# GuyTevet/motion-diffusion-model

Hardware: AMD Instinct MI355X
Metric: motions/sec (B=128, T=196, 50-step DDPM) (higher is better)
Workload: dtype f16x3 (fp32 operands split into fp16 hi+lo, 3 fp16 MFMA products, fp32 accumulate; everything else fp32); 1 GPU; HumanML3D text2motion, 50-step p_sample_loop with CFG 2.5 (2 denoiser forwards per step), batch=128 per GPU, T=196, 8-layer d=512 trans_enc MDM, random-init weights, cached text embedding; global_batch=128, diffusion_steps=50, parallelism=dp1: batch shards, no data-path collective, all_gather of final samples

## Files before the change

include/mdm_hip_probe.h:

```cpp
#ifndef MDM_HIP_PROBE_H
#define MDM_HIP_PROBE_H

#include "mdm_hip.h"

#ifdef __cplusplus
extern "C" {
#endif

int mdm_debug_set(int what, int value);
int mdm_debug_get(int idx, double* out);

size_t mdm_linear_f16f6_scratch_bytes(int32_t M, int32_t N, int32_t K);
int mdm_linear_f16f6(const float* in_dev, const float* w_dev, const float* bias_dev, const float* res_dev,
                     float* out_dev, int32_t M, int32_t N, int32_t K, int32_t act, void* scratch_dev,
                     size_t scratch_bytes, void* stream);

int mdm_probe_in_proj(const float* tokens, const float* w, const float* bias, void* planes_dev, int32_t nseq, int32_t S,
                      int32_t D, void* scratch_dev, void* stream);

int mdm_probe_attention_x3(const float* qkv_dev, float* out_dev, void* out_hi_dev, void* out_lo_dev, const int32_t* lengths_dev,
                           int32_t nseq, int32_t B, int32_t S, int32_t D, int32_t H, int32_t lead, int32_t wide, void* scratch_dev,
                           size_t scratch_bytes, void* stream);

#ifdef __cplusplus
}
#endif
#endif
```

motion-diffusion-model_amd/_native.py:

```python
import ctypes as C
import os

_HERE = os.path.dirname(os.path.abspath(__file__))
LIB_NAME = "libmdm_hip.so"
LIB_PATH = os.path.join(_HERE, "csrc", LIB_NAME)
PROBE_LIB_PATH = os.path.join(_HERE, "csrc", "libmdm_hip_probe.so")

MDM_OK = 0
BRANCH_COND, BRANCH_UNCOND, BRANCH_BOTH = 0, 1, 2
ACT_NONE, ACT_GELU, ACT_SILU = 0, 1, 2
PRECISIONS = {"f32": 0, "f16x3": 1}
PROF_CLASSES = ("linear", "attention", "layernorm", "embed", "outproj", "elementwise")

EXPORTED_SYMBOLS = [
    "mdm_abi_version", "mdm_build_info", "mdm_last_error", "mdm_create", "mdm_destroy", "mdm_set_weight", "mdm_const_bytes",
    "mdm_prepare", "mdm_workspace_bytes", "mdm_forward", "mdm_sampler_step", "mdm_randn", "mdm_sample_loop",
    "mdm_linear", "mdm_layernorm", "mdm_attention", "mdm_profile_enable", "mdm_profile_read", "mdm_profile_reset",
    "mdm_set_precision", "mdm_linear_x3", "mdm_linear_x3_scratch_bytes", "mdm_attention_x3", "mdm_attention_x3_scratch_bytes",
    "mdm_recover_from_ric", "mdm_workspace_bytes_dec", "mdm_forward_dec", "mdm_workspace_bytes_dec_loop",
    "mdm_sample_loop_dec", "mdm_weights_in_range", "mdm_set_option", "mdm_get_option", "mdm_set_time_add",
    "mdm_rot6d_to_smpl_joints", "mdm_smpl_workspace_bytes", "mdm_smpl_forward",
    "mdm_eval_workspace_bytes", "mdm_eval_motion_embeddings", "mdm_eval_text_embeddings",
    "mdm_text_workspace_bytes", "mdm_text_encode",
    "mdm_stgcn_workspace_bytes", "mdm_stgcn_forward",
    "mdm_gru_cls_workspace_bytes", "mdm_gru_cls_forward",
    "mdm_clip_text_workspace_bytes", "mdm_clip_text_encode",
]
PROBE_SYMBOLS = ["mdm_debug_set", "mdm_debug_get", "mdm_linear_f16f6", "mdm_linear_f16f6_scratch_bytes", "mdm_probe_in_proj",
                 "mdm_probe_attention_x3"]
ABI_VERSION = 10
OPTIONS = {"small_gemm_max_seqs": 1, "small_gemm_row_tiles": 2, "dec_fused_xattn": 3, "dec_fused_selfattn": 4, "attn_direct_out": 5,
           "dec_time_token": 6, "enc_shared_layer0": 7, "attn_wide": 8}
ARCH = {"trans_enc": 0, "trans_dec": 1}


class MdmConfig(C.Structure):
    _fields_ = [(n, C.c_int32) for n in ("njoints", "nfeats", "latent_dim", "ff_size", "num_layers", "num_heads",
                                         "clip_dim", "max_len", "mask_frames", "arch", "context_len")]


class MdmSmplModel(C.Structure):
    _fields_ = [(n, C.c_void_p) for n in ("j0", "jdirs", "blend", "weights_t", "sel_blend", "sel_weights_t", "extra_t")] + \
               [("parents", C.POINTER(C.c_int32))] + [(n, C.c_int32) for n in ("J", "V", "n_sel", "n_extra")]


class MdmSmplCall(C.Structure):
    _fields_ = [(n, C.c_int32) for n in ("pose_rep", "glob", "translation", "vertstrans", "n_points", "root_point")] + \
               [("point_map", C.POINTER(C.c_int32)), ("glob_rot_mat", C.POINTER(C.c_float)), ("beta1", C.c_float)]


class MdmEvalGru(C.Structure):
    _fields_ = [(n, C.c_void_p) for n in ("in_w", "in_b", "w_ih", "b_ih", "w_hh", "b_hh", "h0", "o1_w", "o1_b", "ln_g", "ln_b",
                                          "o2_w", "o2_b")] + [(n, C.c_int32) for n in ("in_dim", "hidden", "out")]


class MdmEvalModel(C.Structure):
    _fields_ = [(n, C.c_void_p) for n in ("conv1_w", "conv1_b", "conv2_w", "conv2_b", "out_w", "out_b", "pos_w", "pos_b")] + \
               [("motion", MdmEvalGru), ("text", MdmEvalGru)] + \
               [(n, C.c_int32) for n in ("dim_pose", "conv_hidden", "latent", "word", "pos", "unit_length")]


class MdmTextLayer(C.Structure):
    _fields_ = [(n, C.c_void_p) for n in ("qkv_w", "qkv_b", "out_w", "out_b", "sa_ln_g", "sa_ln_b", "lin1_w", "lin1_b", "lin2_w",
                                          "lin2_b", "out_ln_g", "out_ln_b")]


class MdmTextModel(C.Structure):
    _fields_ = [(n, C.c_void_p) for n in ("word_emb", "pos_emb", "emb_ln_g", "emb_ln_b")] + [("layers", C.POINTER(MdmTextLayer))] + \
               [(n, C.c_int32) for n in ("n_layers", "dim", "n_heads", "hidden", "vocab", "max_pos")] + [("ln_eps", C.c_float)]


class MdmStgcnBlock(C.Structure):
    _fields_ = [(n, C.c_void_p) for n in ("gcn_w", "gcn_scale", "gcn_shift", "nbr_idx", "nbr_w", "nbr_cnt", "tcn_w", "tcn_scale",
                                          "tcn_shift", "res_w", "res_scale", "res_shift")] + \
               [(n, C.c_int32) for n in ("c_in", "c_out", "stride", "residual")]


class MdmStgcnModel(C.Structure):
    _fields_ = [("blocks", C.POINTER(MdmStgcnBlock))] + [(n, C.c_void_p) for n in ("in_scale", "in_shift", "fcn_w", "fcn_b")] + \
               [(n, C.c_int32) for n in ("n_blocks", "V", "K", "num_class")]


class MdmGruClsLayer(C.Structure):
    _fields_ = [(n, C.c_void_p) for n in ("w_ih", "w_hh", "b_ih", "b_hh")]


GRU_CLS_MAX_LAYERS = 4


class MdmGruClsModel(C.Structure):
    _fields_ = [("layers", MdmGruClsLayer * GRU_CLS_MAX_LAYERS)] + [(n, C.c_void_p) for n in ("lin1_w", "lin1_b", "lin2_w", "lin2_b")] + \
               [(n, C.c_int32) for n in ("input_size", "hidden_size", "num_layers", "mid", "num_class")]


class MdmClipTextLayer(C.Structure):
    _fields_ = [(n, C.c_void_p) for n in ("ln1_g", "ln1_b", "qkv_w", "qkv_b", "out_w", "out_b", "ln2_g", "ln2_b", "fc_w", "fc_b", "proj_w",
                                          "proj_b")]


class MdmClipTextModel(C.Structure):
    _fields_ = [(n, C.c_void_p) for n in ("tok_emb", "pos_emb", "lnf_g", "lnf_b", "text_proj")] + [("layers", C.POINTER(MdmClipTextLayer))] + \
               [(n, C.c_int32) for n in ("n_layers", "dim", "n_heads", "mlp", "vocab", "max_pos", "embed")]


STGCN_RES = {"none": 0, "identity": 1, "conv": 2}
STGCN_MAX_BLOCKS, STGCN_MAX_NEIGHBOURS = 16, 8

SMPL_POSE_REPS = {"rot6d": 0, "rotvec": 1, "rotmat": 2, "rotquat": 3}
SMPL_REP_FEATS = {"rot6d": 6, "rotvec": 3, "rotmat": 9, "rotquat": 4}


class MdmStep(C.Structure):
    _fields_ = [("a_x0", C.c_float), ("a_xt", C.c_float), ("sigma", C.c_float), ("clip_denoised", C.c_int32),
                ("seed", C.c_uint64), ("sample_base", C.c_uint32), ("draw", C.c_uint32), ("const_noise", C.c_int32)]


class MdmSampleParams(C.Structure):
    _fields_ = [
        ("B", C.c_int32), ("T", C.c_int32), ("num_timesteps", C.c_int32), ("start_index", C.c_int32),
        ("a_x0", C.c_void_p), ("a_xt", C.c_void_p), ("sigma", C.c_void_p), ("timestep_map", C.c_void_p),
        ("text_embed_dev", C.c_void_p), ("scale_dev", C.c_void_p), ("lengths_dev", C.c_void_p),
        ("inpaint_mask_dev", C.c_void_p), ("inpaint_motion_dev", C.c_void_p), ("noise_dev", C.c_void_p),
        ("seed", C.c_uint64), ("sample_base", C.c_uint32), ("clip_denoised", C.c_int32),
        ("force_uncond", C.c_int32), ("x0_dev", C.c_void_p), ("dump_steps", C.c_void_p), ("num_dump", C.c_int32),
        ("dump_dev", C.c_void_p), ("const_noise", C.c_int32),
    ]


class MdmSampleDecParams(C.Structure):
    _fields_ = [("loop", MdmSampleParams), ("ntok", C.c_int32), ("prefix_dev", C.c_void_p),
                ("text_lengths_dev", C.c_void_p)]


class MdmError(RuntimeError):
    pass


class MdmLib:

    def __init__(self, path):
        if not os.path.isfile(path):
            raise MdmError(
                f"{path} not found: the MI355X HIP extension is not built. Run `python __graft_entry__.py build` "
                f"(hipcc --offload-arch=gfx950). There is no CPU fallback for this path.")
        self.path = path
        lib = self.lib = C.CDLL(path)
        vp, i32, i64, u32, u64, f32, sz = C.c_void_p, C.c_int32, C.c_int64, C.c_uint32, C.c_uint64, C.c_float, C.c_size_t
        P = C.POINTER
        sig = {
            "mdm_abi_version": (C.c_int, []),
            "mdm_last_error": (C.c_char_p, []),
            "mdm_build_info": (C.c_char_p, []),
            "mdm_create": (C.c_int, [P(MdmConfig), P(vp)]),
            "mdm_destroy": (None, [vp]),
            "mdm_set_weight": (C.c_int, [vp, C.c_char_p, vp, i64]),
            "mdm_const_bytes": (sz, [vp]),
            "mdm_prepare": (C.c_int, [vp, vp, sz, vp]),
            "mdm_workspace_bytes": (sz, [vp, i32, i32]),
            "mdm_forward": (C.c_int, [vp, vp, vp, vp, vp, i32, i32, i32, vp, vp, sz, vp]),
            "mdm_sampler_step": (C.c_int, [vp, vp, vp, vp, vp, vp, vp, vp, vp, i32, i32, P(MdmStep), vp]),
            "mdm_randn": (C.c_int, [vp, vp, vp, f32, f32, i32, i32, u64, u32, u32, vp]),
            "mdm_sample_loop": (C.c_int, [vp, P(MdmSampleParams), vp, vp, sz, vp]),
            "mdm_linear": (C.c_int, [vp, vp, vp, vp, vp, i32, i32, i32, i32, vp]),
            "mdm_layernorm": (C.c_int, [vp, vp, vp, i32, i32, vp]),
            "mdm_attention": (C.c_int, [vp, vp, vp, i32, i32, i32, i32, i32, vp]),
            "mdm_set_precision": (C.c_int, [vp, i32]),
            "mdm_weights_in_range": (C.c_int, [vp, P(i32), vp]),
            "mdm_linear_x3_scratch_bytes": (sz, [i32, i32, i32]),
            "mdm_linear_x3": (C.c_int, [vp, vp, vp, vp, vp, i32, i32, i32, i32, vp, sz, vp]),
            "mdm_attention_x3_scratch_bytes": (sz, [i32, i32, i32]),
            "mdm_attention_x3": (C.c_int, [vp, vp, vp, i32, i32, i32, i32, i32, vp, sz, vp]),
            "mdm_recover_from_ric": (C.c_int, [vp, vp, vp, vp, i32, i32, i32, i32, vp]),
            "mdm_workspace_bytes_dec": (sz, [vp, i32, i32, i32]),
            "mdm_forward_dec": (C.c_int, [vp, vp, vp, vp, vp, vp, vp, i32, i32, i32, i32, vp, vp, sz, vp]),
            "mdm_workspace_bytes_dec_loop": (sz, [vp, i32, i32, i32, i32]),
            "mdm_sample_loop_dec": (C.c_int, [vp, P(MdmSampleDecParams), vp, vp, sz, vp]),
            "mdm_profile_enable": (C.c_int, [vp, C.c_int]),
            "mdm_profile_read": (C.c_int, [vp, i32, P(C.c_double), P(i64), P(C.c_double)]),
            "mdm_profile_reset": (C.c_int, [vp]),
            "mdm_set_option": (C.c_int, [vp, i32, i32]),
            "mdm_get_option": (C.c_int, [vp, i32, P(i32)]),
            "mdm_set_time_add": (C.c_int, [vp, vp, i32]),
            "mdm_rot6d_to_smpl_joints": (C.c_int, [vp, vp, P(f32), P(i32), vp, i32, i32, i32, i32, vp]),
            "mdm_smpl_workspace_bytes": (sz, [P(MdmSmplModel), P(MdmSmplCall), i32, i32]),
            "mdm_smpl_forward": (C.c_int, [P(MdmSmplModel), P(MdmSmplCall), vp, vp, vp, vp, vp, i32, i32, i32, i32, vp, sz, vp]),
            "mdm_eval_workspace_bytes": (sz, [P(MdmEvalModel), i32, i32, i32]),
            "mdm_eval_motion_embeddings": (C.c_int, [P(MdmEvalModel), vp, vp, vp, i32, i32, i32, vp, sz, vp]),
            "mdm_eval_text_embeddings": (C.c_int, [P(MdmEvalModel), vp, vp, vp, vp, i32, i32, i32, vp, sz, vp]),
            "mdm_text_workspace_bytes": (sz, [P(MdmTextModel), i32, i32]),
            "mdm_text_encode": (C.c_int, [P(MdmTextModel), vp, vp, vp, i32, i32, i32, vp, sz, vp]),
            "mdm_clip_text_workspace_bytes": (sz, [P(MdmClipTextModel), i32, i32]),
            "mdm_clip_text_encode": (C.c_int, [P(MdmClipTextModel), vp, vp, vp, i32, i32, vp, sz, vp]),
            "mdm_stgcn_workspace_bytes": (sz, [P(MdmStgcnModel), i32, i32]),
            "mdm_stgcn_forward": (C.c_int, [P(MdmStgcnModel), vp, vp, vp, i32, i32, vp, sz, vp]),
            "mdm_gru_cls_workspace_bytes": (sz, [P(MdmGruClsModel), i32, i32]),
            "mdm_gru_cls_forward": (C.c_int, [P(MdmGruClsModel), vp, vp, vp, vp, vp, i32, i32, vp, sz, vp]),
        }
        probe_sig = {
            "mdm_debug_set": (C.c_int, [C.c_int, C.c_int]),
            "mdm_debug_get": (C.c_int, [C.c_int, P(C.c_double)]),
            "mdm_linear_f16f6_scratch_bytes": (sz, [i32, i32, i32]),
            "mdm_linear_f16f6": (C.c_int, [vp, vp, vp, vp, vp, i32, i32, i32, i32, vp, sz, vp]),
            "mdm_probe_in_proj": (C.c_int, [vp, vp, vp, vp, i32, i32, i32, vp, vp]),
            "mdm_probe_attention_x3": (C.c_int, [vp, vp, vp, vp, vp, i32, i32, i32, i32, i32, i32, i32, vp, sz, vp]),
        }
        self.has_probes = hasattr(lib, "mdm_debug_set")
        if self.has_probes:
            sig.update(probe_sig)
        for name, (res, args) in sig.items():
            fn = getattr(lib, name)
            fn.restype = res
            fn.argtypes = args
        if lib.mdm_abi_version() != ABI_VERSION:
            raise MdmError(f"{path}: ABI version {lib.mdm_abi_version()} != {ABI_VERSION}")
        self.build_info = dict(kv.split("=", 1) for kv in lib.mdm_build_info().decode().split(";"))
        if self.build_info.get("emu") != "1" and self.build_info.get("slp") != "off" \
                and os.environ.get("MDM_ALLOW_SLP_BUILD") != "1":
            raise MdmError(f"{path} was built without -fno-slp-vectorize -DMDM_NO_SLP=1 (mdm_build_info: "
                           f"{lib.mdm_build_info().decode()}): rebuild with `python __graft_entry__.py`, or set "
                           f"MDM_ALLOW_SLP_BUILD=1 for an A/B experiment on an otherwise idle device")

    def check(self, rc, what):
        if rc != MDM_OK:
            msg = self.lib.mdm_last_error()
            raise MdmError(f"{what} failed (rc={rc}): {msg.decode() if msg else ''}")

    def __getattr__(self, name):
        return getattr(self.lib, name)


_LIB = None


def load_native():
    global _LIB
    if _LIB is None:
        _LIB = MdmLib(os.environ.get("MDM_HIP_LIB", LIB_PATH))
    return _LIB


_PROBE_LIB = None


def load_probe():
    global _PROBE_LIB
    if _PROBE_LIB is None:
        _PROBE_LIB = MdmLib(os.environ.get("MDM_HIP_PROBE_LIB", PROBE_LIB_PATH))
        if not _PROBE_LIB.has_probes:
            raise MdmError(f"{_PROBE_LIB.path} was not built with -DMDM_PROBES")
    return _PROBE_LIB
```

motion-diffusion-model_amd/csrc/api_launch.h:

```cpp
#pragma once

namespace {

struct Workspace {
  float *tok, *qkv, *att, *ffn, *cond;
  QkvPlanes qp;
  p16_t *xah, *xal;
  float *stat1, *stat2;
  p16_t *tokh, *tokl;
  p16_t *atth, *attl;
  p16_t *ffnh, *ffnl;
  size_t bytes;
};

QkvPlanes carve_qkv_planes(float* qkv, size_t nseq, size_t S, size_t D, int H) {
  const size_t NKT = (S + 31) / 32, SP = 32 * NKT, plane = nseq * SP * D;
  p16_t* q = reinterpret_cast<p16_t*>(qkv);
  QkvPlanes qp{};
  qp.qh = q; qp.SP = (int)SP; qp.NKT = (int)NKT; qp.H = H;
  if (q != nullptr) { qp.ql = q + plane; qp.kh = q + 2 * plane; qp.kl = q + 3 * plane; qp.vh = q + 4 * plane; qp.vl = q + 5 * plane; }
  return qp;
}

Workspace carve(const mdm_model* m, int nseq, int T, void* base) {
  const size_t D = m->cfg.latent_dim, FF = m->cfg.ff_size, S = (size_t)T + 1, M = (size_t)nseq * S;
  size_t off = 0;
  auto take = [&](size_t floats) {
    size_t o = off;
    off += align_up(floats * sizeof(float), 256);
    return base ? reinterpret_cast<float*>(static_cast<char*>(base) + o) : nullptr;
  };
  Workspace w;
  w.tok = take(M * D);
  const size_t NKT = (S + 31) / 32, SP = 32 * NKT;
  w.qkv = take((size_t)nseq * SP * 3 * D);
  w.att = take(M * D);
  w.ffn = take(M * std::max(FF, (size_t)m->jf_k));
  w.cond = take((size_t)nseq * D);
  float* tp = take(M * D);
  w.tokh = reinterpret_cast<p16_t*>(tp);
  w.tokl = tp ? w.tokh + M * D : nullptr;
  w.atth = reinterpret_cast<p16_t*>(w.att);
  w.attl = w.att ? w.atth + M * D : nullptr;
  w.ffnh = reinterpret_cast<p16_t*>(w.ffn);
  w.ffnl = w.ffn ? w.ffnh + M * FF : nullptr;
  w.xah = reinterpret_cast<p16_t*>(w.tok);
  w.xal = w.tok ? w.xah + M * D : nullptr;
  const size_t parts = (D + 127) / 128;
  w.stat1 = take(M * parts * 2 + 4);
  w.stat2 = take(M * parts * 2 + 4);
  w.qp = carve_qkv_planes(w.qkv, nseq, S, D, m->cfg.num_heads);
  w.bytes = off;
  return w;
}

int launch_layernorm(Profiler* pf, float* x, const float* g, const float* b, int rows, int D, p16_t* xh, p16_t* xl,
                     hipStream_t s, bool write_f32 = true) {
  ProfScope ps(pf, MDM_PROF_LAYERNORM, 0.0, s);
  const dim3 grid((rows + 3) / 4), block(256);
  switch (D / 256) {
    case 1: { auto k = &layernorm_kernel<1>; MDM_LAUNCH(k, grid, block, 0, s, x, g, b, rows, 1e-5f, xh, xl, (int)write_f32); break; }
    case 2: { auto k = &layernorm_kernel<2>; MDM_LAUNCH(k, grid, block, 0, s, x, g, b, rows, 1e-5f, xh, xl, (int)write_f32); break; }
    case 3: { auto k = &layernorm_kernel<3>; MDM_LAUNCH(k, grid, block, 0, s, x, g, b, rows, 1e-5f, xh, xl, (int)write_f32); break; }
    case 4: { auto k = &layernorm_kernel<4>; MDM_LAUNCH(k, grid, block, 0, s, x, g, b, rows, 1e-5f, xh, xl, (int)write_f32); break; }
    default: return fail(MDM_EUNSUPPORTED, "layernorm: D must be 256, 512, 768 or 1024");
  }
  return rt_launch_status();
}

template <int NKT>
int launch_attention_t(const AttnF32Args& a, float* out, int nseq, int D, int H, p16_t* oh, p16_t* ol, hipStream_t s) {
  auto k = &attention_f32_kernel<NKT>;
  const int nqt = (a.Sq + 31) / 32;
  const size_t lds = attention_lds_bytes(NKT, nqt);
  if (int rc = rt_allow_lds(k, lds)) return rc;
  MDM_LAUNCH(k, dim3(nseq * H), dim3(64 * nqt), lds, s, a, out, D, H, oh, ol);
  return rt_launch_status();
}

int launch_attention_args(Profiler* pf, const AttnF32Args& a, float* out, int nseq, int D, int H, p16_t* oh, p16_t* ol,
                          hipStream_t s) {
  ProfScope ps(pf, MDM_PROF_ATTENTION, 4.0 * nseq * H * (double)a.Sq * a.Sk * ATT_HD, s);
  if (D != H * ATT_HD) return fail(MDM_EUNSUPPORTED, "attention: head_dim must be 128");
  if (a.Sq < 1 || a.Sk < 1) return fail(MDM_EUNSUPPORTED, "attention: no tokens");
  if (a.Sq > 224 || a.Sk > 224) {
    const int nqb = al_query_blocks(a.Sq);
    MDM_LAUNCH(attention_f32_long_kernel, dim3(nseq * H * nqb), dim3(256), al_f32_lds_bytes(), s, a, out, D, H, oh, ol, nqb);
    return rt_launch_status();
  }
  switch ((a.Sk + 31) / 32) {
    case 1: return launch_attention_t<1>(a, out, nseq, D, H, oh, ol, s);
    case 2: return launch_attention_t<2>(a, out, nseq, D, H, oh, ol, s);
    case 3: return launch_attention_t<3>(a, out, nseq, D, H, oh, ol, s);
    case 4: return launch_attention_t<4>(a, out, nseq, D, H, oh, ol, s);
    case 5: return launch_attention_t<5>(a, out, nseq, D, H, oh, ol, s);
    case 6: return launch_attention_t<6>(a, out, nseq, D, H, oh, ol, s);
    default: return launch_attention_t<7>(a, out, nseq, D, H, oh, ol, s);
  }
}

int launch_attention(Profiler* pf, const float* qkv, float* out, const int* lengths, int nseq, int B, int S, int D,
                     int H, p16_t* oh, p16_t* ol, hipStream_t s, int lead = 1, int len_B = 0, int len_b0 = 0) {
  AttnF32Args a{qkv, 3 * D, qkv + D, qkv + 2 * D, 3 * D, S, S, lengths, lead, B};
  a.len_B = len_B;
  a.len_b0 = len_b0;
  return launch_attention_args(pf, a, out, nseq, D, H, oh, ol, s);
}

template <int NKT, bool DIRECT>
int launch_attention_x3_t(const QkvPlanes& qp, const int* lengths, int nseq, int B, int S, int D, float* out, p16_t* oh,
                          p16_t* ol, hipStream_t s, int lead) {
  auto k = &attention_x3_kernel<NKT, DIRECT>;
  const size_t lds = attention_x3_lds_bytes(NKT);
  if (int rc = rt_allow_lds(k, lds)) return rc;
  const int items = nseq * qp.H, groups = (items + 7) / 8;
  const int grid = std::min(groups * 16, std::max(16, 2 * x3_grid_limit() / 16 * 16));
  MDM_LAUNCH(k, dim3(grid), dim3(256), lds, s, qp, lengths, S, D, B, lead, out, oh, ol, items);
  return rt_launch_status();
}
template <bool DIRECT>
int launch_attention_x3_nkt(const QkvPlanes& qp, const int* lengths, int nseq, int B, int S, int D, float* out, p16_t* oh,
                            p16_t* ol, hipStream_t s, int lead) {
  switch (qp.NKT) {
    case 1: return launch_attention_x3_t<1, DIRECT>(qp, lengths, nseq, B, S, D, out, oh, ol, s, lead);
    case 2: return launch_attention_x3_t<2, DIRECT>(qp, lengths, nseq, B, S, D, out, oh, ol, s, lead);
    case 3: return launch_attention_x3_t<3, DIRECT>(qp, lengths, nseq, B, S, D, out, oh, ol, s, lead);
    case 4: return launch_attention_x3_t<4, DIRECT>(qp, lengths, nseq, B, S, D, out, oh, ol, s, lead);
    case 5: return launch_attention_x3_t<5, DIRECT>(qp, lengths, nseq, B, S, D, out, oh, ol, s, lead);
    case 6: return launch_attention_x3_t<6, DIRECT>(qp, lengths, nseq, B, S, D, out, oh, ol, s, lead);
    default: return launch_attention_x3_t<7, DIRECT>(qp, lengths, nseq, B, S, D, out, oh, ol, s, lead);
  }
}

template <int NKT>
int launch_attention_x3_wide_t(const QkvPlanes& qp, const int* lengths, int nseq, int B, int S, int D, float* out, p16_t* oh,
                               p16_t* ol, hipStream_t s, int lead) {
  auto k = &attention_x3_kernel_wide<NKT>;
  const size_t lds = (size_t)axw_lds_bytes(NKT);
  if (int rc = rt_allow_lds(k, lds)) return rc;
  const int items = nseq * qp.H;
  const int grid = std::min(items, x3_grid_limit());
  MDM_LAUNCH(k, dim3(grid), dim3(AXW_THREADS), lds, s, qp, lengths, S, D, B, lead, out, oh, ol, items);
  return rt_launch_status();
}

int launch_attention_x3(Profiler* pf, const QkvPlanes& qp, const int* lengths, int nseq, int B, int S, int D, float* out,
                        p16_t* oh, p16_t* ol, hipStream_t s, int lead = 1, bool direct = false, bool wide = true) {
  ProfScope ps(pf, MDM_PROF_ATTENTION, 4.0 * nseq * qp.H * (double)S * S * AX_HD, s);
  if (D != qp.H * AX_HD) return fail(MDM_EUNSUPPORTED, "attention: head_dim must be 128");
  if (S < 1) return fail(MDM_EUNSUPPORTED, "attention: no tokens");
  if (S > 224) {
    if (qp.NKT != (S + 31) / 32 || qp.SP != 32 * qp.NKT) return fail(MDM_EINVAL, "attention: the operand planes do not match the sequence length");
    const int nqb = al_query_blocks(S);
    MDM_LAUNCH(attention_x3_long_kernel, dim3(nseq * qp.H * nqb), dim3(256), al_x3_lds_bytes(), s, qp, lengths, S, D, B, lead, out, oh, ol, nqb);
    return rt_launch_status();
  }
  if (direct && out == nullptr && oh != nullptr)
    return launch_attention_x3_nkt<true>(qp, lengths, nseq, B, S, D, out, oh, ol, s, lead);
  if (wide && qp.NKT >= 5) {
    if (qp.NKT != (S + 31) / 32 || qp.SP != 32 * qp.NKT) return fail(MDM_EINVAL, "attention: the operand planes do not match the sequence length");
    switch (qp.NKT) {
      case 5: return launch_attention_x3_wide_t<5>(qp, lengths, nseq, B, S, D, out, oh, ol, s, lead);
      case 6: return launch_attention_x3_wide_t<6>(qp, lengths, nseq, B, S, D, out, oh, ol, s, lead);
      default: return launch_attention_x3_wide_t<7>(qp, lengths, nseq, B, S, D, out, oh, ol, s, lead);
    }
  }
  return launch_attention_x3_nkt<false>(qp, lengths, nseq, B, S, D, out, oh, ol, s, lead);
}

struct X3Call {
  X3Kind kind = X3K_OUT_LN_RES;
  Profiler* pf = nullptr; int prof_cat = MDM_PROF_LINEAR;
  X3Operand a{nullptr, nullptr}; X3Weights w{nullptr, nullptr}; const float* bias = nullptr;
  float* out = nullptr; p16_t* oh = nullptr; p16_t* ol = nullptr; const QkvPlanes* qp = nullptr;
  int M = 0, N = 0, K = 0, S = 0, D = 0;
  int scale_cols = 0; float col_scale = 1.f;
  const float* astat = nullptr; const float* colsum = nullptr;
  X3Operand res{nullptr, nullptr}; const float* rstat = nullptr; const float* rgamma = nullptr; const float* rbeta = nullptr;
  float* ostat = nullptr;
  int parts = 1; float inv_dim = 1.f;
  const float* res_f32 = nullptr; int emb_T = 1, emb_B = 1, emb_nbranch = 1;
  bool small = false;
  X3sShape shape{1};
  int stat_cols = 256;
};
X3Epilogue x3_epilogue(const X3Call& c) {
  X3Epilogue ep{};
  ep.out = c.out; ep.bias = c.bias; ep.res = c.res_f32; ep.resh = c.res.hi; ep.resl = c.res.lo; ep.oh = c.oh; ep.ol = c.ol;
  ep.ld = c.N; ep.scale_cols = c.scale_cols; ep.col_scale = c.col_scale;
  if (c.qp != nullptr) ep.qkv = *c.qp;
  ep.S = c.S; ep.D = c.D;
  ep.astat = c.astat; ep.colsum = c.colsum; ep.rstat = c.rstat; ep.rgamma = c.rgamma; ep.rbeta = c.rbeta; ep.ostat = c.ostat;
  ep.stat_parts = c.parts; ep.inv_dim = c.inv_dim; ep.emb_T = c.emb_T; ep.emb_B = c.emb_B; ep.emb_nbranch = c.emb_nbranch;
  ep.stat_cols = c.stat_cols;
  return ep;
}

#ifdef MDM_PROBES
int g_f6_linear = 0;
void* g_f6_dbg_scratch = nullptr;
size_t g_f6_dbg_bytes = 0;
int launch_linear_f6_debug(Profiler* pf, const float* in, int ld_in, const float* w, const float* bias, const float* res,
                           float* out, int M, int N, int K, int act, int scale_cols, float col_scale, hipStream_t s) {
  const size_t wfrag = align_up(x3_packed_weight_elems(N, K) * 2, 256);
  const size_t need = f6_plane_bytes(M, K) + 2 * wfrag;
  if (need > g_f6_dbg_bytes) {
#ifdef MDM_EMU
    free(g_f6_dbg_scratch);
    g_f6_dbg_scratch = malloc(need);
#else
    if (hipDeviceSynchronize() != hipSuccess) return fail(MDM_EHIP, "f16f6 debug mode: synchronize failed");
    if (g_f6_dbg_scratch != nullptr) (void)hipFree(g_f6_dbg_scratch);
    if (hipMalloc(&g_f6_dbg_scratch, need) != hipSuccess) { g_f6_dbg_scratch = nullptr; g_f6_dbg_bytes = 0; return fail(MDM_EHIP, "f16f6 debug mode: hipMalloc failed"); }
#endif
    g_f6_dbg_bytes = need;
  }
  ProfScope ps(pf, MDM_PROF_LINEAR, 2.0 * M * (double)N * K, s);
  char* base = static_cast<char*>(g_f6_dbg_scratch);
  const F6Planes pa = f6_carve(base, M, K);
  p16_t* wfh = reinterpret_cast<p16_t*>(base + f6_plane_bytes(M, K));
  p16_t* wfl = reinterpret_cast<p16_t*>(base + f6_plane_bytes(M, K) + wfrag);
  MDM_LAUNCH(pack_f16f6_kernel, dim3((M * (K / 32) + 255) / 256), dim3(256), 0, s, in, pa, M, K, ld_in);
  if (int rc = rt_launch_status()) return rc;
  const int npad = (N + 31) / 32 * 32;
  MDM_LAUNCH(pack_weight_f16f6_kernel, dim3((npad * (K / 32) + 255) / 256), dim3(256), 0, s, w, wfh, wfl, N, K);
  if (int rc = rt_launch_status()) return rc;
  X3Call c; c.out = out; c.bias = bias; c.res_f32 = res; c.N = N; c.scale_cols = scale_cols; c.col_scale = col_scale;
  X3Epilogue ep = x3_epilogue(c);
  ep.acc_scale = 1.f;
  const X3Operand a{reinterpret_cast<const p16_t*>(pa.h16), reinterpret_cast<const p16_t*>(pa.rec)};
  const int rc = launch_gemm_f16f6(a, X3Weights{wfh, wfl}, ep, M, N, K, act, s);
  if (rc != 0) return fail(MDM_EUNSUPPORTED, "f16f6 debug mode: launch failed");
  return rt_launch_status();
}
#endif

int launch_linear(Profiler* pf, const float* in, int ld_in, const float* w, const float* bias, const float* res,
                  float* out, int M, int N, int K, int act, int scale_cols, float col_scale, hipStream_t s, bool x3 = false) {
#ifdef MDM_PROBES
  if (g_f6_linear && K % 32 == 0 && N % 4 == 0 && ld_in % 4 == 0 && (scale_cols % 256 == 0) &&
      (act == ACT_NONE || (act == ACT_GELU && res == nullptr)))
    return launch_linear_f6_debug(pf, in, ld_in, w, bias, res, out, M, N, K, act, scale_cols, col_scale, s);
#endif
  ProfScope ps(pf, MDM_PROF_LINEAR, 2.0 * M * (double)N * K, s);
  if (K % 4 != 0 || ld_in % 4 != 0) return fail(MDM_EINVAL, "linear: K and the row stride must be multiples of 4");
  RowMajorLoader al{in, ld_in, M, K};
  RowMajorLoader bl{w, K, N, K};
  LinearEpilogue ep{out, bias, res, N, act, scale_cols, col_scale, nullptr, nullptr};
  launch_gemm_f32(al, bl, ep, M, N, K, s, x3);
  return rt_launch_status();
}

int launch_linear_lnfold(Profiler* pf, const float* in, int ld_in, const LnFold& a_ln, const float* w, X3Weights wp,
                         const float* bias, const float* colsum, const float* res, const LnFold& res_ln, float* out,
                         float* ostat, int M, int N, int K, int act, int scale_cols, float col_scale, hipStream_t s, bool x3) {
  ProfScope ps(pf, MDM_PROF_LINEAR, 2.0 * M * (double)N * K, s);
  if (K % 16 != 0 || ld_in % 4 != 0 || N % LN_PART_COLS != 0) return fail(MDM_EINVAL, "linear (LayerNorm fold): bad K / N");
  RowMajorLoader al{in, ld_in, M, K};
  LnLinearEpilogue ep{out, bias, N, act, scale_cols, col_scale, a_ln, colsum, res, res_ln, ostat};
  if (x3 && wp.hi != nullptr) {
    X3FragB bl{wp.hi, wp.lo, (N + 31) / 32, K};
    launch_gemm_f32(al, bl, ep, M, N, K, s, true);
  } else {
    RowMajorLoader bl{w, K, N, K};
    launch_gemm_f32(al, bl, ep, M, N, K, s, x3);
  }
  return rt_launch_status();
}

int launch_linear_x3(Profiler* pf, X3Operand a, X3Weights w, const float* bias, const float* res, float* out,
                     p16_t* oh, p16_t* ol, int M, int N, int K, int act, int scale_cols, float col_scale, int seq_len,
                     hipStream_t s, X3Operand res_planes = X3Operand{nullptr, nullptr}) {
  if (K % X3_BK != 0) return fail(MDM_EINVAL, "f16x3 linear: K must be a multiple of 32");
  if (N % 4 != 0) return fail(MDM_EINVAL, "f16x3 linear: N must be a multiple of 4");
  ProfScope ps(pf, MDM_PROF_LINEAR, 2.0 * M * (double)N * K, s);
  X3Call c; c.out = out; c.oh = oh; c.ol = ol; c.bias = bias; c.res_f32 = res; c.res = res_planes; c.N = N;
  c.scale_cols = scale_cols; c.col_scale = col_scale;
  const int rc = launch_gemm_x3(a, w, x3_epilogue(c), M, N, K, act, seq_len, s);
  if (rc == -2) return fail(MDM_EUNSUPPORTED, "f16x3 linear: unsupported (activation, residual, output) combination");
  return rt_launch_status();
}

int launch_in_proj_x3(Profiler* pf, X3Operand a, X3Weights w, const float* bias, const QkvPlanes& qp, int nseq, int S,
                      int D, float qscale, hipStream_t s, int pair_B = 0) {
  if (D % X3_BK != 0) return fail(MDM_EINVAL, "f16x3 in_proj: latent_dim must be a multiple of 32");
  const double rows = pair_B > 0 ? (double)pair_B * (S + 1) : (double)nseq * S;
  ProfScope ps(pf, MDM_PROF_LINEAR, 2.0 * rows * 3.0 * D * (double)D, s);
  X3Call c; c.bias = bias; c.qp = &qp; c.N = 3 * D; c.S = S; c.D = D; c.scale_cols = D; c.col_scale = qscale;
  const int rc = launch_gemm_x3_qkv(a, w, x3_epilogue(c), nseq, S, D, s, pair_B);
  if (rc == -2) return fail(MDM_EUNSUPPORTED, pair_B > 0 ? "f16x3 in_proj: the paired layer-0 launch does not cover this shape"
                                                         : "f16x3 in_proj: sequences longer than 224 tokens");
  return rt_launch_status();
}

inline bool use_small_gemm(const mdm_model* m, int nseq, int S) {
  return m->precision == MDM_PREC_F16X3 && m->lnfold && (nseq <= m->x3s.max_seqs || S > X3_TM) &&
         m->cfg.latent_dim % 128 == 0 && m->cfg.latent_dim % 256 == 0 && m->cfg.ff_size % 256 == 0;
}
int launch_x3_ln(const X3Call& c, hipStream_t s) {
  const X3Kind kind = c.kind;
  const int M = c.M, N = c.N, K = c.K, S = c.S;
  if (K % X3_BK != 0 || N % 4 != 0) return fail(MDM_EINVAL, "f16x3 linear: K % 32 and N % 4 must be 0");
  if (c.parts < 1 || c.parts > (c.small ? 8 : 4)) return fail(MDM_EUNSUPPORTED, "folded LayerNorm: too many partial sums per row (D <= 1024)");
  ProfScope ps(c.pf, c.prof_cat, 2.0 * M * (double)N * K, s);
  const X3Epilogue ep = x3_epilogue(c);
  const bool in_proj = kind == X3K_IN_PROJ_FOLD || kind == X3K_IN_PROJ_PLAIN;
  if (c.small) {
    const int group_rows = in_proj ? S : (kind == X3K_EMBED ? c.emb_T : M);
    const int rc = launch_gemm_x3s(kind, c.shape, c.a, c.w, ep, M, N, K, group_rows, s);
    if (rc == -1 || rc == -3) return lds_fail(rc, "f16x3 linear (small tiles)");
    if (rc == -2) return fail(MDM_EUNSUPPORTED, "f16x3 linear (small tiles): unsupported shape (K must be 288 or a multiple of 256)");
    return rt_launch_status();
  }
  if (kind == X3K_IN_PROJ_PLAIN) {
    const int rc6 = launch_gemm_x3_qkv(c.a, c.w, ep, M / S, S, c.D, s);
    if (rc6 != 0) return fail(MDM_EUNSUPPORTED, "f16x3 in_proj: launch failed");
    return rt_launch_status();
  }
  const int rpt = (kind == X3K_IN_PROJ_FOLD) ? S : x3_rows_per_tile(M, kind == X3K_EMBED ? c.emb_T : S);
  const int rc = launch_gemm_x3_ln(kind, c.a, c.w, ep, M, N, K, rpt, s);
  if (rc == -1 || rc == -3) return lds_fail(rc, "f16x3 linear");
  if (rc == -2) return fail(MDM_EUNSUPPORTED, "f16x3 linear: unsupported folded-LayerNorm GEMM kind");
  return rt_launch_status();
}

int launch_pack_weights(const float* src, p16_t* hi, p16_t* lo, int N, int K, hipStream_t s, int* overflow = nullptr) {
  if (K % 16 != 0) return fail(MDM_EINVAL, "pack_weights: K must be a multiple of 16");
  const size_t n = x3_packed_weight_elems(N, K) / 8;
  const int grid = (int)std::min<size_t>((n + 255) / 256, 4096);
  MDM_LAUNCH(pack_weight_planes_kernel, dim3(grid), dim3(256), 0, s, src, hi, lo, N, K, overflow);
  return rt_launch_status();
}

int launch_split(const float* src, p16_t* hi, p16_t* lo, size_t n, hipStream_t s) {
  if (n % 4 != 0) return fail(MDM_EINVAL, "split: element count must be a multiple of 4");
  const size_t n4 = n / 4;
  const int grid = (int)std::min<size_t>((n4 + 255) / 256, 4096);
  MDM_LAUNCH(split_planes_kernel, dim3(grid), dim3(256), 0, s, src, hi, lo, n4);
  return rt_launch_status();
}

}
```

motion-diffusion-model_amd/csrc/api_runtime.h:

```cpp
#pragma once

namespace {

thread_local std::string g_err;
#ifdef MDM_PROBES
int g_x3_reuse_planes = 0;
int g_f6_reference = 0;
#else
constexpr int g_x3_reuse_planes = 0;
#endif

int fail(int code, const std::string& msg) {
  g_err = msg;
  return code;
}

#ifdef MDM_EMU
inline int rt_launch_status() { return 0; }
inline int rt_copy(void* dst, const void* src, size_t bytes, hipStream_t) { memcpy(dst, src, bytes); return 0; }
template <class K> inline int rt_allow_lds(K, size_t) { return 0; }
#else
inline int rt_launch_status() {
  hipError_t e = hipGetLastError();
  if (e != hipSuccess) return fail(MDM_EHIP, std::string("kernel launch failed: ") + hipGetErrorString(e));
  return 0;
}
inline int rt_copy(void* dst, const void* src, size_t bytes, hipStream_t s) {
  hipError_t e = hipMemcpyAsync(dst, src, bytes, hipMemcpyDeviceToDevice, s);
  if (e != hipSuccess) return fail(MDM_EHIP, std::string("hipMemcpyAsync failed: ") + hipGetErrorString(e));
  return 0;
}
template <class K> inline int rt_allow_lds(K kernel, size_t bytes) {
  hipError_t e = hipFuncSetAttribute(reinterpret_cast<const void*>(kernel),
                                     hipFuncAttributeMaxDynamicSharedMemorySize, (int)bytes);
  if (e != hipSuccess) return fail(MDM_EHIP, std::string("hipFuncSetAttribute failed: ") + hipGetErrorString(e));
  return 0;
}
#endif

inline size_t align_up(size_t v, size_t a) { return (v + a - 1) / a * a; }

inline size_t ws_bytes_of(size_t floats) { return floats * sizeof(float) + 64; }
inline float* ws_floats(void* ws) { return reinterpret_cast<float*>((reinterpret_cast<uintptr_t>(ws) + 15) & ~(uintptr_t)15); }

inline int check_weight_ptrs(const std::string& f, const void* const* ptrs, const char* const* names, int n,
                             const std::string& group = std::string()) {
  for (int i = 0; i < n; ++i) {
    if (ptrs[i] == nullptr) return fail(MDM_EINVAL, f + "null weight pointer " + group + names[i]);
    if ((reinterpret_cast<uintptr_t>(ptrs[i]) & 15) != 0)
      return fail(MDM_EINVAL, f + "weight pointer " + group + names[i] + " must be 16-byte aligned");
  }
  return 0;
}

inline int lds_fail(int rc, const char* what) {
  if (rc == -3)
    return fail(MDM_EUNSUPPORTED, std::string(what) + ": first use of this kernel instantiation while the stream is being captured into a "
                "hipGraph -- run one warm-up call of the SAME shapes (batch, frames, text tokens) outside the capture first");
  return fail(MDM_EHIP, std::string(what) + ": hipFuncSetAttribute(MaxDynamicSharedMemorySize) failed");
}

}

struct Profiler {
  bool on = false;
#ifdef MDM_EMU
  int64_t launches[MDM_PROF_NUM] = {};
#else
  struct Rec { int cat; hipEvent_t a, b; double flops; };
  std::vector<Rec> recs;
  std::vector<hipEvent_t> pool;
  hipEvent_t get() {
    if (!pool.empty()) { hipEvent_t e = pool.back(); pool.pop_back(); return e; }
    hipEvent_t e = nullptr;
    (void)hipEventCreate(&e);
    return e;
  }
  ~Profiler() {
    for (auto& r : recs) { (void)hipEventDestroy(r.a); (void)hipEventDestroy(r.b); }
    for (auto e : pool) (void)hipEventDestroy(e);
  }
#endif
};

struct ProfScope {
#ifndef MDM_EMU
  Profiler* p; size_t idx; hipStream_t s;
  ProfScope(Profiler* prof, int cat, double flops, hipStream_t st) : p(prof && prof->on ? prof : nullptr), idx(0), s(st) {
    if (!p) return;
    Profiler::Rec r{cat, p->get(), p->get(), flops};
    (void)hipEventRecord(r.a, s);
    idx = p->recs.size();
    p->recs.push_back(r);
  }
  ~ProfScope() { if (p) (void)hipEventRecord(p->recs[idx].b, s); }
#else
  ProfScope(Profiler* prof, int cat, double, hipStream_t) { if (prof && prof->on) ++prof->launches[cat]; }
#endif
};

struct AuxStreams {
  static constexpr int kMax = 3;
#ifndef MDM_EMU
  hipStream_t s[kMax] = {};
  hipEvent_t fork = nullptr, join[kMax] = {};
  int n = 0;
  int ensure(int want) {
    if (fork == nullptr && hipEventCreateWithFlags(&fork, hipEventDisableTiming) != hipSuccess) return fail(MDM_EHIP, "hipEventCreate failed");
    for (; n < want && n < kMax; ++n)
      if (hipStreamCreateWithFlags(&s[n], hipStreamNonBlocking) != hipSuccess ||
          hipEventCreateWithFlags(&join[n], hipEventDisableTiming) != hipSuccess) return fail(MDM_EHIP, "hipStreamCreate failed");
    return MDM_OK;
  }
  ~AuxStreams() {
    for (int i = 0; i < kMax; ++i) {
      if (join[i] != nullptr) (void)hipEventDestroy(join[i]);
      if (s[i] != nullptr) (void)hipStreamDestroy(s[i]);
    }
    if (fork != nullptr) (void)hipEventDestroy(fork);
  }
#endif
};

struct mdm_model {
  mdm_config_t cfg;
  Profiler prof;
  AuxStreams aux;
  std::map<std::string, const float*> w;
  std::map<std::string, int64_t> expect;
  bool prepared = false;
  int* range_flag = nullptr;
  float* w_in_pad = nullptr;
  float* time_table = nullptr;
  const float* time_add_next = nullptr;
  int time_add_B = 0;
  const float* time_add = nullptr;
  bool dec_time_token = false;
  int jf = 0, jf_pad = 0;
  int precision = MDM_PREC_F16X3;
  struct LayerPlanes { X3Weights in_proj, out_proj, linear1, linear2; };
  std::vector<LayerPlanes> planes;
  struct LayerFold { X3Weights in_proj, linear1; float *c_qkv, *b_qkv, *c_1, *b_1; };
  std::vector<LayerFold> fold;
  struct DecFold { float *w_in, *c_in, *b_in, *w_q, *c_q, *b_q, *w_1, *c_1, *b_1; };
  std::vector<DecFold> dec_fold;
  struct DecPlanes { X3Weights in_proj, out_proj, q, out_proj2, linear1, linear2; };
  std::vector<DecPlanes> dec_planes;
  X3Weights in_planes{nullptr, nullptr};
  int jf_k = 0;
  X3Weights out_planes_f{nullptr, nullptr};
  float *c_out = nullptr, *b_out = nullptr;
  float *wkv_all = nullptr, *bkv_all = nullptr;
  bool lnfold = false;
  X3sOptions x3s;
  int fused_xattn = 3;
  bool fused_selfattn = true;
  bool enc_shared_l0 = true;
  bool attn_direct = false;
  bool attn_wide = true;
  X3Weights out_planes{nullptr, nullptr};
  float* out_bias_pad = nullptr;
  int jf_out = 0;

  const float* W(const std::string& k) const { return w.at(k); }
  const float* L(int layer, const char* suffix) const {
    return w.at((cfg.arch == MDM_ARCH_TRANS_DEC ? "seqTransDecoder.layers." : "seqTransEncoder.layers.") +
                std::to_string(layer) + "." + suffix);
  }
};

namespace {

#ifdef MDM_EMU
struct ChainGuard { explicit ChainGuard(void*) {} };
#else
struct DeviceChain {
  std::mutex mu;
  hipEvent_t ev = nullptr;
  hipStream_t last = nullptr;
  bool has = false;
};
DeviceChain g_chain[kMaxDevices];
struct ChainGuard {
  DeviceChain& c;
  hipStream_t s;
  explicit ChainGuard(void* stream) : c(g_chain[rt_device_ordinal()]), s(static_cast<hipStream_t>(stream)) {
    c.mu.lock();
#ifdef MDM_PROBES
    static const bool chain_free = [] { const char* e = getenv("MDM_CHAIN_FREE"); return e != nullptr && e[0] == '1'; }();
#else
    constexpr bool chain_free = false;
#endif
    if (c.has && c.last != s && !chain_free) {
      hipStreamCaptureStatus cap = hipStreamCaptureStatusNone;
      const bool capturing = hipStreamIsCapturing(s, &cap) == hipSuccess && cap != hipStreamCaptureStatusNone;
      if (!capturing) {
        if (c.ev == nullptr && hipEventCreateWithFlags(&c.ev, hipEventDisableTiming) != hipSuccess) c.ev = nullptr;
        if (c.ev != nullptr && hipEventRecord(c.ev, c.last) == hipSuccess) (void)hipStreamWaitEvent(s, c.ev, 0);
        else (void)hipGetLastError();
      }
    }
  }
  ~ChainGuard() {
    c.last = s;
    c.has = true;
    c.mu.unlock();
  }
  ChainGuard(const ChainGuard&) = delete;
  ChainGuard& operator=(const ChainGuard&) = delete;
};
#endif

int check_ready(const mdm_model* m) {
  if (m == nullptr) return fail(MDM_EINVAL, "null model");
  if (!m->prepared) return fail(MDM_ESTATE, "mdm_prepare has not been called (or weights changed since)");
  return 0;
}

struct TimeAddScope {
  mdm_model* m;
  int rc = 0;
  TimeAddScope(mdm_model* m_, int B, const char* who) : m(m_) {
    if (m->time_add_next == nullptr) return;
    if (m->time_add_B != B)
      rc = fail(MDM_EINVAL, std::string(who) + ": mdm_set_time_add bound " + std::to_string(m->time_add_B) + " samples, this call has " +
                                std::to_string(B));
    else
      m->time_add = m->time_add_next;
    m->time_add_next = nullptr;
    m->time_add_B = 0;
  }
  ~TimeAddScope() { m->time_add = nullptr; }
  TimeAddScope(const TimeAddScope&) = delete;
  TimeAddScope& operator=(const TimeAddScope&) = delete;
};

}
```

motion-diffusion-model_amd/csrc/attention_x3.h:

```cpp
#pragma once
#include "common.h"

namespace mdm {

constexpr int AX_HD = 128;
constexpr int AX_OLD = AX_HD + 4;

struct QkvPlanes {
  p16_t *qh, *ql, *kh, *kl, *vh, *vl;
  int SP, NKT, H;
};

__host__ __device__ __forceinline__ int ax_key_of_pos(int p) { return (p & 3) + 8 * ((p >> 2) & 1) + 4 * (p >> 3); }

constexpr int AX_SLOT = 16384, AX_RING = 4;
constexpr int AX_OST = 64 + 4;
constexpr int AX_KMASK_BYTES = 1024;
constexpr int ax_lds_bytes(int) { return AX_RING * AX_SLOT + AX_KMASK_BYTES; }
static_assert(AX_SLOT + 4 * 32 * AX_OST * 4 <= AX_RING * AX_SLOT, "output staging must fit behind ring slot 0");

template <int N> __device__ __forceinline__ void ax_vm_wait() {
#ifdef MDM_EMU
  emu::vm_wait(N);
#else
// ... 11 lines not shown
  asm volatile("global_store_dwordx2 %0, %1, off" : : "v"(lo_p), "v"(u32x2{l01, l23}) : "memory");
#endif
}
template <int NKT, bool DIRECT>
__global__ __launch_bounds__(256, 2) void attention_x3_kernel(QkvPlanes P, const int* __restrict__ lengths,
                                                                    int S, int D, int B, int lead, float* __restrict__ out,
                                                                    p16_t* __restrict__ oh, p16_t* __restrict__ ol,
                                                                    int items) {
  MDM_DYN_SMEM(unsigned char, lds);
  constexpr int SP = 32 * NKT;
  constexpr int NTILES = 2 * NKT;

  const int tid = threadIdx.x;
  const int lane = tid & 63;
#ifdef MDM_EMU
  const int w = tid >> 6;
#else
  const int w = __builtin_amdgcn_readfirstlane(tid >> 6);
#endif
  const int r = lane & 31, h = lane >> 5;
  const int H = P.H;
  int vb = (int)blockIdx.x;
  const int vb_total = (items + 7) / 8 * 16, vb_step = (int)gridDim.x;
  const int half = (vb >> 3) & 1;
  auto item_of = [](int b) { return (b >> 4) * 8 + (b & 7); };
  if (item_of(vb) >= items) return;
  const int qt = 4 * half + w;
  const bool active = qt < NKT;
  const bool last_group = S > 32 * (NKT - 1) + 16;

  auto issue_tile = [&](size_t sh, int t, int lv) {
#pragma unroll
    for (int i = 0; i < 4; ++i) {
      const int j = 4 * w + i, plane = j >> 3, idx = j & 7;
      unsigned char* dst = lds + (t & (AX_RING - 1)) * AX_SLOT + plane * 8192 + idx * 1024;
      if (t < NKT) {
        const int key = 32 * t + 4 * idx + (lv >> 4);
        const p16_t* src = (plane ? P.kl : P.kh) + (sh * SP + (size_t)min(key, S - 1)) * AX_HD + (((lv & 15) ^ (key & 15)) * 8);
        glds16(src, dst);
      } else {
        const int d = 16 * idx + (lv >> 2);
        const p16_t* src = (plane ? P.vl : P.vh) + ((sh * NKT + (size_t)(t - NKT)) * AX_HD + d) * 32 + (((lv & 3) ^ ((d >> 2) & 3)) * 8);
        glds16(src, dst);
      }
    }
  };
  p16x8 qh[8], ql[8];
  auto load_q = [&](size_t sh) {
    const size_t qo = (sh * SP + min(32 * (active ? qt : 0) + r, S - 1)) * AX_HD + 8 * h;
#pragma unroll
    for (int st = 0; st < 8; ++st) {
      qh[st] = *reinterpret_cast<const p16x8*>(P.qh + qo + 16 * st);
      ql[st] = *reinterpret_cast<const p16x8*>(P.ql + qo + 16 * st);
    }
  };
  issue_tile((size_t)item_of(vb), 0, lane);
  load_q((size_t)item_of(vb));
  bool first_item = true;
  constexpr int AX_NST = 32;

  for (;;) {
  const int item = item_of(vb);
  const int seq = item / H, head = item - seq * H;
  const size_t sh = (size_t)item;
  const int vb_next = vb + vb_step;
  const bool has_next = vb_next < vb_total && item_of(vb_next) < items;
  int nvalid = S;
  const uint32_t* kbits = nullptr;
  if (lengths != nullptr) {
    const int cnt = lengths[seq % B];
    if (cnt >= 0) nvalid = min(S, lead + cnt);
    else kbits = reinterpret_cast<const uint32_t*>(lengths + B + 8 * (seq % B));
  }
  if (tid < 32 * NKT) {
    const int f = max(tid - lead, 0);
    const bool ok = kbits == nullptr ? tid < nvalid : (tid < S && (tid < lead || ((kbits[f >> 5] >> (f & 31)) & 1u)));
    reinterpret_cast<float*>(lds + AX_RING * AX_SLOT)[tid] = ok ? 0.f : -INFINITY;
  }
  int lv = lane;
#ifndef MDM_EMU
  asm volatile("" : "+v"(lv));
#endif

  const bool carried = DIRECT && !first_item;
  if (!carried) {
    wait_vmem_all();
    wg_barrier();
    if (NTILES > 1) issue_tile(sh, 1, lv);
    if (NTILES > 2) issue_tile(sh, 2, lv);
  }

  f32x16 p[NKT];
#pragma unroll
  for (int kt = 0; kt < NKT; ++kt)
#pragma unroll
    for (int e = 0; e < 16; ++e) p[kt][e] = 0.f;
  f32x16 o[4];
  float inv = 1.f;

  const uint32_t klane = (uint32_t)(r * 256 + ((h ^ (r & 15)) * 16));
  const uint32_t vlane = (uint32_t)(r * 64 + ((h ^ ((r >> 2) & 3)) * 16));
#ifndef MDM_EMU
  const uint32_t lbase = lds_addr_of(lds);
#endif

  static_for<NTILES>([&](auto t_tag) __attribute__((always_inline)) {
    constexpr int t = decltype(t_tag)::value;
    constexpr int slot = t & (AX_RING - 1);
    constexpr int ahead = (NTILES - 1 - t) < 2 ? (NTILES - 1 - t) : 2;
    if constexpr (DIRECT && t < 3 && NTILES > 3) {
#ifdef MDM_EMU
      constexpr int kTrk = 0;
#else
      constexpr int kTrk = 1;
#endif
      if (carried && active) ax_vm_wait<4 * ahead + kTrk * (AX_NST + (t == 0 ? 16 : 0))>();
      else if (carried) ax_vm_wait<4 * ahead + kTrk * (t == 0 ? 16 : 0)>();
      else wait_vmem_upto<4 * ahead>();
    } else wait_vmem_upto<4 * ahead>();
    wg_barrier();
    if constexpr (t + 3 < NTILES) issue_tile(sh, t + 3, lv);
    if constexpr (t == NTILES - 1) {
      if (has_next) issue_tile((size_t)item_of(vb_next), 0, lv);
      load_q(has_next ? (size_t)item_of(vb_next) : sh);
    }

    if constexpr (t < NKT) {
      if (active) {
        p16x8 kh[3], kl[3];
#ifdef MDM_EMU
#define AX_RD_K(dst, plane, st) lds_read16(dst, lds, slot * AX_SLOT + (plane) * 8192 + (klane ^ ((st) << 5)))
#else
        const uint32_t kb = lbase + klane;
#define AX_RD_K(dst, plane, st) lds_read16<slot * AX_SLOT + (plane) * 8192>(dst, kb ^ (uint32_t)((st) << 5))
#endif
        static_for<8 + 2>([&](auto u_tag) __attribute__((always_inline)) {
          constexpr int u = decltype(u_tag)::value;
          if constexpr (u < 8) {
            AX_RD_K(kh[u % 3], 0, u);
            AX_RD_K(kl[u % 3], 1, u);
          }
          if constexpr (u >= 2) {
            constexpr int st = u - 2;
            constexpr int younger = 2 * ((7 - st) < 2 ? (7 - st) : 2);
            lds_wait<younger>(kh[st % 3], kl[st % 3]);
            sched_fence();
            p[t] = mfma_p16(kl[st % 3], qh[st], p[t]);
            p[t] = mfma_p16(kh[st % 3], ql[st], p[t]);
            p[t] = mfma_p16(kh[st % 3], qh[st], p[t]);
            sched_fence();
          }
        });
#undef AX_RD_K
      }
      if constexpr (t == NKT - 1) {
        float mx = -INFINITY;
        {
          const float* km = reinterpret_cast<const float*>(lds + AX_RING * AX_SLOT) + 4 * h;
#pragma unroll
          for (int kt = 0; kt < NKT; ++kt)
#pragma unroll
            for (int g = 0; g < 4; ++g) {
              const float4 m4 = ld4(km + kt * 32 + 8 * g);
              const float s0 = p[kt][4 * g] + m4.x, s1 = p[kt][4 * g + 1] + m4.y, s2 = p[kt][4 * g + 2] + m4.z,
                          s3 = p[kt][4 * g + 3] + m4.w;
              p[kt][4 * g] = s0; p[kt][4 * g + 1] = s1; p[kt][4 * g + 2] = s2; p[kt][4 * g + 3] = s3;
              mx = fmaxf(mx, fmaxf(fmaxf(s0, s1), fmaxf(s2, s3)));
            }
        }
        mx = fmaxf(mx, shfl_xor_f32(mx, 32));
        mx -= 6.931471805599453f;
        float sum = 0.f;
#pragma unroll
        for (int kt = 0; kt < NKT; ++kt)
#pragma unroll
          for (int e = 0; e < 16; ++e) {
#ifdef MDM_EMU
            const float pe = expf(p[kt][e] - mx);
#else
            const float pe = __expf(p[kt][e] - mx);
#endif
            p[kt][e] = pe;
            sum += pe;
          }
        sum += shfl_xor_f32(sum, 32);
        inv = 1.0f / sum;
      }
    } else {
      constexpr int kt = t - NKT;
      if constexpr (kt == 0) {
#pragma unroll
        for (int dt = 0; dt < 4; ++dt)
#pragma unroll
          for (int e = 0; e < 16; ++e) o[dt][e] = 0.f;
      }
      if (active) {
        p16x8 vh[3], vl[3], ph, pl;
#ifdef MDM_EMU
#define AX_RD_V(dst, plane, s2, dt) lds_read16(dst, lds, slot * AX_SLOT + (plane) * 8192 + (dt) * 2048 + (vlane ^ ((s2) << 5)))
#else
        const uint32_t vb = lbase + vlane;
#define AX_RD_V(dst, plane, s2, dt) lds_read16<slot * AX_SLOT + (plane) * 8192 + (dt) * 2048>(dst, vb ^ (uint32_t)((s2) << 5))
#endif
        static_for<8 + 2>([&](auto u_tag) __attribute__((always_inline)) {
          constexpr int u = decltype(u_tag)::value;
          if constexpr (u < 8) {
            AX_RD_V(vh[u % 3], 0, u / 4, u % 4);
            AX_RD_V(vl[u % 3], 1, u / 4, u % 4);
          }
          if constexpr (u >= 2) {
            constexpr int uv = u - 2, s2 = uv / 4, dt = uv % 4;
            if constexpr (dt == 0) {
              float pv[8];
#pragma unroll
              for (int j = 0; j < 8; ++j) pv[j] = p[kt][8 * s2 + j];
              split8(pv, ph, pl);
            }
            constexpr int younger = 2 * ((7 - uv) < 2 ? (7 - uv) : 2);
            lds_wait<younger>(vh[uv % 3], vl[uv % 3]);
            sched_fence();
            if (kt < NKT - 1 || s2 == 0 || last_group) {
              o[dt] = mfma_p16(vl[uv % 3], ph, o[dt]);
              o[dt] = mfma_p16(vh[uv % 3], pl, o[dt]);
              o[dt] = mfma_p16(vh[uv % 3], ph, o[dt]);
            }
            sched_fence();
          }
        });
#undef AX_RD_V
      }
    }
  });
  wg_barrier();
  if constexpr (DIRECT) {
    if (has_next) {
      if (NTILES > 1) issue_tile((size_t)item_of(vb_next), 1, lv);
      if (NTILES > 2) issue_tile((size_t)item_of(vb_next), 2, lv);
    }
    if (active) {
      const int qq = 32 * qt + r;
      if (qq < S) {
        const size_t obase = ((size_t)seq * S + qq) * D + head * AX_HD + 4 * h;
#pragma unroll
        for (int dt = 0; dt < 4; ++dt)
#pragma unroll
          for (int g = 0; g < 4; ++g)
            ax_split4_store_counted(oh + obase + 32 * dt + 8 * g, ol + obase + 32 * dt + 8 * g,
                                    make_float4(o[dt][4 * g + 0] * inv, o[dt][4 * g + 1] * inv, o[dt][4 * g + 2] * inv, o[dt][4 * g + 3] * inv));
      }
    }
    first_item = false;
    if (!has_next) break;
    vb = vb_next;
    continue;
  }

  float* so = reinterpret_cast<float*>(lds + AX_SLOT) + w * (32 * AX_OST);
  if (active) {
    const size_t obase = (size_t)seq * S * D + head * AX_HD;
#pragma unroll
    for (int pass = 0; pass < 2; ++pass) {
#pragma unroll
      for (int dd = 0; dd < 2; ++dd)
#pragma unroll
        for (int g = 0; g < 4; ++g) {
          const int dt = 2 * pass + dd;
          st4(&so[r * AX_OST + dd * 32 + 8 * g + 4 * h],
              make_float4(o[dt][4 * g + 0] * inv, o[dt][4 * g + 1] * inv, o[dt][4 * g + 2] * inv, o[dt][4 * g + 3] * inv));
        }
      wave_lds_fence();
#pragma unroll
      for (int i = 0; i < 8; ++i) {
        const int row = 4 * i + (lv >> 4), qq = 32 * qt + row, c4 = lv & 15;
        if (qq < S) {
          const float4 v = ld4(&so[row * AX_OST + 4 * c4]);
          const size_t oo = obase + (size_t)qq * D + 64 * pass + 4 * c4;
          if (out != nullptr) st4(out + oo, v);
          if (oh != nullptr) {
            split4_store(oh + oo, ol + oo, v);
          }
        }
      }
      wave_lds_fence();
    }
  }
  if (!has_next) break;
  vb = vb_next;
  }
  wait_vmem_all();
}

inline size_t attention_x3_lds_bytes(int nkt) { return (size_t)ax_lds_bytes(nkt); }

constexpr int AXW_RING = 6, AXW_AHEAD = 3, AXW_THREADS = 512;
constexpr int AXW_STAGE = 32 * AX_OST * 4;
constexpr int AXW_KMASK_OFF = AXW_RING * AX_SLOT, AXW_STAGE_OFF = AXW_KMASK_OFF + AX_KMASK_BYTES;
constexpr int axw_lds_bytes(int nkt) { return AXW_STAGE_OFF + nkt * AXW_STAGE; }
static_assert(axw_lds_bytes(7) <= 160 * 1024, "ring + mask + staging of seven compute waves fit the CU's LDS");
__host__ __device__ __forceinline__ int axw_slot(int first, int t) {
  const int s = first + t % AXW_RING;
  return s >= AXW_RING ? s - AXW_RING : s;
}

template <int NKT>
__global__ __launch_bounds__(AXW_THREADS) void attention_x3_kernel_wide(QkvPlanes P, const int* __restrict__ lengths, int S, int D,
                                                                       int B, int lead, float* __restrict__ out,
                                                                       p16_t* __restrict__ oh, p16_t* __restrict__ ol, int items) {
  static_assert(NKT >= 5 && NKT <= 7, "one wave per query tile and at least one copy wave");
  MDM_DYN_SMEM(unsigned char, lds);
  constexpr int SP = 32 * NKT;
  constexpr int NTILES = 2 * NKT;
  static_assert(NTILES > AXW_AHEAD, "the prologue's tiles belong to the first item");
  constexpr int NCW = (8 - NKT) >= 2 ? 2 : 1;
  constexpr int PPW = 16 / NCW;

  const int tid = threadIdx.x;
  const int lane = tid & 63;
#ifdef MDM_EMU
  const int w = tid >> 6;
#else
  const int w = __builtin_amdgcn_readfirstlane(tid >> 6);
#endif
  const int H = P.H;
  const int step = (int)gridDim.x;
  int item = (int)blockIdx.x;
  int first = 0;

  if (w >= NKT) {
    const int c = w - NKT;
    const bool carrier = c < NCW;
    auto issue_tile = [&](size_t sh, int t, int slot, int lv) {
      if (!carrier) return;
#pragma unroll
      for (int i = 0; i < PPW; ++i) {
        const int j = PPW * c + i, plane = j >> 3, idx = j & 7;
        unsigned char* dst = lds + slot * AX_SLOT + plane * 8192 + idx * 1024;
        if (t < NKT) {
          const int key = 32 * t + 4 * idx + (lv >> 4);
          const p16_t* src = (plane ? P.kl : P.kh) + (sh * SP + (size_t)min(key, S - 1)) * AX_HD + (((lv & 15) ^ (key & 15)) * 8);
          glds16(src, dst);
        } else {
          const int d = 16 * idx + (lv >> 2);
          const p16_t* src = (plane ? P.vl : P.vh) + ((sh * NKT + (size_t)(t - NKT)) * AX_HD + d) * 32 + (((lv & 3) ^ ((d >> 2) & 3)) * 8);
          glds16(src, dst);
        }
      }
    };
#pragma unroll
    for (int t = 0; t < AXW_AHEAD; ++t) issue_tile((size_t)item, t, t, lane);
    for (;;) {
      const int next = item + step;
      const bool has_next = next < items;
      const int first_next = axw_slot(first, NTILES);
      int lv = lane;
#ifndef MDM_EMU
      asm volatile("" : "+v"(lv));
#endif
      static_for<NTILES>([&](auto t_tag) __attribute__((always_inline)) {
        constexpr int t = decltype(t_tag)::value;
        constexpr int tn = t + AXW_AHEAD;
        if constexpr (tn < NTILES) issue_tile((size_t)item, tn, axw_slot(first, tn), lv);
        else if (has_next) issue_tile((size_t)next, tn - NTILES, axw_slot(first_next, tn - NTILES), lv);
        constexpr int tail = (NTILES - 1 - t) < AXW_AHEAD ? (NTILES - 1 - t) : AXW_AHEAD;
        if (has_next) ax_vm_wait<PPW * AXW_AHEAD>();
        else ax_vm_wait<PPW * tail>();
        wg_barrier();
      });
      if (!has_next) break;
      item = next;
      first = first_next;
    }
    wait_vmem_all();
    return;
  }

  const int r = lane & 31, h = lane >> 5;
  const int qt = w;
  const bool last_group = S > 32 * (NKT - 1) + 16;
  p16x8 qh[8], ql[8];
  auto load_q = [&](size_t sh) {
    const size_t qo = (sh * SP + min(32 * qt + r, S - 1)) * AX_HD + 8 * h;
#pragma unroll
    for (int st = 0; st < 8; ++st) {
      qh[st] = *reinterpret_cast<const p16x8*>(P.qh + qo + 16 * st);
      ql[st] = *reinterpret_cast<const p16x8*>(P.ql + qo + 16 * st);
    }
  };
  load_q((size_t)item);
  const uint32_t klane = (uint32_t)(r * 256 + ((h ^ (r & 15)) * 16));
  const uint32_t vlane = (uint32_t)(r * 64 + ((h ^ ((r >> 2) & 3)) * 16));
#ifndef MDM_EMU
  const uint32_t lbase = lds_addr_of(lds);
#endif
  float* const kmask = reinterpret_cast<float*>(lds + AXW_KMASK_OFF);
  float* const so = reinterpret_cast<float*>(lds + AXW_STAGE_OFF) + w * (32 * AX_OST);

  for (;;) {
  const int seq = item / H, head = item - seq * H;
  const int next = item + step;
  const bool has_next = next < items;
  int nvalid = S;
  const uint32_t* kbits = nullptr;
  if (lengths != nullptr) {
    const int cnt = lengths[seq % B];
    if (cnt >= 0) nvalid = min(S, lead + cnt);
    else kbits = reinterpret_cast<const uint32_t*>(lengths + B + 8 * (seq % B));
  }
  if (tid < 32 * NKT) {
    const int f = max(tid - lead, 0);
    const bool ok = kbits == nullptr ? tid < nvalid : (tid < S && (tid < lead || ((kbits[f >> 5] >> (f & 31)) & 1u)));
    kmask[tid] = ok ? 0.f : -INFINITY;
  }

#ifndef MDM_EMU
  asm volatile("" : "+s"(first));
#endif

  f32x16 p[NKT];
#pragma unroll
  for (int kt = 0; kt < NKT; ++kt)
#pragma unroll
    for (int e = 0; e < 16; ++e) p[kt][e] = 0.f;
  f32x16 o[4];
  float inv = 1.f;

  static_for<NTILES>([&](auto t_tag) __attribute__((always_inline)) {
    constexpr int t = decltype(t_tag)::value;
    const uint32_t soff = (uint32_t)(axw_slot(first, t) * AX_SLOT);
    wg_barrier();
    if constexpr (t == NTILES - 1) load_q(has_next ? (size_t)next : (size_t)item);

    if constexpr (t < NKT) {
      {
        p16x8 kh[3], kl[3];
#ifdef MDM_EMU
#define AX_RD_K(dst, plane, st) lds_read16(dst, lds, soff + (plane) * 8192 + (klane ^ ((st) << 5)))
#else
        const uint32_t kb = lbase + soff + klane;
#define AX_RD_K(dst, plane, st) lds_read16<(plane) * 8192>(dst, kb ^ (uint32_t)((st) << 5))
#endif
        static_for<8 + 2>([&](auto u_tag) __attribute__((always_inline)) {
          constexpr int u = decltype(u_tag)::value;
          if constexpr (u < 8) {
            AX_RD_K(kh[u % 3], 0, u);
            AX_RD_K(kl[u % 3], 1, u);
          }
          if constexpr (u >= 2) {
            constexpr int st = u - 2;
            constexpr int younger = 2 * ((7 - st) < 2 ? (7 - st) : 2);
            lds_wait<younger>(kh[st % 3], kl[st % 3]);
            sched_fence();
            p[t] = mfma_p16(kl[st % 3], qh[st], p[t]);
            p[t] = mfma_p16(kh[st % 3], ql[st], p[t]);
            p[t] = mfma_p16(kh[st % 3], qh[st], p[t]);
            sched_fence();
          }
        });
#undef AX_RD_K
      }
      if constexpr (t == NKT - 1) {
        float mx = -INFINITY;
        {
          const float* km = kmask + 4 * h;
#pragma unroll
          for (int kt = 0; kt < NKT; ++kt)
#pragma unroll
            for (int g = 0; g < 4; ++g) {
              const float4 m4 = ld4(km + kt * 32 + 8 * g);
              const float s0 = p[kt][4 * g] + m4.x, s1 = p[kt][4 * g + 1] + m4.y, s2 = p[kt][4 * g + 2] + m4.z,
                          s3 = p[kt][4 * g + 3] + m4.w;
              p[kt][4 * g] = s0; p[kt][4 * g + 1] = s1; p[kt][4 * g + 2] = s2; p[kt][4 * g + 3] = s3;
              mx = fmaxf(mx, fmaxf(fmaxf(s0, s1), fmaxf(s2, s3)));
            }
        }
        mx = fmaxf(mx, shfl_xor_f32(mx, 32));
        mx -= 6.931471805599453f;
        float sum = 0.f;
#pragma unroll
        for (int kt = 0; kt < NKT; ++kt)
#pragma unroll
          for (int e = 0; e < 16; ++e) {
#ifdef MDM_EMU
            const float pe = expf(p[kt][e] - mx);
#else
            const float pe = __expf(p[kt][e] - mx);
#endif
            p[kt][e] = pe;
            sum += pe;
          }
        sum += shfl_xor_f32(sum, 32);
        inv = 1.0f / sum;
      }
    } else {
      constexpr int kt = t - NKT;
      if constexpr (kt == 0) {
#pragma unroll
        for (int dt = 0; dt < 4; ++dt)
#pragma unroll
          for (int e = 0; e < 16; ++e) o[dt][e] = 0.f;
      }
      {
        p16x8 vh[3], vl[3], ph, pl;
#ifdef MDM_EMU
#define AX_RD_V(dst, plane, s2, dt) lds_read16(dst, lds, soff + (plane) * 8192 + (dt) * 2048 + (vlane ^ ((s2) << 5)))
#else
        const uint32_t vb = lbase + soff + vlane;
#define AX_RD_V(dst, plane, s2, dt) lds_read16<(plane) * 8192 + (dt) * 2048>(dst, vb ^ (uint32_t)((s2) << 5))
#endif
        static_for<8 + 2>([&](auto u_tag) __attribute__((always_inline)) {
          constexpr int u = decltype(u_tag)::value;
          if constexpr (u < 8) {
            AX_RD_V(vh[u % 3], 0, u / 4, u % 4);
            AX_RD_V(vl[u % 3], 1, u / 4, u % 4);
          }
          if constexpr (u >= 2) {
            constexpr int uv = u - 2, s2 = uv / 4, dt = uv % 4;
            if constexpr (dt == 0) {
              float pv[8];
#pragma unroll
              for (int j = 0; j < 8; ++j) pv[j] = p[kt][8 * s2 + j];
              split8(pv, ph, pl);
            }
            constexpr int younger = 2 * ((7 - uv) < 2 ? (7 - uv) : 2);
            lds_wait<younger>(vh[uv % 3], vl[uv % 3]);
            sched_fence();
            if (kt < NKT - 1 || s2 == 0 || last_group) {
              o[dt] = mfma_p16(vl[uv % 3], ph, o[dt]);
              o[dt] = mfma_p16(vh[uv % 3], pl, o[dt]);
              o[dt] = mfma_p16(vh[uv % 3], ph, o[dt]);
            }
            sched_fence();
          }
        });
#undef AX_RD_V
      }
    }
  });

  {
    const size_t obase = (size_t)seq * S * D + head * AX_HD;
#pragma unroll
    for (int pass = 0; pass < 2; ++pass) {
#pragma unroll
      for (int dd = 0; dd < 2; ++dd)
#pragma unroll
        for (int g = 0; g < 4; ++g) {
          const int dt = 2 * pass + dd;
          st4(&so[r * AX_OST + dd * 32 + 8 * g + 4 * h],
              make_float4(o[dt][4 * g + 0] * inv, o[dt][4 * g + 1] * inv, o[dt][4 * g + 2] * inv, o[dt][4 * g + 3] * inv));
        }
      wave_lds_fence();
#pragma unroll
      for (int i = 0; i < 4; ++i) {
        const int row = 8 * i + (lane >> 3), qq = 32 * qt + row, c8 = lane & 7;
        if (qq < S) {
          const float4 v0 = ld4(&so[row * AX_OST + 8 * c8]), v1 = ld4(&so[row * AX_OST + 8 * c8 + 4]);
          const size_t oo = obase + (size_t)qq * D + 64 * pass + 8 * c8;
          if (out != nullptr) {
            st4(out + oo, v0);
            st4(out + oo + 4, v1);
          }
          if (oh != nullptr) {
            const float v[8] = {v0.x, v0.y, v0.z, v0.w, v1.x, v1.y, v1.z, v1.w};
            p16x8 hi, lo;
            split8(v, hi, lo);
            *reinterpret_cast<p16x8*>(oh + oo) = hi;
            *reinterpret_cast<p16x8*>(ol + oo) = lo;
          }
        }
      }
      wave_lds_fence();
    }
  }
  if (!has_next) break;
  item = next;
  first = axw_slot(first, NTILES);
  }
}

__global__ __launch_bounds__(256) void qkv_pack_kernel(const float* __restrict__ qkv, QkvPlanes P, int nseq, int S,
                                                       int D) {
  const int SP = P.SP, H = P.H;
  const size_t total = (size_t)nseq * H * SP * AX_HD;
  for (size_t i = (size_t)blockIdx.x * blockDim.x + threadIdx.x; i < total; i += (size_t)gridDim.x * blockDim.x) {
    const int d = (int)(i % AX_HD);
    const int tok = (int)((i / AX_HD) % SP);
    const size_t shd = i / ((size_t)AX_HD * SP);
    const int head = (int)(shd % H), seq = (int)(shd / H);
    float q = 0.f, k = 0.f, v = 0.f;
    if (tok < S) {
      const float* row = qkv + ((size_t)seq * S + tok) * 3 * D + head * AX_HD + d;
      q = row[0]; k = row[D]; v = row[2 * D];
    }
    p16_t a, b;
    const size_t rk = (shd * SP + tok) * AX_HD + d;
    split_p16(q, a, b); P.qh[rk] = a; P.ql[rk] = b;
    split_p16(k, a, b); P.kh[rk] = a; P.kl[rk] = b;
    const int kt = tok >> 5, k32 = tok & 31, g16 = k32 >> 4, k16 = k32 & 15;
    int pos = 0;
    for (int pp = 0; pp < 16; ++pp)
      if (ax_key_of_pos(pp) == k16) pos = pp;
    const size_t vk = ((shd * P.NKT + kt) * AX_HD + d) * 32 + 16 * g16 + pos;
    split_p16(v, a, b); P.vh[vk] = a; P.vl[vk] = b;
  }
}

}
```

motion-diffusion-model_amd/csrc/encoder.h:

```cpp
#pragma once

namespace {

int embed_frames_x3(mdm_model* m, const Workspace& ws, const float* x, int B, int T, int nbranch, hipStream_t s, const CondTokArgs& ct) {
  const int D = m->cfg.latent_dim, KP = m->jf_k;
  ProfScope ps(&m->prof, MDM_PROF_EMBED, 2.0 * B * T * (double)D * m->jf, s);
  p16_t* ph = reinterpret_cast<p16_t*>(ws.ffn);
  p16_t* pl = ph + (size_t)B * T * KP;
  MDM_LAUNCH(pose_planes_cond_kernel, dim3(((T + 31) / 32) * (KP / 32) * B + nbranch * B), dim3(256), 0, s, x, ph, pl, T, m->jf, KP, B, ct);
  if (int rc = rt_launch_status()) return rc;
  X3Call c;
  c.kind = X3K_EMBED; c.prof_cat = MDM_PROF_EMBED;
  c.a = X3Operand{ph, pl}; c.w = m->in_planes; c.bias = m->W("input_process.poseEmbedding.bias");
  c.oh = ws.tokh; c.ol = ws.tokl; c.M = B * T; c.N = D; c.K = KP; c.S = T + 1; c.D = D;
  c.res_f32 = m->W("sequence_pos_encoder.pe");
  c.emb_T = T; c.emb_B = B; c.emb_nbranch = nbranch;
  c.small = use_small_gemm(m, nbranch * B, T + 1) && KP == 288;
  c.shape = x3s_shape(m->x3s, nbranch * B);
  return launch_x3_ln(c, s);
}
inline bool use_embed_x3(const mdm_model* m, int T) {
  return m->precision == MDM_PREC_F16X3 &&
         (T + 1 <= X3_TM || (use_small_gemm(m, 1, T + 1) && m->jf_k == 288));
}

int launch_embed_f32(mdm_model* m, float* tok, p16_t* th, p16_t* tl, const float* x, const float* prefix, int C, int B, int T, int lead,
                     int nbranch, bool x3, hipStream_t s) {
  const int D = m->cfg.latent_dim;
  PoseGatherLoader al{x, T, m->jf, B * T, prefix, C};
  RowMajorLoader bl{m->w_in_pad, m->jf_pad, D, m->jf_pad};
  EmbedEpilogue ep{tok, m->W("input_process.poseEmbedding.bias"), m->W("sequence_pos_encoder.pe"), B, T, T + lead, D, nbranch, th, tl, lead};
  ProfScope ps(&m->prof, MDM_PROF_EMBED, 2.0 * B * T * (double)D * m->jf, s);
  launch_gemm_f32(al, bl, ep, B * T, D, m->jf_pad, s, x3);
  return rt_launch_status();
}

int embed_tokens(mdm_model* m, const Workspace& ws, const float* x, const long long* timesteps, int t_uniform,
                 const float* cond_emb, int B, int T, int nbranch, int uncond_from_branch, hipStream_t s) {
  const int D = m->cfg.latent_dim, S = T + 1;
  const bool x3 = m->precision == MDM_PREC_F16X3;
  if (use_embed_x3(m, T)) {
    const CondTokArgs ct{ws.tok, cond_emb, m->W("embed_text.bias"), m->time_table, timesteps, t_uniform, m->W("sequence_pos_encoder.pe"), B, S, D,
                         uncond_from_branch, (int)m->cfg.max_len, ws.tokh, ws.tokl, m->time_add};
    return embed_frames_x3(m, ws, x, B, T, nbranch, s, ct);
  }
  if (int rc = launch_embed_f32(m, ws.tok, x3 ? ws.tokh : nullptr, x3 ? ws.tokl : nullptr, x, nullptr, 0, B, T, 1, nbranch,
                                false, s)) return rc;
  ProfScope ps(&m->prof, MDM_PROF_ELEMENTWISE, 0.0, s);
  MDM_LAUNCH(cond_token_kernel, dim3(nbranch * B), dim3(128), 0, s, ws.tok, cond_emb, m->W("embed_text.bias"),
             (const float*)m->time_table, timesteps, t_uniform, m->W("sequence_pos_encoder.pe"), B, S, D, uncond_from_branch,
             (int)m->cfg.max_len, x3 ? ws.tokh : (p16_t*)nullptr, x3 ? ws.tokl : (p16_t*)nullptr, m->time_add);
  return rt_launch_status();
}

X3Call enc_ln_call(mdm_model* m, int nseq, int S) {
  const int D = m->cfg.latent_dim;
  X3Call c; c.M = nseq * S; c.S = S; c.D = D; c.inv_dim = 1.0f / (float)D;
  c.small = use_small_gemm(m, nseq, S);
  c.shape = x3s_shape(m->x3s, nseq);
  c.stat_cols = c.small ? X3S_TN : 256;
  c.parts = (D + c.stat_cols - 1) / c.stat_cols;
  return c;
}

int encoder(mdm_model* m, const Workspace& ws, int nseq, int B, int S, const int* lengths, hipStream_t s) {
  Profiler* pf = &m->prof;
  const int D = m->cfg.latent_dim, FF = m->cfg.ff_size, H = m->cfg.num_heads, M = nseq * S;
  const float qscale = 1.0f / sqrtf((float)(D / H));
  if (m->precision == MDM_PREC_F16X3 && m->lnfold && (S <= X3_TM || use_small_gemm(m, nseq, S))) {
    const X3Operand xb{ws.tokh, ws.tokl}, xa{ws.xah, ws.xal}, attp{ws.atth, ws.attl}, ffnp{ws.ffnh, ws.ffnl};
    const X3Call stack = enc_ln_call(m, nseq, S);
    const bool small = stack.small;
    auto LN = [&](X3Kind kind, X3Operand a, X3Weights w, const float* bias, int N, int K) {
      X3Call c = stack; c.kind = kind; c.pf = pf; c.a = a; c.w = w; c.bias = bias; c.N = N; c.K = K;
      return c;
    };
    for (int l = 0; l < m->cfg.num_layers; ++l) {
      const mdm_model::LayerPlanes& P = m->planes[l];
      const mdm_model::LayerFold& F = m->fold[l];
      if (l == 0 && small) {
        X3Call c = LN(X3K_IN_PROJ_PLAIN, xb, P.in_proj, m->L(l, "self_attn.in_proj_bias"), 3 * D, D);
        c.qp = &ws.qp; c.scale_cols = D; c.col_scale = qscale;
        if (int rc = launch_x3_ln(c, s)) return rc;
      } else if (l == 0) {
        const int pair_B = (m->enc_shared_l0 && nseq == 2 * B && x3_qkv_pairs(S, D)) ? B : 0;
        if (int rc = launch_in_proj_x3(pf, xb, P.in_proj, m->L(l, "self_attn.in_proj_bias"), ws.qp, nseq, S, D, qscale, s, pair_B)) return rc;
      } else {
        X3Call c = LN(X3K_IN_PROJ_FOLD, xb, F.in_proj, F.b_qkv, 3 * D, D);
        c.astat = ws.stat2; c.colsum = F.c_qkv; c.qp = &ws.qp; c.scale_cols = D; c.col_scale = qscale;
        if (int rc = launch_x3_ln(c, s)) return rc;
      }
      if (int rc = launch_attention_x3(pf, ws.qp, lengths, nseq, B, S, D, nullptr, ws.atth, ws.attl, s, 1, m->attn_direct, m->attn_wide)) return rc;
      {
        X3Call c = LN(l == 0 ? X3K_OUT_PROJ_L0 : X3K_OUT_LN_RES, attp, P.out_proj, m->L(l, "self_attn.out_proj.bias"), D, D);
        c.oh = ws.xah; c.ol = ws.xal; c.res = xb; c.ostat = ws.stat1;
        if (l >= 1) { c.rstat = ws.stat2; c.rgamma = m->L(l - 1, "norm2.weight"); c.rbeta = m->L(l - 1, "norm2.bias"); }
        if (int rc = launch_x3_ln(c, s)) return rc;
      }
      {
        X3Call c = LN(X3K_LINEAR1_GELU, xa, F.linear1, F.b_1, FF, D);
        c.oh = ws.ffnh; c.ol = ws.ffnl; c.astat = ws.stat1; c.colsum = F.c_1;
        if (int rc = launch_x3_ln(c, s)) return rc;
      }
      {
        X3Call c = LN(X3K_OUT_LN_RES, ffnp, P.linear2, m->L(l, "linear2.bias"), D, FF);
        c.oh = ws.tokh; c.ol = ws.tokl; c.res = xa; c.rstat = ws.stat1; c.rgamma = m->L(l, "norm1.weight"); c.rbeta = m->L(l, "norm1.bias");
        c.ostat = ws.stat2;
        if (int rc = launch_x3_ln(c, s)) return rc;
      }
    }
    return 0;
  }
  if (m->precision == MDM_PREC_F16X3) {
    const X3Operand tokp{ws.tokh, ws.tokl}, attp{ws.atth, ws.attl}, ffnp{ws.ffnh, ws.ffnl};
    for (int l = 0; l < m->cfg.num_layers; ++l) {
      const mdm_model::LayerPlanes& P = m->planes[l];
      if (int rc = launch_in_proj_x3(pf, tokp, P.in_proj, m->L(l, "self_attn.in_proj_bias"), ws.qp, nseq, S, D, qscale, s)) return rc;
      if (int rc = launch_attention_x3(pf, ws.qp, lengths, nseq, B, S, D, nullptr, ws.atth, ws.attl, s, 1, m->attn_direct, m->attn_wide)) return rc;
      if (int rc = launch_linear_x3(pf, attp, P.out_proj, m->L(l, "self_attn.out_proj.bias"), nullptr, ws.tok, nullptr,
                                    nullptr, M, D, D, ACT_NONE, 0, 1.f, S, s, tokp)) return rc;
      if (int rc = launch_layernorm(pf, ws.tok, m->L(l, "norm1.weight"), m->L(l, "norm1.bias"), M, D, ws.tokh, ws.tokl, s, false)) return rc;
      if (int rc = launch_linear_x3(pf, tokp, P.linear1, m->L(l, "linear1.bias"), nullptr, nullptr, ws.ffnh, ws.ffnl, M,
                                    FF, D, ACT_GELU, 0, 1.f, S, s)) return rc;
      if (int rc = launch_linear_x3(pf, ffnp, P.linear2, m->L(l, "linear2.bias"), nullptr, ws.tok, nullptr, nullptr, M, D,
                                    FF, ACT_NONE, 0, 1.f, S, s, tokp)) return rc;
      if (int rc = launch_layernorm(pf, ws.tok, m->L(l, "norm2.weight"), m->L(l, "norm2.bias"), M, D, ws.tokh, ws.tokl, s, false)) return rc;
    }
    return 0;
  }
  for (int l = 0; l < m->cfg.num_layers; ++l) {
    if (int rc = launch_linear(pf, ws.tok, D, m->L(l, "self_attn.in_proj_weight"), m->L(l, "self_attn.in_proj_bias"),
                               nullptr, ws.qkv, M, 3 * D, D, ACT_NONE, D, qscale, s)) return rc;
    if (int rc = launch_attention(pf, ws.qkv, ws.att, lengths, nseq, B, S, D, H, nullptr, nullptr, s)) return rc;
    if (int rc = launch_linear(pf, ws.att, D, m->L(l, "self_attn.out_proj.weight"), m->L(l, "self_attn.out_proj.bias"),
                               ws.tok, ws.tok, M, D, D, ACT_NONE, 0, 1.f, s)) return rc;
    if (int rc = launch_layernorm(pf, ws.tok, m->L(l, "norm1.weight"), m->L(l, "norm1.bias"), M, D, nullptr, nullptr, s)) return rc;
    if (int rc = launch_linear(pf, ws.tok, D, m->L(l, "linear1.weight"), m->L(l, "linear1.bias"), nullptr, ws.ffn, M,
                               FF, D, ACT_GELU, 0, 1.f, s)) return rc;
    if (int rc = launch_linear(pf, ws.ffn, FF, m->L(l, "linear2.weight"), m->L(l, "linear2.bias"), ws.tok, ws.tok, M,
                               D, FF, ACT_NONE, 0, 1.f, s)) return rc;
    if (int rc = launch_layernorm(pf, ws.tok, m->L(l, "norm2.weight"), m->L(l, "norm2.bias"), M, D, nullptr, nullptr, s)) return rc;
  }
  return 0;
}

int launch_outproj_finish(mdm_model* m, const float* out_tok, int nseq, int B, int S, int T, const float* scale, int mode, float* out,
                          float* x0_out, const float* x_t, NoiseSource noise, const unsigned char* inpaint_mask,
                          const float* inpaint_motion, StepCoefs co, hipStream_t s) {
  MDM_LAUNCH(outproj_finish_kernel, dim3((T + 31) / 32, (m->jf + 31) / 32, mode == 1 ? B : nseq), dim3(256), 0, s, out_tok,
             m->jf_out, S, T, m->jf, B, scale, mode, out, x0_out, x_t, noise, inpaint_mask, inpaint_motion, co);
  return rt_launch_status();
}

int outproj_x3(mdm_model* m, const Workspace& ws, int nseq, int B, int T, const float* scale, int mode, float* out,
               float* x0_out, const float* x_t, NoiseSource noise, const unsigned char* inpaint_mask,
               const float* inpaint_motion, StepCoefs co, hipStream_t s) {
  const int D = m->cfg.latent_dim, S = T + 1, ldo = m->jf_out;
  float* out_tok = ws.qkv;
  ProfScope ps(&m->prof, MDM_PROF_OUTPROJ, 2.0 * nseq * T * (double)D * m->jf, s);
  if (m->lnfold && (S <= X3_TM || use_small_gemm(m, nseq, S))) {
    X3Call c = enc_ln_call(m, nseq, S);
    c.kind = X3K_FOLD_F32; c.prof_cat = MDM_PROF_OUTPROJ;
    c.a = X3Operand{ws.tokh, ws.tokl}; c.w = m->out_planes_f; c.bias = m->b_out; c.out = out_tok; c.N = ldo; c.K = D;
    c.astat = ws.stat2; c.colsum = m->c_out;
    if (int rc = launch_x3_ln(c, s)) return rc;
  } else if (int rc = launch_linear_x3(nullptr, X3Operand{ws.tokh, ws.tokl}, m->out_planes, m->out_bias_pad, nullptr, out_tok,
                                       nullptr, nullptr, nseq * S, ldo, D, ACT_NONE, 0, 1.f, S, s)) return rc;
  return launch_outproj_finish(m, out_tok, nseq, B, S, T, scale, mode, out, x0_out, x_t, noise, inpaint_mask, inpaint_motion, co, s);
}

}
```

motion-diffusion-model_amd/csrc/gemm_x3.h:

```cpp
#pragma once
#include "attention_x3.h"
#include "common.h"
#include "gemm_f32.h"

namespace mdm {

constexpr int X3_TM = 224, X3_BK = 32;
__host__ __device__ constexpr int x3_swz(int q) { return (((q ^ (q >> 1)) & 1) << 1) | (q >> 1); }
static_assert(x3_swz(0) == 0 && x3_swz(1) == 2 && x3_swz(2) == 3 && x3_swz(3) == 1, "A-stage swizzle permutation");
constexpr int X3_NWAVE = 8;
constexpr int X3_TN = 32 * X3_NWAVE;
constexpr int X3_MSUB = X3_TM / 32;
constexpr int X3_A_BYTES = X3_TM * X3_BK * 2;
constexpr int X3_A_STAGE = 2 * X3_A_BYTES;
constexpr int X3_A_RING = 2;
constexpr int X3_PIPE_RING = 4;
constexpr int X3M_WAIT_WS = 7, X3M_WAIT_MID = 11;
constexpr int x3_patch_base(int ring) { return ring * X3_A_STAGE; }
constexpr int X3_PATCH_BYTES = 8 * 32 * 4;
constexpr int X3_TAB_BYTES = X3_TM * 8;
constexpr int x3_tab_base(int ring) { return x3_patch_base(ring) + X3_NWAVE * X3_PATCH_BYTES; }
constexpr int X3_RAW_BYTES = 7 * 1024;
constexpr int x3_raw_base(int ring) { return x3_tab_base(ring) + 2 * X3_TAB_BYTES; }
constexpr int x3_part_base(int ring) { return x3_raw_base(ring) + 2 * X3_RAW_BYTES; }
constexpr int X3_CVEC_BYTES = 4 * 1024;
constexpr int x3_cvec_base(bool ln, int ring) { return ln ? x3_part_base(ring) + X3_NWAVE * X3_TAB_BYTES : x3_tab_base(ring); }
constexpr int x3_lds_bytes(bool ln, int ring) { return x3_cvec_base(ln, ring) + 2 * X3_CVEC_BYTES; }
static_assert(x3_lds_bytes(false, X3_A_RING) == 73728 && x3_lds_bytes(true, X3_A_RING) == 105984, "LDS of the step-synchronous form");
static_assert(x3_lds_bytes(false, X3_PIPE_RING) == 131072 && x3_lds_bytes(true, X3_PIPE_RING) == 163328, "LDS of the pipelined form");
constexpr int X3_A_GROUPS = X3_A_STAGE / 1024;
constexpr int X3_A_PIECES = (X3_A_GROUPS + X3_NWAVE - 1) / X3_NWAVE;

struct X3Operand {
  const p16_t* hi;
  const p16_t* lo;
};
struct X3Weights {
  const p16_t* hi;
  const p16_t* lo;
};
inline size_t x3_packed_weight_elems(int N, int K) { return (size_t)((N + 31) / 32 * 32) * K; }

struct X3Epilogue {
  float* out;
  const float* bias;
  const float* res;
  const p16_t* resh;
  const p16_t* resl;
  p16_t* oh;
  p16_t* ol;
  int ld;
  int scale_cols;
  float col_scale;
  QkvPlanes qkv;
  int S, D;
  const float* astat;
  const float* colsum;
  const float* rstat;
  const float* rgamma;
  const float* rbeta;
  float* ostat;
  int stat_parts;
  float inv_dim;
  int emb_T, emb_B, emb_nbranch;
  float acc_scale = kX3AccScale;
  int stat_cols = 256;
  int pair_B = 0;
};

constexpr bool x3_has_col_scale(int act, int res) { return act == 0 && (res == 0 || res == 1); }

__device__ __forceinline__ float gelu_erf_fast(float x) {
  const float z = fabsf(x) * 0.70710678118654752440f;
#ifdef MDM_EMU
  const float t = 1.0f / (1.0f + 0.3275911f * z);
#else
  const float t = __builtin_amdgcn_rcpf(1.0f + 0.3275911f * z);
#endif
  float p = 1.061405429f;
  p = p * t - 1.453152027f;
  p = p * t + 1.421413741f;
  p = p * t - 0.284496736f;
  p = p * t + 0.254829592f;
#ifdef MDM_EMU
  const float erfc_z = p * t * expf(-z * z);
#else
  const float erfc_z = p * t * __expf(-z * z);
#endif
  const float erf_abs = 1.0f - erfc_z;
  return 0.5f * x * (1.0f + copysignf(erf_abs, x));
}

__global__ __launch_bounds__(256) void pack_weight_planes_kernel(const float* __restrict__ w, p16_t* __restrict__ hi,
                                                                 p16_t* __restrict__ lo, int N, int K, int* overflow) {
  const int npad = (N + 31) / 32 * 32, k8n = K / 8;
  const size_t total = (size_t)npad * k8n;
  for (size_t i = (size_t)blockIdx.x * blockDim.x + threadIdx.x; i < total; i += (size_t)gridDim.x * blockDim.x) {
    const int n = (int)(i / k8n), k8 = (int)(i - (size_t)n * k8n);
    float v[8];
#pragma unroll
    for (int j = 0; j < 8; ++j) v[j] = (n < N) ? w[(size_t)n * K + 8 * k8 + j] * kX3WeightScale : 0.f;
    p16x8 h8, l8;
    split8(v, h8, l8);
    if (overflow != nullptr) {
      bool bad = false;
#pragma unroll
      for (int j = 0; j < 8; ++j) {
        const float back = p16_to_f32((p16_t)h8[j]);
        bad = bad || !(fabsf(back) <= 3.0e38f);
      }
      if (bad) *overflow = 1;
    }
    const int kstep = k8 >> 1, half = k8 & 1, lane = (n & 31) + 32 * half;
    const size_t o = (((size_t)(n >> 5) * (K / 16) + kstep) * 64 + lane) * 8;
    *reinterpret_cast<p16x8*>(hi + o) = h8;
    *reinterpret_cast<p16x8*>(lo + o) = l8;
  }
}

constexpr int x3_res_rounds(int t, bool t16) { return (t16 && t == X3_MSUB - 1) ? 2 : 4; }
constexpr int x3_res_younger_rounds(int t, int rr, bool t16) {
  int n = 0;
  for (int q = t + 1; q <= t + rr - 1 && q < X3_MSUB; ++q) n += x3_res_rounds(q, t16);
  return n;
}

struct X3Cursor {
  int v;
  int k;
  uint32_t off[X3_A_PIECES];
};

enum : unsigned {
  X3_OUT_F32 = 1u << 0,
  X3_OUT_PLANES = 1u << 1,
  X3_OUT_QKV = 1u << 2,
  X3_FOLD = 1u << 3,
  X3_OSTAT = 1u << 4,
  X3_EMBED = 1u << 5,
  X3_T16 = 1u << 6,
  X3_F6 = 1u << 7,
  X3_PIPE = 1u << 8,
  X3_PAIR = 1u << 9,
};
template <int ACT, int RES, unsigned FLAGS>
__global__ __launch_bounds__(64 * X3_NWAVE, 2) void gemm_x3_kernel(X3Operand A, X3Weights W, X3Epilogue ep, int M, int N, int K,
                                                                   int rows_per_tile, int tiles_n, int total) {
  MDM_DYN_SMEM(unsigned char, lds);
  constexpr bool OUT_F32 = (FLAGS & X3_OUT_F32) != 0, OUT_PLANES = (FLAGS & X3_OUT_PLANES) != 0, OUT_QKV = (FLAGS & X3_OUT_QKV) != 0;
  constexpr bool FOLD = (FLAGS & X3_FOLD) != 0, OSTAT = (FLAGS & X3_OSTAT) != 0, EMBED = (FLAGS & X3_EMBED) != 0;
  constexpr bool T16 = (FLAGS & X3_T16) != 0, F6 = (FLAGS & X3_F6) != 0, PIPE = (FLAGS & X3_PIPE) != 0, PAIR = (FLAGS & X3_PAIR) != 0;
  static_assert(FLAGS < (X3_PAIR << 1), "unknown flag");
  static_assert((int)OUT_F32 + (int)OUT_PLANES + (int)OUT_QKV == 1, "exactly one output form");
  static_assert(RES >= 0 && RES <= 3 && !(OUT_QKV && RES != 0), "in_proj has no residual");
  static_assert(!(FOLD && RES == 3), "one (mean, rstd) table: of the A rows or of the residual rows");
  static_assert(!OSTAT || OUT_PLANES, "row statistics are written next to the planes they describe");
  static_assert(!EMBED || (OUT_PLANES && RES == 1 && !PIPE), "InputProcess: fp32 positional rows, planes out, step-synchronous loop");
  static_assert(!PIPE || (T16 && !F6), "the pipelined k-loop exists for 208-row (T16) tiles");
  static_assert(!F6 || (!T16 && OUT_F32 && !FOLD && !OSTAT), "the f16f6 k-loop: 224-row tiles, plain fp32-out epilogues");
  static_assert(!PAIR || (PIPE && OUT_QKV && !FOLD), "the paired tile: layer 0's in_proj (no folded LayerNorm) on the pipelined loop");
  constexpr int RINGN = PIPE ? X3_PIPE_RING : X3_A_RING;
  constexpr int NT32 = T16 ? X3_MSUB - 1 : X3_MSUB;
  constexpr int NROUNDS = 4 * NT32 + (T16 ? 2 : 0);
  using Cursor = X3Cursor;

  const int tid = threadIdx.x;
  const int lane = tid & 63;
#ifdef MDM_EMU
  const int wid = tid >> 6;
#else
  const int wid = __builtin_amdgcn_readfirstlane(tid >> 6);
#endif
  const int r = lane & 31, h = lane >> 5;
  const int nk = K / X3_BK;
  const int gstride = (int)gridDim.x;

  auto tile_origin = [&](int v, int& m0, int& n0) {
    const int lid = xcd_remap(v, total);
    const int tile_m = lid / tiles_n, tile_n = lid - tile_m * tiles_n;
    m0 = tile_m * rows_per_tile;
    n0 = tile_n * X3_TN;
  };

  const int schunk = (lane & 3) ^ x3_swz((lane >> 4) & 3);
  auto aim_a = [&](Cursor& c) {
    int m0, n0;
    tile_origin(c.v, m0, n0);
#pragma unroll
    for (int i = 0; i < X3_A_PIECES; ++i) {
      const int jj = min(wid + X3_NWAVE * i, 25);
      const int q = PIPE ? (jj < 13 ? jj : jj + 1) : min(wid + X3_NWAVE * i, X3_A_GROUPS - 1);
      const int ga = (q < 14) ? q : q - 14;
      int arow = min(m0 + ga * 16 + (lane >> 2), M - 1);
      if constexpr (PAIR) {
        if (ga * 16 + (lane >> 2) == rows_per_tile) arow = m0 + M;
      }
      c.off[i] = (uint32_t)arow * (uint32_t)K + schunk * 8;
    }
  };
  auto piece_a = [&](const Cursor& c, int i, int buf) {
    if constexpr (PIPE) {
      const int j = wid + X3_NWAVE * i;
      const int q = j < 13 ? j : j + 1;
      if (j < 26) glds16(((q < 14) ? A.hi : A.lo) + c.off[i] + c.k * X3_BK, lds + buf * X3_A_STAGE + q * 1024);
    } else {
      const int q = wid + X3_NWAVE * i;
      if (q < X3_A_GROUPS && !(T16 && (q == 13 || q == 27)))
        glds16(((q < 14) ? A.hi : A.lo) + c.off[i] + c.k * X3_BK, lds + buf * X3_A_STAGE + q * 1024);
    }
  };
  auto advance_a = [&](Cursor& c) {
    if (++c.k == nk) {
      c.k = 0;
      if (c.v + gstride < total) { c.v += gstride; aim_a(c); }
    }
  };

  const size_t wk16 = (size_t)(K / 16);
  auto load_w = [&](int v, int k, p16x8 (&fh)[2], p16x8 (&fl)[2]) {
    int m0, n0;
    tile_origin(v, m0, n0);
    const size_t nb = (size_t)((n0 >> 5) + wid);
    const size_t o = ((nb * wk16 + 2 * (size_t)k) * 64 + lane) * 8;
    fh[0] = *reinterpret_cast<const p16x8*>(W.hi + o);
    fl[0] = *reinterpret_cast<const p16x8*>(W.lo + o);
    fh[1] = *reinterpret_cast<const p16x8*>(W.hi + o + 512);
    fl[1] = *reinterpret_cast<const p16x8*>(W.lo + o + 512);
  };

  const int sw = x3_swz((r >> 2) & 3);
  const int fa = r * 64;
  const int r16 = lane & 15, g16 = lane >> 4;
  const int fa16 = (192 + r16) * 64 + ((g16 ^ x3_swz((r16 >> 2) & 3)) * 16);
#ifndef MDM_EMU
  const uint32_t lds_base = lds_addr_of(lds);
#endif

  int v = (int)blockIdx.x;
  if (v >= total) return;
  Cursor ca{v, 0, {}};
  aim_a(ca);
  int wv = v, wkk = 0;

  auto stats_dma = [&](int m0s, int par) {
    const float* st = FOLD ? ep.astat : ep.rstat;
    const int npieces = (X3_TM * ep.stat_parts * 8 + 1023) / 1024;
    for (int pc = wid; pc < npieces; pc += X3_NWAVE) {
      const long long total_f = (long long)M * ep.stat_parts * 2;
      long long fo = (long long)m0s * ep.stat_parts * 2 + 4LL * (64 * pc + lane);
      if (fo >= total_f) fo = 0;
      glds16(st + fo, lds + x3_raw_base(RINGN) + par * X3_RAW_BYTES + pc * 1024);
    }
  };
  constexpr bool LN_ANY = FOLD || OSTAT || RES == 3;
  auto cvec_dma = [&](int n0c, int par) {
    const float* src = nullptr;
    if (wid == 0) src = ep.bias;
    if constexpr (FOLD) { if (wid == 1) src = ep.colsum; }
    if constexpr (RES == 3) { if (wid == 2) src = ep.rgamma; if (wid == 3) src = ep.rbeta; }
    if (src != nullptr) glds16(src + min(n0c + 4 * lane, N - 4), lds + x3_cvec_base(LN_ANY, RINGN) + par * X3_CVEC_BYTES + wid * 1024);
  };
  {
    int m0f, n0f;
    tile_origin(v, m0f, n0f);
    if constexpr (FOLD || RES == 3) stats_dma(m0f, 0);
    cvec_dma(n0f, 0);
  }
  p16x8 wh[2], wl[2], wnh[2], wnl[2];
  p16x8 wsh[4] = {}, wsl[4] = {};
  uint32_t wso = 0;
  uint32_t wtile = 0;
  auto aim_w_tile = [&]() {
    int m0w, n0w;
    tile_origin(wv, m0w, n0w);
    wtile = (uint32_t)((n0w >> 5) + wid) * (uint32_t)wk16 * 512u;
  };
  const uint32_t lane_wo = (uint32_t)((lane >> 5) * 512 + ((lane & 15) + 32 * ((lane >> 4) & 1)) * 8);
  auto aim_w = [&]() { wso = wtile + (uint32_t)wkk * 1024u + lane_wo; };
  auto advance_w = [&]() {
    if (++wkk == nk) {
      wkk = 0;
      if (wv + gstride < total) { wv += gstride; aim_w_tile(); }
    }
  };
  auto load_w_half = [&](int c, auto q_tag) __attribute__((always_inline)) {
    constexpr int q = decltype(q_tag)::value;
    const uint32_t o = wso + 128u * (uint32_t)c;
    gload16_refill(wsh[q], W.hi + o);
    gload16_refill(wsl[q], W.lo + o);
  };
  auto wait_all_slots = [&]() __attribute__((always_inline)) {
    vmem_wait<0>(wsh[0], wsl[0], wsh[1], wsl[1], wsh[2], wsl[2], wsh[3], wsl[3]);
  };
  int gs = 0;
  if constexpr (PIPE) {
#pragma unroll
    for (int st = 0; st < 3; ++st) {
#pragma unroll
      for (int i = 0; i < X3_A_PIECES; ++i) piece_a(ca, i, st);
      advance_a(ca);
    }
    aim_w_tile();
#pragma unroll
    for (int st = 0; st < 2; ++st) {
      aim_w();
      if (st == 0) { load_w_half(0, std::integral_constant<int, 0>{}); load_w_half(1, std::integral_constant<int, 1>{}); }
      else { load_w_half(0, std::integral_constant<int, 2>{}); load_w_half(1, std::integral_constant<int, 3>{}); }
      advance_w();
    }
    wait_all_slots();
    wg_barrier();
  } else {
#pragma unroll
    for (int i = 0; i < X3_A_PIECES; ++i) piece_a(ca, i, 0);
    advance_a(ca);
    load_w(wv, wkk, wh, wl);
    wait_vmem_all();
    wg_barrier();
  }

  int abuf = 0;
  int tile_parity = 0;
  for (; v < total; v += gstride, tile_parity ^= 1) {
    int m0, n0;
    tile_origin(v, m0, n0);
    f32x16 acc[NT32];
    f32x4 acc16[2];
    constexpr int NS16 = 2 * X3_MSUB - 1;
    f32x4 accm_[PIPE ? NS16 : 1][2];
    if constexpr (PIPE) {
#pragma unroll
      for (int s = 0; s < NS16; ++s) accm_[s][0] = accm_[s][1] = f32x4{0.f, 0.f, 0.f, 0.f};
    } else {
#pragma unroll
      for (int t = 0; t < NT32; ++t)
#pragma unroll
        for (int e = 0; e < 16; ++e) acc[t][e] = 0.f;
      acc16[0] = f32x4{0.f, 0.f, 0.f, 0.f};
      acc16[1] = f32x4{0.f, 0.f, 0.f, 0.f};
    }
    const int ncol0 = n0 + wid * 32;
    const float* const cvec = reinterpret_cast<const float*>(lds + x3_cvec_base(LN_ANY, RINGN) + tile_parity * X3_CVEC_BYTES);
    const int kt_cvec = nk > 1 ? 1 : 0;
    if (nk == 1) wg_barrier();
    constexpr bool LN_TABS = FOLD || RES == 3;
    float2* const stab = reinterpret_cast<float2*>(lds + x3_tab_base(RINGN) + tile_parity * X3_TAB_BYTES);
    if constexpr (LN_TABS) {
      if (tid < X3_TM) {
        int m0t, n0t;
        tile_origin(v, m0t, n0t);
        const bool pad_row = m0t + tid >= M;
        const float* sraw = reinterpret_cast<const float*>(lds + x3_raw_base(RINGN) + tile_parity * X3_RAW_BYTES);
        float s1 = 0.f;
        for (int p = 0; p < ep.stat_parts; ++p) s1 += sraw[(tid * ep.stat_parts + p) * 2];
        const float mean = s1 * ep.inv_dim;
        const float pcols = (float)ep.stat_cols, inv_pcols = 1.0f / pcols;
        float m2 = 0.f;
        for (int p = 0; p < ep.stat_parts; ++p) {
          const float dm = sraw[(tid * ep.stat_parts + p) * 2] * inv_pcols - mean;
          m2 += sraw[(tid * ep.stat_parts + p) * 2 + 1] + pcols * dm * dm;
        }
        const float var = m2 * ep.inv_dim;
#ifdef MDM_EMU
        stab[tid] = pad_row ? make_float2(0.f, 0.f) : make_float2(mean, 1.0f / sqrtf(var + 1e-5f));
#else
        stab[tid] = pad_row ? make_float2(0.f, 0.f) : make_float2(mean, __builtin_amdgcn_rsqf(var + 1e-5f));
#endif
      }
      if (v + gstride < total) {
        int m0n, n0n;
        tile_origin(v + gstride, m0n, n0n);
        stats_dma(m0n, tile_parity ^ 1);
      }
    }
    float2* const atab = stab;
    float2* const rtab = stab;
    if constexpr (PIPE) {
      constexpr int NE = NS16, DEPTH = 2, RING = DEPTH + 1, XB = NE / 2;
      auto slot = [](int e) constexpr { return e == NE - 1 ? RING : e % RING; };
      p16x8 ah[RING + 1] = {}, al[RING + 1] = {};
#ifndef MDM_EMU
      const uint32_t lane_a = lds_base + fa16 - 192 * 64;
#endif
      auto issue_reads = [&](auto e_tag, uint32_t stg) __attribute__((always_inline)) {
        constexpr int e = decltype(e_tag)::value;
#ifdef MDM_EMU
        lds_refill16(ah[slot(e)], lds + stg * X3_A_STAGE, fa16 - 192 * 64 + e * 1024);
        lds_refill16(al[slot(e)], lds + stg * X3_A_STAGE, X3_A_BYTES + fa16 - 192 * 64 + e * 1024);
#else
        lds_refill16<e * 1024>(ah[slot(e)], lane_a + stg * X3_A_STAGE);
        lds_refill16<X3_A_BYTES + e * 1024>(al[slot(e)], lane_a + stg * X3_A_STAGE);
#endif
      };
      auto pipe_step = [&](auto par_tag) __attribute__((always_inline)) {
        constexpr int PAR = decltype(par_tag)::value, W0 = 2 * PAR, W1 = 2 * PAR + 1;
        const uint32_t cur = (uint32_t)gs & 3u, nxt = (uint32_t)(gs + 1) & 3u, fill = (uint32_t)(gs + 3) & 3u;
        vmem_wait<X3M_WAIT_WS>(wsh[W0], wsl[W0], wsh[W1], wsl[W1]);
        static_for<NE>([&](auto e_tag) __attribute__((always_inline)) {
          constexpr int e = decltype(e_tag)::value;
          if constexpr (e + DEPTH < NE) issue_reads(std::integral_constant<int, e + DEPTH>{}, cur);
          else issue_reads(std::integral_constant<int, e + DEPTH - NE>{}, nxt);
          if constexpr (e == XB) {
            vmem_wait<X3M_WAIT_MID>(wsh[W0], wsl[W0], wsh[W1], wsl[W1]);
            sched_fence();
            wg_barrier_nodrain();
            sched_fence();
          }
          lds_wait<2 * DEPTH>(ah[slot(e)], al[slot(e)]);
          sched_fence();
#pragma unroll
          for (int c = 0; c < 2; ++c) accm_[e][c] = mfma16_p16(al[slot(e)], wsh[W0 + c], accm_[e][c]);
#pragma unroll
          for (int c = 0; c < 2; ++c) accm_[e][c] = mfma16_p16(ah[slot(e)], wsl[W0 + c], accm_[e][c]);
#pragma unroll
          for (int c = 0; c < 2; ++c) accm_[e][c] = mfma16_p16(ah[slot(e)], wsh[W0 + c], accm_[e][c]);
          sched_fence();
          if constexpr (e >= XB && e < XB + X3_A_PIECES) piece_a(ca, e - XB, (int)fill);
          sched_fence();
        });
        aim_w();
        load_w_half(0, std::integral_constant<int, W0>{});
        load_w_half(1, std::integral_constant<int, W1>{});
        advance_w();
        advance_a(ca);
        ++gs;
      };
      static_for<DEPTH>([&](auto d_tag) __attribute__((always_inline)) { issue_reads(d_tag, (uint32_t)gs & 3u); });
      for (int kt = 0; kt < nk; kt += 2) {
        pipe_step(std::integral_constant<int, 0>{});
        if (kt == 0 && v + gstride < total) {
          int m0n, n0n;
          tile_origin(v + gstride, m0n, n0n);
          cvec_dma(n0n, tile_parity ^ 1);
        }
        pipe_step(std::integral_constant<int, 1>{});
      }
      lds_wait<0>(ah[0], al[0], ah[1], al[1]);
      wait_all_slots();
    } else {
    for (int kt = 0; kt < nk; ++kt) {
      if (kt == kt_cvec && v + gstride < total) {
        int m0n, n0n;
        tile_origin(v + gstride, m0n, n0n);
        cvec_dma(n0n, tile_parity ^ 1);
      }
      if (++wkk == nk) {
        wkk = 0;
        if (wv + gstride < total) wv += gstride;
      }
      load_w(wv, wkk, wnh, wnl);
      constexpr int DEPTH = 2, RING = DEPTH + 1;
      p16x8 ah[RING], al[RING];
#ifdef MDM_EMU
      const unsigned char* sa = lds + abuf * X3_A_STAGE;
#define X3_RD_A(dst, plane, t, ks) lds_read16(dst, sa, (plane) * X3_A_BYTES + fa + (t) * 2048 + ((((ks) * 2 + h) ^ sw) * 16))
#else
      const uint32_t sa0 = lds_base + abuf * X3_A_STAGE + fa;
      const uint32_t aaddr[2] = {sa0 + ((h ^ sw) * 16), sa0 + (((2 + h) ^ sw) * 16)};
#define X3_RD_A(dst, plane, t, ks) lds_read16<(plane) * X3_A_BYTES + (t) * 2048>(dst, aaddr[ks])
#endif
      p16x8 a16h, a16l, w16h[2], w16l[2];
      if constexpr (T16) {
#ifdef MDM_EMU
        lds_read16(a16h, sa, fa16);
        lds_read16(a16l, sa, X3_A_BYTES + fa16);
#else
        const uint32_t a16addr = lds_base + abuf * X3_A_STAGE + fa16;
        lds_read16<0>(a16h, a16addr);
        lds_read16<X3_A_BYTES>(a16l, a16addr);
#endif
        w16h[0] = wh[0]; w16h[1] = wh[1];
        w16l[0] = wl[0]; w16l[1] = wl[1];
        frag32_to_frag16(w16h[0], w16h[1]);
        frag32_to_frag16(w16l[0], w16l[1]);
      }
      constexpr int NU = 2 * NT32;
      p16x8 f6_hold = {0, 0, 0, 0, 0, 0, 0, 0};
      static_for<NU + DEPTH>([&](auto u_tag) __attribute__((always_inline)) {
        constexpr int u = decltype(u_tag)::value;
        if constexpr (u < NU) {
          constexpr int ks = F6 ? (u & 1) : u / NT32, t = F6 ? (u >> 1) : u - ks * NT32;
          X3_RD_A(ah[u % RING], 0, t, ks);
          X3_RD_A(al[u % RING], 1, t, ks);
        }
        if constexpr (u >= DEPTH) {
          constexpr int uv = u - DEPTH, ks = F6 ? (uv & 1) : uv / NT32, t = F6 ? (uv >> 1) : uv - ks * NT32;
          constexpr int younger = 2 * ((NU - 1 - uv) < DEPTH ? (NU - 1 - uv) : DEPTH);
          if constexpr (T16 && uv == 0) lds_wait<younger>(ah[uv % RING], al[uv % RING], a16h, a16l);
          else lds_wait<younger>(ah[uv % RING], al[uv % RING]);
          sched_fence();
          if constexpr (F6) {
            if constexpr (ks == 0) {
              f6_hold = al[uv % RING];
              acc[t] = mfma_f16(__builtin_bit_cast(f16x8, ah[uv % RING]), __builtin_bit_cast(f16x8, wh[0]), acc[t]);
            } else {
              acc[t] = mfma_f16(__builtin_bit_cast(f16x8, ah[uv % RING]), __builtin_bit_cast(f16x8, wh[1]), acc[t]);
              const u32x4 c0 = __builtin_bit_cast(u32x4, f6_hold), c1 = __builtin_bit_cast(u32x4, al[uv % RING]);
              const u32x4 w0 = __builtin_bit_cast(u32x4, wl[0]), w1 = __builtin_bit_cast(u32x4, wl[1]);
              const i32x8 a6 = {(int)c0[0], (int)c0[1], (int)c0[2], (int)c0[3], (int)c1[0], (int)c1[1], 0, 0};
              const i32x8 w6 = {(int)w0[0], (int)w0[1], (int)w0[2], (int)w0[3], (int)w1[0], (int)w1[1], 0, 0};
              acc[t] = mfma_mx_fp6(a6, w6, acc[t], (int)c1[2], (int)w1[2]);
            }
          } else {
            acc[t] = mfma_p16(al[uv % RING], wh[ks], acc[t]);
            acc[t] = mfma_p16(ah[uv % RING], wl[ks], acc[t]);
            acc[t] = mfma_p16(ah[uv % RING], wh[ks], acc[t]);
            if constexpr (T16 && uv == 0) {
#pragma unroll
              for (int cb = 0; cb < 2; ++cb) {
                acc16[cb] = mfma16_p16(a16l, w16h[cb], acc16[cb]);
                acc16[cb] = mfma16_p16(a16h, w16l[cb], acc16[cb]);
                acc16[cb] = mfma16_p16(a16h, w16h[cb], acc16[cb]);
              }
            }
          }
          sched_fence();
          if constexpr (uv < X3_A_PIECES) piece_a(ca, uv, abuf ^ 1);
          sched_fence();
        }
      });
#undef X3_RD_A
      advance_a(ca);
      wait_vmem_all();
      wg_barrier();
      abuf ^= 1;
      wh[0] = wnh[0]; wh[1] = wnh[1]; wl[0] = wnl[0]; wl[1] = wnl[1];
    }
    }

    [&]() __attribute__((always_inline)) {
    int lane_e = lane;
#ifndef MDM_EMU
    asm volatile("" : "+v"(lane_e));
#endif
    const int r = lane_e & 31, h = lane_e >> 5, r16 = lane_e & 15, g16 = lane_e >> 4;
    const int m_end = min(M, m0 + rows_per_tile);
    float* patch = reinterpret_cast<float*>(lds + x3_patch_base(RINGN)) + wid * (X3_PATCH_BYTES / 4);
    const int prow = lane_e >> 3, pc4 = (lane_e & 7) * 4;
    const int n4 = ncol0 + pc4;
    const int cl4 = wid * 32 + pc4;
    const float4 b4 = ld4(cvec + cl4);
    constexpr bool COL_SCALE = x3_has_col_scale(ACT, RES);
    const float mult4 = (COL_SCALE && n4 < ep.scale_cols) ? ep.col_scale : 1.f;
    float4 c4 = zero4(), g4 = zero4(), be4 = zero4();
    if constexpr (FOLD) c4 = ld4(cvec + 256 + cl4);
    if constexpr (RES == 3) {
      g4 = ld4(cvec + 512 + cl4);
      be4 = ld4(cvec + 768 + cl4);
    }
    const float bias = cvec[wid * 32 + r];
    float csum = 0.f;
    if constexpr (FOLD) csum = cvec[256 + wid * 32 + r];
    const float accs = ep.acc_scale;
    const float4 bb4 = RES == 3 ? make_float4(b4.x + be4.x, b4.y + be4.y, b4.z + be4.z, b4.w + be4.w) : b4;
    auto finish4 = [&](float4 v4, float2 st) __attribute__((always_inline)) {
      v4.x *= accs; v4.y *= accs; v4.z *= accs; v4.w *= accs;
      if constexpr (FOLD) {
        v4.x = st.y * (v4.x - st.x * c4.x) + bb4.x; v4.y = st.y * (v4.y - st.x * c4.y) + bb4.y;
        v4.z = st.y * (v4.z - st.x * c4.z) + bb4.z; v4.w = st.y * (v4.w - st.x * c4.w) + bb4.w;
      } else {
        v4.x += bb4.x; v4.y += bb4.y; v4.z += bb4.z; v4.w += bb4.w;
      }
      if (ACT == ACT_GELU) { v4.x = gelu_erf_fast(v4.x); v4.y = gelu_erf_fast(v4.y); v4.z = gelu_erf_fast(v4.z); v4.w = gelu_erf_fast(v4.w); }
      else if (ACT == ACT_SILU) { v4.x = silu(v4.x); v4.y = silu(v4.y); v4.z = silu(v4.z); v4.w = silu(v4.w); }
      if constexpr (COL_SCALE) { v4.x *= mult4; v4.y *= mult4; v4.z *= mult4; v4.w *= mult4; }
      return v4;
    };
    auto row_stats = [&](auto j_tag) __attribute__((always_inline)) {
      constexpr int j = decltype(j_tag)::value;
      if constexpr (LN_TABS && j < NROUNDS) return stab[(j / 4) * 32 + 8 * (j % 4) + prow];
      else return make_float2(0.f, 1.f);
    };
    auto patch_write = [&](auto j_tag) __attribute__((always_inline)) {
      constexpr int j = decltype(j_tag)::value, t = j / 4, g = j % 4;
      if constexpr (PIPE) {
        if constexpr (j < NROUNDS) {
          if (h == j % 2) {
#pragma unroll
            for (int cb = 0; cb < 2; ++cb)
#pragma unroll
              for (int e = 0; e < 4; ++e) patch[((e + 4 * (g16 & 1)) << 5) + 16 * cb + r16] = accm_[j / 2][cb][e];
          }
        }
      } else if constexpr (j < 4 * NT32) {
#pragma unroll
        for (int e = 0; e < 4; ++e) patch[((e + 4 * h) << 5) + r] = acc[t][4 * g + e];
      } else if constexpr (T16 && j < NROUNDS) {
        if (h == g) {
#pragma unroll
          for (int cb = 0; cb < 2; ++cb)
#pragma unroll
            for (int e = 0; e < 4; ++e) patch[((e + 4 * (g16 & 1)) << 5) + 16 * cb + r16] = acc16[cb][e];
        }
      }
    };

    if (OUT_QKV) {
      const int Dm = ep.D, SPq = ep.qkv.SP, Hq = ep.qkv.H;
      int ncol_e = ncol0, m0_e = m0;
#ifndef MDM_EMU
      asm volatile("" : "+s"(ncol_e), "+s"(m0_e));
#endif
      const int which = ncol_e / Dm, hcol = ncol_e - which * Dm, head = hcol >> 7, d0 = hcol & 127;
      const size_t shq = (size_t)(m0_e / rows_per_tile) * Hq + head;
      if (ncol0 < N) {
        if (which == 2) {
          p16_t* vhp = ep.qkv.vh + ((shq * ep.qkv.NKT) * AX_HD + d0 + r) * 32 + 8 * h;
          p16_t* vlp = ep.qkv.vl + ((shq * ep.qkv.NKT) * AX_HD + d0 + r) * 32 + 8 * h;
          const int nkt = ep.qkv.NKT;
          if constexpr (PIPE) {
#pragma unroll
            for (int cb = 0; cb < 2; ++cb) {
              const int cl = 16 * cb + r16;
              const float b16 = cvec[wid * 32 + cl];
              const float c16 = FOLD ? cvec[256 + wid * 32 + cl] : 0.f;
              const size_t o0 = (shq * ep.qkv.NKT * AX_HD + d0 + cl) * 32 + 4 * ((g16 >> 1) + 2 * (g16 & 1));
              auto vfin = [&](float a) __attribute__((always_inline)) { return a * accs + b16; };
              float u0 = 0.f;
              size_t po = 0;
              if constexpr (PAIR) {
                const int sS = ep.S >> 4, eS = ep.S & 3;
#pragma unroll
                for (int s = 0; s < NS16; ++s) {
                  if (s == sS) {
                    const f32x4 a = accm_[s][cb];
                    u0 = vfin(eS == 0 ? a[0] : eS == 1 ? a[1] : eS == 2 ? a[2] : a[3]);
                  }
                }
                u0 = lane_bcast(u0, r16 + 16 * ((ep.S >> 2) & 3));
                po = (size_t)ep.pair_B * Hq * ep.qkv.NKT * (AX_HD * 32);
              }
#pragma unroll
              for (int s = 0; s < NS16; ++s) {
                if ((s >> 1) < nkt) {
                  float vv[4];
#pragma unroll
                  for (int e = 0; e < 4; ++e) {
                    if constexpr (FOLD) {
                      const float2 st = atab[16 * s + 4 * g16 + e];
                      vv[e] = st.y * (accm_[s][cb][e] * accs - st.x * c16) + b16;
                    } else {
                      vv[e] = vfin(accm_[s][cb][e]);
                    }
                  }
                  const size_t o = o0 + (size_t)(s >> 1) * (AX_HD * 32) + 16 * (s & 1);
                  split4_store(ep.qkv.vh + o, ep.qkv.vl + o, make_float4(vv[0], vv[1], vv[2], vv[3]));
                  if constexpr (PAIR) {
                    const float k0 = (s == 0 && g16 == 0) ? u0 : vv[0];
                    split4_store(ep.qkv.vh + po + o, ep.qkv.vl + po + o, make_float4(k0, vv[1], vv[2], vv[3]));
                  }
                }
              }
            }
          } else {
#pragma unroll
          for (int t = 0; t < NT32; ++t) {
            if (t < nkt) {
#pragma unroll
              for (int s2 = 0; s2 < 2; ++s2) {
                float vv[8];
#pragma unroll
                for (int j = 0; j < 8; ++j) {
                  if constexpr (FOLD) {
                    const float2 st = atab[32 * t + mfma_row(8 * s2 + j, h)];
                    vv[j] = st.y * (acc[t][8 * s2 + j] * accs - st.x * csum) + bias;
                  } else {
                    vv[j] = acc[t][8 * s2 + j] * accs + bias;
                  }
                }
                p16x8 vh8, vl8;
                split8(vv, vh8, vl8);
                *reinterpret_cast<p16x8*>(vhp + t * (AX_HD * 32) + 16 * s2) = vh8;
                *reinterpret_cast<p16x8*>(vlp + t * (AX_HD * 32) + 16 * s2) = vl8;
              }
            }
          }
          if constexpr (T16) {
            if (NT32 < nkt) {
#pragma unroll
              for (int cb = 0; cb < 2; ++cb) {
                const int cl = 16 * cb + r16;
                const float b16 = lane_bcast(bias, cl);
                const float c16 = FOLD ? lane_bcast(csum, cl) : 0.f;
                float vv[4];
#pragma unroll
                for (int e = 0; e < 4; ++e) {
                  if constexpr (FOLD) {
                    const float2 st = atab[192 + 4 * g16 + e];
                    vv[e] = st.y * (acc16[cb][e] * accs - st.x * c16) + b16;
                  } else {
                    vv[e] = acc16[cb][e] * accs + b16;
                  }
                }
                const size_t o = ((shq * ep.qkv.NKT + NT32) * AX_HD + d0 + cl) * 32 + 4 * ((g16 >> 1) + 2 * (g16 & 1));
                split4_store(ep.qkv.vh + o, ep.qkv.vl + o, make_float4(vv[0], vv[1], vv[2], vv[3]));
              }
            }
          }
          }
        } else {
          p16_t* dh = (which == 0 ? ep.qkv.qh : ep.qkv.kh) + shq * SPq * AX_HD + d0 + pc4;
          p16_t* dl = (which == 0 ? ep.qkv.ql : ep.qkv.kl) + shq * SPq * AX_HD + d0 + pc4;
          const int nkt = PAIR ? (ep.S + 32) / 32 : ep.qkv.NKT;
          const size_t pq = PAIR ? (size_t)ep.pair_B * Hq * SPq * AX_HD : 0;
          patch_write(std::integral_constant<int, 0>{});
          float2 st_cur = row_stats(std::integral_constant<int, 0>{});
          static_for<NROUNDS>([&](auto j_tag) __attribute__((always_inline)) {
            constexpr int j = decltype(j_tag)::value, t = j / 4, g = j % 4;
            wave_lds_fence();
            float4 v4 = ld4(&patch[prow * 32 + pc4]);
            const float2 st_next = row_stats(std::integral_constant<int, j + 1>{});
            wave_lds_fence();
            patch_write(std::integral_constant<int, j + 1>{});
            const float2 st = st_cur;
            st_cur = st_next;
            if (t < nkt) {
              const int tok = 32 * t + 8 * g + prow;
              v4 = finish4(v4, st);
              if constexpr (PAIR) {
                if (tok < ep.S) split4_store(dh + tok * AX_HD, dl + tok * AX_HD, v4);
                if ((unsigned)(tok - 1) < (unsigned)ep.S) {
                  const int tok2 = tok == ep.S ? 0 : tok;
                  split4_store(dh + pq + tok2 * AX_HD, dl + pq + tok2 * AX_HD, v4);
                }
              } else {
                if (t < X3_MSUB - 1 || tok < ep.S) split4_store(dh + tok * AX_HD, dl + tok * AX_HD, v4);
              }
            }
          });
        }
      }
    } else {
      constexpr bool HAS_RES = RES != 0;
      constexpr bool RES_PLANES = RES == 2 || RES == 3;
      static_assert(!(EMBED && RES_PLANES), "the EMBED epilogue takes an fp32 residual");
      constexpr bool CLIP_OUT = OUT_PLANES && !EMBED;
      const uint32_t pitch2 = (uint32_t)ep.ld * 2u;
      const uint32_t voff0 = n4 < N ? ((uint32_t)prow * (uint32_t)ep.ld + (uint32_t)n4) * 2u : CLIP_OFF;
      ClipWin w_oh = {}, w_ol = {}, w_rh = {}, w_rl = {};
      {
        int m0_e = m0;
#ifndef MDM_EMU
        asm volatile("" : "+s"(m0_e));
#endif
        const size_t row0 = (size_t)m0_e * ep.ld;
        if constexpr (CLIP_OUT) {
          const uint32_t bytes = (uint32_t)(m_end - m0_e) * pitch2;
          w_oh = clip_win(ep.oh + row0, bytes);
          w_ol = clip_win(ep.ol + row0, bytes);
        }
        if constexpr (RES_PLANES) {
          const uint32_t bytes = (uint32_t)min(M - m0_e, X3_TM) * pitch2;
          w_rh = clip_win(ep.resh + row0, bytes);
          w_rl = clip_win(ep.resl + row0, bytes);
        }
      }
      constexpr int RR = (RES == 3) ? 2 : 3;
      f32x4 rr[RR][4];
      u32x2 rh[RR][4], rl[RR][4];
      auto res_issue = [&](auto t_tag) __attribute__((always_inline)) {
        constexpr int t = decltype(t_tag)::value;
        if constexpr (HAS_RES && t < X3_MSUB) {
#pragma unroll
          for (int g = 0; g < x3_res_rounds(t, T16); ++g) {
            if constexpr (RES == 1) {
              const int m = min(m0 + t * 32 + 8 * g + prow, M - 1);
              const size_t o = (size_t)(EMBED ? 1 + m % ep.emb_T : m) * ep.ld + (n4 < N ? n4 : 0);
              gload16_async(rr[t % RR][g], ep.res + o);
            } else {
              const uint32_t o = voff0 + (uint32_t)(t * 32 + 8 * g) * pitch2;
              clip_load8_async(rh[t % RR][g], w_rh, o);
              clip_load8_async(rl[t % RR][g], w_rl, o);
            }
          }
        }
      };
      auto res_wait = [&](auto t_tag) __attribute__((always_inline)) {
        constexpr int t = decltype(t_tag)::value;
        constexpr int ahead = x3_res_younger_rounds(t, RR, T16);
        if constexpr (RES == 1) {
          vmem_wait<ahead>(rr[t % RR][0], rr[t % RR][1], rr[t % RR][2], rr[t % RR][3]);
        } else if constexpr (RES_PLANES) {
          vmem_wait<2 * ahead>(rh[t % RR][0], rh[t % RR][1], rh[t % RR][2], rh[t % RR][3], rl[t % RR][0], rl[t % RR][1],
                               rl[t % RR][2], rl[t % RR][3]);
        }
      };
      res_issue(std::integral_constant<int, 0>{});
      if constexpr (RR == 3) res_issue(std::integral_constant<int, 1>{});
      float2* part = reinterpret_cast<float2*>(lds + x3_part_base(RINGN)) + wid * X3_TM;
      patch_write(std::integral_constant<int, 0>{});
      float2 st_cur = row_stats(std::integral_constant<int, 0>{});
      static_for<NROUNDS>([&](auto j_tag) __attribute__((always_inline)) {
        constexpr int j = decltype(j_tag)::value, t = j / 4, g = j % 4;
        if constexpr (HAS_RES && g == 0) {
          res_issue(std::integral_constant<int, t + RR - 1>{});
          res_wait(std::integral_constant<int, t>{});
        }
        wave_lds_fence();
        float4 v4 = ld4(&patch[prow * 32 + pc4]);
        const float2 st_next = row_stats(std::integral_constant<int, j + 1>{});
        wave_lds_fence();
        patch_write(std::integral_constant<int, j + 1>{});
        const float2 st = st_cur;
        st_cur = st_next;
        const int row_in_tile = t * 32 + 8 * g + prow;
        v4 = finish4(v4, st);
        if constexpr (RES == 1) {
          const f32x4 q4 = rr[t % RR][g];
          v4.x += q4[0]; v4.y += q4[1]; v4.z += q4[2]; v4.w += q4[3];
        } else if constexpr (RES_PLANES) {
          const u32x2 a = rh[t % RR][g], b = rl[t % RR][g];
          const float c0 = RES == 3 ? -st.x : 0.f;
          const float d0 = f16_half_plus<0>(b[0], f16_half_plus<0>(a[0], c0));
          const float d1 = f16_half_plus<1>(b[0], f16_half_plus<1>(a[0], c0));
          const float d2 = f16_half_plus<0>(b[1], f16_half_plus<0>(a[1], c0));
          const float d3 = f16_half_plus<1>(b[1], f16_half_plus<1>(a[1], c0));
          if constexpr (RES == 3) {
            v4.x = fmaf(d0, st.y * g4.x, v4.x); v4.y = fmaf(d1, st.y * g4.y, v4.y);
            v4.z = fmaf(d2, st.y * g4.z, v4.z); v4.w = fmaf(d3, st.y * g4.w, v4.w);
          } else {
            v4.x += d0; v4.y += d1; v4.z += d2; v4.w += d3;
          }
        }
        if constexpr (OSTAT) {
          const float s1 = sum_lanes8((v4.x + v4.y) + (v4.z + v4.w));
          const float mw = s1 * (1.0f / 32.0f);
          const float dx = v4.x - mw, dy = v4.y - mw, dz = v4.z - mw, dw = v4.w - mw;
          const float m2 = sum_lanes8((dx * dx + dy * dy) + (dz * dz + dw * dw));
          if ((lane_e & 7) == 0) part[row_in_tile] = make_float2(s1, m2);
        }
        if constexpr (CLIP_OUT) split4_store_clip(w_oh, w_ol, voff0 + (uint32_t)(t * 32 + 8 * g) * pitch2, v4);
        if constexpr (EMBED || OUT_F32) {
          const int m = m0 + row_in_tile;
          if (m < m_end && n4 < N) {
            if constexpr (EMBED) {
              const int bb = m / ep.emb_T, tt = m - bb * ep.emb_T;
              for (int br = 0; br < ep.emb_nbranch; ++br) {
                const size_t o = ((size_t)(br * ep.emb_B + bb) * (ep.emb_T + 1) + 1 + tt) * ep.ld + n4;
                split4_store(ep.oh + o, ep.ol + o, v4);
              }
            } else {
              st4(ep.out + (size_t)m * ep.ld + n4, v4);
            }
          }
        }
      });
    }
    }();
    if constexpr (OSTAT && !OUT_QKV) {
        const int m_end = min(M, m0 + rows_per_tile);
        wg_barrier();
        if (tid < X3_TM && m0 + tid < m_end) {
          const float2* pp = reinterpret_cast<const float2*>(lds + x3_part_base(RINGN));
          float s1 = 0.f;
#pragma unroll
          for (int w8 = 0; w8 < X3_NWAVE; ++w8) s1 += pp[w8 * X3_TM + tid].x;
          const float mt = s1 * (1.0f / X3_TN);
          float m2 = 0.f;
#pragma unroll
          for (int w8 = 0; w8 < X3_NWAVE; ++w8) {
            const float2 v = pp[w8 * X3_TM + tid];
            const float dm = v.x * (1.0f / 32.0f) - mt;
            m2 += v.y + 32.0f * dm * dm;
          }
          *reinterpret_cast<float2*>(ep.ostat + ((size_t)(m0 + tid) * tiles_n + n0 / X3_TN) * 2) = make_float2(s1, m2);
        }
      }
  }
  wait_vmem_all();
}

#ifndef MDM_X3_KERNEL_ONLY
inline int x3_rows_per_tile(int M, int seq_len) {
  if (seq_len > 0 && seq_len <= X3_TM && M % seq_len == 0) return (X3_TM / seq_len) * seq_len;
  return X3_TM;
}

inline int x3_grid_limit() {
#ifdef MDM_EMU
  return 3;
#else
  static int cus_of[kMaxDevices] = {};
  const int dev = rt_device_ordinal();
  int& cus = cus_of[dev];
  if (cus == 0) {
    hipDeviceProp_t prop;
    if (hipGetDeviceProperties(&prop, dev) == hipSuccess) cus = prop.multiProcessorCount;
    if (cus <= 0) cus = 256;
  }
  const int wgs = cus / 8 * 8;
  return wgs > 0 ? wgs : 8;
#endif
}

template <int ACT, int RES, unsigned FLAGS>
inline int launch_gemm_x3_w(const X3Operand& A, const X3Weights& W, const X3Epilogue& ep, int M, int N, int K,
                                int rpt, hipStream_t stream) {
  constexpr bool T16 = (FLAGS & X3_T16) != 0, PIPE = (FLAGS & X3_PIPE) != 0, PAIR = (FLAGS & X3_PAIR) != 0;
  constexpr bool LN = (FLAGS & (X3_FOLD | X3_OSTAT)) != 0 || RES == 3;
  constexpr int RINGN = PIPE ? X3_PIPE_RING : X3_A_RING;
  const int tiles_m = (M + rpt - 1) / rpt, tiles_n = (N + X3_TN - 1) / X3_TN;
  const int total = tiles_m * tiles_n;
  auto kfn = &gemm_x3_kernel<ACT, RES, FLAGS>;
  if (T16 && rpt > X3_TM - 16) return -2;
  if (PAIR && (rpt + 1 > X3_TM - 16 || ep.pair_B < 1 || M != ep.pair_B * rpt)) return -2;
  if (PIPE && (K / X3_BK) % 2 != 0) return -2;
  if (!x3_has_col_scale(ACT, RES) && ep.scale_cols > 0) return -2;
#ifndef MDM_EMU
  {
    static bool configured[kMaxDevices] = {};
    if (const int rc = rt_dyn_lds_once(kfn, x3_lds_bytes(LN, RINGN), configured, stream)) return rc;
  }
#endif
  const int grid = std::min(total, x3_grid_limit());
  MDM_LAUNCH(kfn, dim3(grid), dim3(64 * X3_NWAVE), x3_lds_bytes(LN, RINGN), stream, A, W, ep, M, N, K, rpt, tiles_n, total);
  return 0;
}

enum X3Kind : int {
  X3K_IN_PROJ_FOLD = 0,
  X3K_OUT_PROJ_L0 = 1,
  X3K_OUT_LN_RES = 2,
  X3K_LINEAR1_GELU = 3,
  X3K_FOLD_F32 = 4,
  X3K_EMBED = 5,
  X3K_IN_PROJ_PLAIN = 6,
};
template <unsigned TILE>
inline int launch_gemm_x3_ln_t(X3Kind kind, const X3Operand& A, const X3Weights& W, const X3Epilogue& ep, int M, int N,
                                   int K, int rpt, hipStream_t s) {
  switch (kind) {
    case X3K_IN_PROJ_FOLD: return launch_gemm_x3_w<ACT_NONE,  0, X3_OUT_QKV | X3_FOLD | TILE>(A, W, ep, M, N, K, rpt, s);
    case X3K_OUT_PROJ_L0: return launch_gemm_x3_w<ACT_NONE,  2, X3_OUT_PLANES | X3_OSTAT | TILE>(A, W, ep, M, N, K, rpt, s);
    case X3K_OUT_LN_RES: return launch_gemm_x3_w<ACT_NONE,  3, X3_OUT_PLANES | X3_OSTAT | TILE>(A, W, ep, M, N, K, rpt, s);
    case X3K_LINEAR1_GELU: return launch_gemm_x3_w<ACT_GELU,  0, X3_OUT_PLANES | X3_FOLD | TILE>(A, W, ep, M, N, K, rpt, s);
    case X3K_FOLD_F32: return launch_gemm_x3_w<ACT_NONE,  0, X3_OUT_F32 | X3_FOLD | TILE>(A, W, ep, M, N, K, rpt, s);
    case X3K_EMBED:
      return launch_gemm_x3_w<ACT_NONE,  1, X3_OUT_PLANES | X3_EMBED | (TILE & X3_T16)>(A, W, ep, M, N, K, rpt, s);
    default: return -2;
  }
}
inline int launch_gemm_x3_ln(X3Kind kind, const X3Operand& A, const X3Weights& W, const X3Epilogue& ep, int M, int N,
                                 int K, int rpt, hipStream_t s) {
  if (rpt <= X3_TM - 16) {
    if (kind != X3K_EMBED && (K / X3_BK) % 2 == 0) return launch_gemm_x3_ln_t<X3_T16 | X3_PIPE>(kind, A, W, ep, M, N, K, rpt, s);
    return launch_gemm_x3_ln_t<X3_T16>(kind, A, W, ep, M, N, K, rpt, s);
  }
  return launch_gemm_x3_ln_t<0u>(kind, A, W, ep, M, N, K, rpt, s);
}

inline int launch_gemm_x3(const X3Operand& A, const X3Weights& W, const X3Epilogue& ep, int M, int N, int K, int act,
                              int seq_len, hipStream_t s) {
  const bool res = ep.res != nullptr, f32 = ep.out != nullptr, pl = ep.oh != nullptr;
  const int rpt = x3_rows_per_tile(M, seq_len);
  if (ep.resh != nullptr) {
    if (act == ACT_NONE && !res && f32 && !pl) return launch_gemm_x3_w<ACT_NONE,  2, X3_OUT_F32>(A, W, ep, M, N, K, rpt, s);
    return -2;
  }
  if (act == ACT_NONE && !res && f32 && !pl) return launch_gemm_x3_w<ACT_NONE,  0, X3_OUT_F32>(A, W, ep, M, N, K, rpt, s);
  if (act == ACT_NONE && res && f32 && !pl) return launch_gemm_x3_w<ACT_NONE,  1, X3_OUT_F32>(A, W, ep, M, N, K, rpt, s);
  if (act == ACT_GELU && !res && !f32 && pl) return launch_gemm_x3_w<ACT_GELU,  0, X3_OUT_PLANES>(A, W, ep, M, N, K, rpt, s);
  if (act == ACT_GELU && !res && f32 && !pl) return launch_gemm_x3_w<ACT_GELU,  0, X3_OUT_F32>(A, W, ep, M, N, K, rpt, s);
  if (act == ACT_GELU && res && f32 && !pl) return launch_gemm_x3_w<ACT_GELU,  1, X3_OUT_F32>(A, W, ep, M, N, K, rpt, s);
  if (act == ACT_SILU && !res && f32 && !pl) return launch_gemm_x3_w<ACT_SILU,  0, X3_OUT_F32>(A, W, ep, M, N, K, rpt, s);
  return -2;
}

#ifdef MDM_PROBES
inline int launch_gemm_f16f6(const X3Operand& A, const X3Weights& W, const X3Epilogue& ep, int M, int N, int K, int act,
                             hipStream_t s) {
  const bool res = ep.res != nullptr;
  if (act == ACT_NONE && !res) return launch_gemm_x3_w<ACT_NONE,  0, X3_OUT_F32 | X3_F6>(A, W, ep, M, N, K, X3_TM, s);
  if (act == ACT_NONE && res) return launch_gemm_x3_w<ACT_NONE,  1, X3_OUT_F32 | X3_F6>(A, W, ep, M, N, K, X3_TM, s);
  if (act == ACT_GELU && !res) return launch_gemm_x3_w<ACT_GELU,  0, X3_OUT_F32 | X3_F6>(A, W, ep, M, N, K, X3_TM, s);
  return -2;
}
#endif

inline bool x3_qkv_pairs(int S, int D) { return S + 1 <= X3_TM - 16 && (D / X3_BK) % 2 == 0; }

inline int launch_gemm_x3_qkv(const X3Operand& A, const X3Weights& W, const X3Epilogue& ep, int nseq, int S, int D,
                                  hipStream_t s, int pair_B = 0) {
  if (S > X3_TM) return -2;
  if (pair_B > 0) {
    if (nseq != 2 * pair_B || !x3_qkv_pairs(S, D)) return -2;
    X3Epilogue ep2 = ep;
    ep2.pair_B = pair_B;
    return launch_gemm_x3_w<ACT_NONE,  0, X3_OUT_QKV | X3_T16 | X3_PIPE | X3_PAIR>(A, W, ep2, pair_B * S, 3 * D, D, S, s);
  }
  if (S <= X3_TM - 16) {
    if ((D / X3_BK) % 2 == 0) return launch_gemm_x3_w<ACT_NONE,  0, X3_OUT_QKV | X3_T16 | X3_PIPE>(A, W, ep, nseq * S, 3 * D, D, S, s);
    return launch_gemm_x3_w<ACT_NONE,  0, X3_OUT_QKV | X3_T16>(A, W, ep, nseq * S, 3 * D, D, S, s);
  }
  return launch_gemm_x3_w<ACT_NONE,  0, X3_OUT_QKV>(A, W, ep, nseq * S, 3 * D, D, S, s);
}

#endif

}
```

motion-diffusion-model_amd/csrc/mdm_api.hip:

```cpp
#include "../../include/mdm_hip.h"
#ifdef MDM_PROBES
#include "../../include/mdm_hip_probe.h"
#endif

#include <algorithm>
#include <cmath>
#include <cstdio>
#include <cstring>
#include <map>
#include <mutex>
#include <new>
#include <string>
#include <vector>

#include "attention_x3.h"
#include "attention_long.h"
#include "attention_f32.h"
#include "common.h"
#include "elementwise.h"
#include "gemm_f32.h"
#include "gemm_x3.h"
#include "gemm_x3s.h"
#include "xattn_block.h"
#include "selfattn_block.h"
#ifdef MDM_PROBES
#include "../../lab/csrc_probe/gemm_f16f6.h"
#endif
#include "motion_recover.h"
#include "smpl_joints.h"
#include "smpl_mesh.h"
#include "evaluator.h"
#include "text_encoder.h"
#include "clip_text.h"
#include "stgcn.h"
#include "gru_recogniser.h"

using namespace mdm;

#include "api_runtime.h"
#include "api_launch.h"
#include "encoder.h"

extern "C" {

int mdm_abi_version(void) { return MDM_ABI_VERSION; }

const char* mdm_build_info(void) {
  return "slp="
#ifdef MDM_NO_SLP
         "off"
#else
         "on"
#endif
         ";probes="
#ifdef MDM_PROBES
         "1"
#else
         "0"
#endif
         ";emu="
#ifdef MDM_EMU
         "1"
#else
         "0"
#endif
         ";planes=f16";
}
const char* mdm_last_error(void) { return g_err.c_str(); }

int mdm_create(const mdm_config_t* cfg, mdm_model_t** out) {
  if (cfg == nullptr || out == nullptr) return fail(MDM_EINVAL, "mdm_create: null argument");
  const int D = cfg->latent_dim, H = cfg->num_heads;
  if (D <= 0 || D % 256 != 0 || D > 1024) return fail(MDM_EUNSUPPORTED, "latent_dim must be 256, 512, 768 or 1024");
  if (H <= 0 || D != H * ATT_HD) return fail(MDM_EUNSUPPORTED, "latent_dim / num_heads must be 128");
  if (cfg->ff_size <= 0 || cfg->ff_size % 32) return fail(MDM_EUNSUPPORTED, "ff_size must be a positive multiple of 32");
  if (cfg->clip_dim <= 0 || cfg->clip_dim % 4) return fail(MDM_EUNSUPPORTED, "clip_dim must be a positive multiple of 4");
  if (cfg->njoints <= 0 || cfg->nfeats <= 0 || cfg->num_layers <= 0 || cfg->max_len < 2)
    return fail(MDM_EINVAL, "mdm_create: non-positive dimension");
  if (cfg->arch != MDM_ARCH_TRANS_ENC && cfg->arch != MDM_ARCH_TRANS_DEC) return fail(MDM_EUNSUPPORTED, "arch must be trans_enc or trans_dec");
  if (cfg->context_len < 0 || (cfg->arch == MDM_ARCH_TRANS_ENC && cfg->context_len != 0))
    return fail(MDM_EUNSUPPORTED, "context_len (prefix completion) belongs to the trans_dec (DiP) configuration");
  mdm_model* m = new (std::nothrow) mdm_model();
  if (m == nullptr) return fail(MDM_EINVAL, "out of host memory");
  m->cfg = *cfg;
  m->jf = cfg->njoints * cfg->nfeats;
  m->jf_pad = (m->jf + 3) / 4 * 4;
  m->jf_out = m->jf_pad;
  m->jf_k = (m->jf + 31) / 32 * 32;
  const int64_t d = D, ff = cfg->ff_size, jf = m->jf;
  auto& e = m->expect;
  e["input_process.poseEmbedding.weight"] = d * jf;
  e["input_process.poseEmbedding.bias"] = d;
  for (int l = 0; l < cfg->num_layers; ++l) {
    const std::string p = (cfg->arch == MDM_ARCH_TRANS_DEC ? "seqTransDecoder.layers." : "seqTransEncoder.layers.") +
                          std::to_string(l) + ".";
    if (cfg->arch == MDM_ARCH_TRANS_DEC) {
      e[p + "multihead_attn.in_proj_weight"] = 3 * d * d;
      e[p + "multihead_attn.in_proj_bias"] = 3 * d;
      e[p + "multihead_attn.out_proj.weight"] = d * d;
      e[p + "multihead_attn.out_proj.bias"] = d;
      e[p + "norm3.weight"] = d;
      e[p + "norm3.bias"] = d;
    }
    e[p + "self_attn.in_proj_weight"] = 3 * d * d;
    e[p + "self_attn.in_proj_bias"] = 3 * d;
    e[p + "self_attn.out_proj.weight"] = d * d;
    e[p + "self_attn.out_proj.bias"] = d;
    e[p + "linear1.weight"] = ff * d;
    e[p + "linear1.bias"] = ff;
    e[p + "linear2.weight"] = d * ff;
    e[p + "linear2.bias"] = d;
    e[p + "norm1.weight"] = d;
    e[p + "norm1.bias"] = d;
    e[p + "norm2.weight"] = d;
    e[p + "norm2.bias"] = d;
  }
  e["embed_timestep.time_embed.0.weight"] = d * d;
  e["embed_timestep.time_embed.0.bias"] = d;
  e["embed_timestep.time_embed.2.weight"] = d * d;
  e["embed_timestep.time_embed.2.bias"] = d;
  e["embed_text.weight"] = d * cfg->clip_dim;
  e["embed_text.bias"] = d;
  e["output_process.poseFinal.weight"] = jf * d;
  e["output_process.poseFinal.bias"] = jf;
  e["sequence_pos_encoder.pe"] = (int64_t)cfg->max_len * d;
  *out = m;
  return MDM_OK;
}

void mdm_destroy(mdm_model_t* m) { delete m; }

int mdm_set_option(mdm_model_t* m, int32_t key, int32_t value) {
  if (m == nullptr) return fail(MDM_EINVAL, "mdm_set_option: null model");
  switch (key) {
    case MDM_OPT_SMALL_GEMM_MAX_SEQS:
      if (value < 0) return fail(MDM_EINVAL, "mdm_set_option: MDM_OPT_SMALL_GEMM_MAX_SEQS must be >= 0");
      m->x3s.max_seqs = value;
      return MDM_OK;
    case MDM_OPT_SMALL_GEMM_ROW_TILES:
      if (value < 0 || value > 2) return fail(MDM_EINVAL, "mdm_set_option: MDM_OPT_SMALL_GEMM_ROW_TILES must be 0 (by size), 1 or 2");
      m->x3s.row_tiles = value;
      return MDM_OK;
    case MDM_OPT_DEC_FUSED_XATTN:
      if (value < 0 || value > 3) return fail(MDM_EINVAL, "mdm_set_option: MDM_OPT_DEC_FUSED_XATTN must be 0, 1, 2 or 3");
      m->fused_xattn = value;
      return MDM_OK;
    case MDM_OPT_DEC_FUSED_SELFATTN:
      if (value != 0 && value != 1) return fail(MDM_EINVAL, "mdm_set_option: MDM_OPT_DEC_FUSED_SELFATTN must be 0 or 1");
      m->fused_selfattn = value != 0;
      return MDM_OK;
    case MDM_OPT_ATTN_DIRECT_OUT:
      if (value != 0 && value != 1) return fail(MDM_EINVAL, "mdm_set_option: MDM_OPT_ATTN_DIRECT_OUT must be 0 or 1");
      m->attn_direct = value != 0;
      return MDM_OK;
    case MDM_OPT_ATTN_WIDE:
      if (value != 0 && value != 1) return fail(MDM_EINVAL, "mdm_set_option: MDM_OPT_ATTN_WIDE must be 0 or 1");
      m->attn_wide = value != 0;
      return MDM_OK;
    case MDM_OPT_DEC_TIME_TOKEN:
      if (value != 0 && value != 1) return fail(MDM_EINVAL, "mdm_set_option: MDM_OPT_DEC_TIME_TOKEN must be 0 or 1");
      if (value == 1 && (m->cfg.arch != MDM_ARCH_TRANS_DEC || m->cfg.context_len != 1))
        return fail(MDM_EINVAL, "mdm_set_option: MDM_OPT_DEC_TIME_TOKEN needs a trans_dec model created with context_len = 1 (the class-token row)");
      m->dec_time_token = value != 0;
      return MDM_OK;
    case MDM_OPT_ENC_SHARED_LAYER0:
      if (value != 0 && value != 1) return fail(MDM_EINVAL, "mdm_set_option: MDM_OPT_ENC_SHARED_LAYER0 must be 0 or 1");
      m->enc_shared_l0 = value != 0;
      return MDM_OK;
    default:
      return fail(MDM_EINVAL, "mdm_set_option: unknown key " + std::to_string(key));
  }
}

int mdm_set_time_add(mdm_model_t* m, const float* add_dev, int32_t B) {
  if (m == nullptr) return fail(MDM_EINVAL, "mdm_set_time_add: null model");
  if (add_dev != nullptr && B <= 0) return fail(MDM_EINVAL, "mdm_set_time_add: B must be >= 1");
  m->time_add_next = add_dev;
  m->time_add_B = add_dev != nullptr ? B : 0;
  return MDM_OK;
}

int mdm_get_option(const mdm_model_t* m, int32_t key, int32_t* value) {
  if (m == nullptr || value == nullptr) return fail(MDM_EINVAL, "mdm_get_option: null argument");
  switch (key) {
    case MDM_OPT_SMALL_GEMM_MAX_SEQS: *value = m->x3s.max_seqs; return MDM_OK;
    case MDM_OPT_SMALL_GEMM_ROW_TILES: *value = m->x3s.row_tiles; return MDM_OK;
    case MDM_OPT_DEC_FUSED_XATTN: *value = m->fused_xattn; return MDM_OK;
    case MDM_OPT_DEC_FUSED_SELFATTN: *value = m->fused_selfattn ? 1 : 0; return MDM_OK;
    case MDM_OPT_ATTN_DIRECT_OUT: *value = m->attn_direct ? 1 : 0; return MDM_OK;
    case MDM_OPT_ATTN_WIDE: *value = m->attn_wide ? 1 : 0; return MDM_OK;
    case MDM_OPT_DEC_TIME_TOKEN: *value = m->dec_time_token ? 1 : 0; return MDM_OK;
    case MDM_OPT_ENC_SHARED_LAYER0: *value = m->enc_shared_l0 ? 1 : 0; return MDM_OK;
    default: return fail(MDM_EINVAL, "mdm_get_option: unknown key " + std::to_string(key));
  }
}

int mdm_set_weight(mdm_model_t* m, const char* name, const float* dev_ptr, int64_t numel) {
  if (m == nullptr || name == nullptr || dev_ptr == nullptr) return fail(MDM_EINVAL, "mdm_set_weight: null argument");
  auto it = m->expect.find(name);
  if (it == m->expect.end()) return fail(MDM_EINVAL, std::string("unexpected state-dict key: ") + name);
  if (it->second != numel)
    return fail(MDM_EINVAL, std::string("size mismatch for ") + name + ": expected " + std::to_string(it->second) +
                                " elements, got " + std::to_string(numel));
  if ((reinterpret_cast<uintptr_t>(dev_ptr) & 15) != 0) return fail(MDM_EINVAL, std::string(name) + ": pointer must be 16-byte aligned");
  m->w[name] = dev_ptr;
  m->prepared = false;
  return MDM_OK;
}

size_t mdm_const_bytes(const mdm_model_t* m) {
  if (m == nullptr) return 0;
  const size_t D = m->cfg.latent_dim;
  const size_t FF = m->cfg.ff_size;
  if (m->cfg.arch == MDM_ARCH_TRANS_DEC) {
    const size_t fold = align_up(3 * D * D * 4, 256) + align_up(D * D * 4, 256) + align_up(FF * D * 4, 256) +
                        2 * (align_up(3 * D * 4, 256) + align_up(D * 4, 256) + align_up(FF * 4, 256));
    const size_t planes = align_up(3 * D * D * 4, 256) + 3 * align_up(D * D * 4, 256) + 2 * align_up(FF * D * 4, 256);
    const size_t outp = align_up((size_t)m->jf * D * 4, 256) + 2 * align_up((size_t)32 * ((m->jf_out + 31) / 32) * 4, 256) +
                        align_up(x3_packed_weight_elems(m->jf, (int)D) * 4, 256);
    const size_t kv_all = align_up((size_t)m->cfg.num_layers * 2 * D * D * 4, 256) + align_up((size_t)m->cfg.num_layers * 2 * D * 4, 256);
    return 256  + align_up(D * m->jf_pad * sizeof(float), 256) +
           2 * align_up((size_t)m->cfg.max_len * D * sizeof(float), 256) + (size_t)m->cfg.num_layers * (fold + planes) + outp + kv_all;
  }
  const size_t per_layer = align_up(3 * D * D * 4, 256) + align_up(D * D * 4, 256) + 2 * align_up(FF * D * 4, 256);
  return 256  + align_up(D * m->jf_pad * sizeof(float), 256) +
         2 * align_up((size_t)m->cfg.max_len * D * sizeof(float), 256) + (size_t)m->cfg.num_layers * per_layer + align_up(x3_packed_weight_elems(m->jf, (int)D) * 4, 256) +
         align_up((size_t)m->jf_out * sizeof(float), 256) +
         (size_t)m->cfg.num_layers * (align_up(3 * D * D * 4, 256) + align_up(FF * D * 4, 256) +
                                      2 * align_up(3 * D * 4, 256) + 2 * align_up(FF * 4, 256)) +
         align_up(x3_packed_weight_elems(m->jf, (int)D) * 4, 256) + 2 * align_up((size_t)32 * ((m->jf_out + 31) / 32) * 4, 256) +
         align_up(std::max<size_t>(3 * D, FF) * D * 4, 256) + align_up((size_t)D * m->jf_k * 4, 256);
}

int mdm_prepare(mdm_model_t* m, void* const_ws, size_t const_ws_bytes, void* stream) {
  ChainGuard chain_guard(stream);
  if (m == nullptr || const_ws == nullptr) return fail(MDM_EINVAL, "mdm_prepare: null argument");
  for (const auto& kv : m->expect)
    if (m->w.find(kv.first) == m->w.end()) return fail(MDM_ESTATE, "missing weight: " + kv.first);
  if (const_ws_bytes < mdm_const_bytes(m)) return fail(MDM_ENOSPC, "mdm_prepare: const workspace too small");
  hipStream_t s = static_cast<hipStream_t>(stream);
  const int D = m->cfg.latent_dim, R = m->cfg.max_len;
  char* base = static_cast<char*>(const_ws);
  m->range_flag = reinterpret_cast<int*>(base);
  base += 256;
#ifdef MDM_EMU
  *m->range_flag = 0;
#else
  if (hipMemsetAsync(m->range_flag, 0, 4, s) != hipSuccess) return fail(MDM_EHIP, "mdm_prepare: hipMemsetAsync failed");
#endif
  m->w_in_pad = reinterpret_cast<float*>(base);
  base += align_up((size_t)D * m->jf_pad * sizeof(float), 256);
  m->time_table = reinterpret_cast<float*>(base);
  base += align_up((size_t)R * D * sizeof(float), 256);
  float* hidden = reinterpret_cast<float*>(base);
  MDM_LAUNCH(pad_rows_kernel, dim3(256), dim3(256), 0, s, m->w_in_pad, m->W("input_process.poseEmbedding.weight"), D,
             m->jf, m->jf_pad);
  if (int rc = rt_launch_status()) return rc;
  if (int rc = launch_linear(nullptr, m->W("sequence_pos_encoder.pe"), D, m->W("embed_timestep.time_embed.0.weight"),
                             m->W("embed_timestep.time_embed.0.bias"), nullptr, hidden, R, D, D, ACT_SILU, 0, 1.f, s))
    return rc;
  if (int rc = launch_linear(nullptr, hidden, D, m->W("embed_timestep.time_embed.2.weight"),
                             m->W("embed_timestep.time_embed.2.bias"), nullptr, m->time_table, R, D, D, ACT_NONE, 0,
                             1.f, s))
    return rc;
  if (m->cfg.arch == MDM_ARCH_TRANS_DEC) {
    base += align_up((size_t)R * D * sizeof(float), 256);
    const int L = m->cfg.num_layers, FFd = m->cfg.ff_size;
    auto take = [&](size_t n) { float* p = reinterpret_cast<float*>(base); base += align_up(n * 4, 256); return p; };
    auto fold_one = [&](const float* w, const float* bias, const float* gamma, const float* beta, int N, float*& wf, float*& cvec,
                        float*& bvec) -> int {
      wf = take((size_t)N * D);
      cvec = take(N);
      bvec = take(N);
      MDM_LAUNCH(fold_layernorm_kernel, dim3((N + 3) / 4), dim3(256), 0, s, w, gamma, beta, bias, wf, cvec, bvec, N, D, N);
      return rt_launch_status();
    };
    m->dec_fold.assign(L, mdm_model::DecFold{});
    for (int l = 0; l < L; ++l) {
      mdm_model::DecFold& F = m->dec_fold[l];
      if (l >= 1)
        if (int rc = fold_one(m->L(l, "self_attn.in_proj_weight"), m->L(l, "self_attn.in_proj_bias"), m->L(l - 1, "norm3.weight"),
                              m->L(l - 1, "norm3.bias"), 3 * D, F.w_in, F.c_in, F.b_in)) return rc;
      if (int rc = fold_one(m->L(l, "multihead_attn.in_proj_weight"), m->L(l, "multihead_attn.in_proj_bias"), m->L(l, "norm1.weight"),
                            m->L(l, "norm1.bias"), D, F.w_q, F.c_q, F.b_q)) return rc;
      if (int rc = fold_one(m->L(l, "linear1.weight"), m->L(l, "linear1.bias"), m->L(l, "norm2.weight"), m->L(l, "norm2.bias"),
                            FFd, F.w_1, F.c_1, F.b_1)) return rc;
    }
    auto make_planes = [&](const float* src, int N, int K, X3Weights& op) -> int {
      const size_t n = x3_packed_weight_elems(N, K);
      p16_t* hi = reinterpret_cast<p16_t*>(base);
      base += align_up(n * 4, 256);
      op = X3Weights{hi, hi + n};
      return launch_pack_weights(src, hi, hi + n, N, K, s, m->range_flag);
    };
    m->dec_planes.assign(L, mdm_model::DecPlanes{});
    for (int l = 0; l < L; ++l) {
      const mdm_model::DecFold& F = m->dec_fold[l];
      mdm_model::DecPlanes& P = m->dec_planes[l];
      if (int rc = make_planes(l >= 1 ? F.w_in : m->L(l, "self_attn.in_proj_weight"), 3 * D, D, P.in_proj)) return rc;
      if (int rc = make_planes(m->L(l, "self_attn.out_proj.weight"), D, D, P.out_proj)) return rc;
      if (int rc = make_planes(F.w_q, D, D, P.q)) return rc;
      if (int rc = make_planes(m->L(l, "multihead_attn.out_proj.weight"), D, D, P.out_proj2)) return rc;
      if (int rc = make_planes(F.w_1, FFd, D, P.linear1)) return rc;
      if (int rc = make_planes(m->L(l, "linear2.weight"), D, FFd, P.linear2)) return rc;
    }
    {
      const int jf32 = (m->jf_out + 31) / 32 * 32;
      float* wf = take((size_t)m->jf * D);
      m->c_out = take(jf32);
      m->b_out = take(jf32);
      MDM_LAUNCH(fold_layernorm_kernel, dim3((jf32 + 3) / 4), dim3(256), 0, s, m->W("output_process.poseFinal.weight"),
                 m->L(L - 1, "norm3.weight"), m->L(L - 1, "norm3.bias"), m->W("output_process.poseFinal.bias"), wf, m->c_out,
                 m->b_out, m->jf, D, jf32);
      if (int rc = rt_launch_status()) return rc;
      if (int rc = make_planes(wf, m->jf, D, m->out_planes_f)) return rc;
    }
    m->wkv_all = take((size_t)L * 2 * D * D);
    m->bkv_all = take((size_t)L * 2 * D);
    for (int l = 0; l < L; ++l) {
      if (int rc = rt_copy(m->wkv_all + (size_t)l * 2 * D * D, m->L(l, "multihead_attn.in_proj_weight") + (size_t)D * D,
                           (size_t)2 * D * D * sizeof(float), s)) return rc;
      if (int rc = rt_copy(m->bkv_all + (size_t)l * 2 * D, m->L(l, "multihead_attn.in_proj_bias") + D, (size_t)2 * D * sizeof(float), s)) return rc;
    }
    if ((size_t)(base - static_cast<char*>(const_ws)) > const_ws_bytes) return fail(MDM_ENOSPC, "mdm_prepare: const workspace too small");
    m->prepared = true;
    return MDM_OK;
  }
  base += align_up((size_t)R * D * sizeof(float), 256);
  const size_t FF = m->cfg.ff_size;
  m->planes.assign(m->cfg.num_layers, mdm_model::LayerPlanes{});
  auto make_planes = [&](const float* src, int N, int K, X3Weights& op) -> int {
    const size_t n = x3_packed_weight_elems(N, K);
    p16_t* hi = reinterpret_cast<p16_t*>(base);
    p16_t* lo = hi + n;
    base += align_up(n * 4, 256);
    op = X3Weights{hi, lo};
    return launch_pack_weights(src, hi, lo, N, K, s, m->range_flag);
  };
  for (int l = 0; l < m->cfg.num_layers; ++l) {
    if (int rc = make_planes(m->L(l, "self_attn.in_proj_weight"), 3 * D, D, m->planes[l].in_proj)) return rc;
    if (int rc = make_planes(m->L(l, "self_attn.out_proj.weight"), D, D, m->planes[l].out_proj)) return rc;
    if (int rc = make_planes(m->L(l, "linear1.weight"), (int)FF, D, m->planes[l].linear1)) return rc;
    if (int rc = make_planes(m->L(l, "linear2.weight"), D, (int)FF, m->planes[l].linear2)) return rc;
  }
  if (int rc = make_planes(m->W("output_process.poseFinal.weight"), m->jf, D, m->out_planes)) return rc;
  m->out_bias_pad = reinterpret_cast<float*>(base);
  base += align_up((size_t)m->jf_out * sizeof(float), 256);
  MDM_LAUNCH(pad_rows_kernel, dim3(1), dim3(256), 0, s, m->out_bias_pad, m->W("output_process.poseFinal.bias"), 1, m->jf,
             m->jf_out);
  if (int rc = rt_launch_status()) return rc;
  {
    const int L = m->cfg.num_layers;
    float* scratch_w = reinterpret_cast<float*>(base);
    base += align_up(std::max<size_t>(3 * (size_t)D, FF) * D * 4, 256);
    auto take_vec = [&](size_t n) { float* p = reinterpret_cast<float*>(base); base += align_up(n * 4, 256); return p; };
    auto fold_one = [&](const float* w, const float* bias, const float* gamma, const float* beta, int N, int Npad,
                        X3Weights& op, float*& cvec, float*& bvec) -> int {
      cvec = take_vec(Npad);
      bvec = take_vec(Npad);
      MDM_LAUNCH(fold_layernorm_kernel, dim3((Npad + 3) / 4), dim3(256), 0, s, w, gamma, beta, bias, scratch_w, cvec, bvec,
                 N, D, Npad);
      if (int rc = rt_launch_status()) return rc;
      return make_planes(scratch_w, N, D, op);
    };
    m->fold.assign(L, mdm_model::LayerFold{});
    for (int l = 0; l < L; ++l) {
      mdm_model::LayerFold& F = m->fold[l];
      if (l >= 1) {
        if (int rc = fold_one(m->L(l, "self_attn.in_proj_weight"), m->L(l, "self_attn.in_proj_bias"),
                              m->L(l - 1, "norm2.weight"), m->L(l - 1, "norm2.bias"), 3 * D, 3 * D, F.in_proj, F.c_qkv, F.b_qkv)) return rc;
      }
      if (int rc = fold_one(m->L(l, "linear1.weight"), m->L(l, "linear1.bias"), m->L(l, "norm1.weight"),
                            m->L(l, "norm1.bias"), (int)FF, (int)FF, F.linear1, F.c_1, F.b_1)) return rc;
    }
    const int jf32 = (m->jf_out + 31) / 32 * 32;
    if (int rc = fold_one(m->W("output_process.poseFinal.weight"), m->W("output_process.poseFinal.bias"),
                          m->L(L - 1, "norm2.weight"), m->L(L - 1, "norm2.bias"), m->jf, jf32, m->out_planes_f, m->c_out,
                          m->b_out)) return rc;
    MDM_LAUNCH(pad_rows_kernel, dim3(256), dim3(256), 0, s, scratch_w, m->W("input_process.poseEmbedding.weight"), D, m->jf,
               m->jf_k);
    if (int rc = rt_launch_status()) return rc;
    {
      const size_t n = x3_packed_weight_elems(D, m->jf_k);
      p16_t* hi = reinterpret_cast<p16_t*>(base);
      base += align_up(n * 4, 256);
      m->in_planes = X3Weights{hi, hi + n};
      if (int rc = launch_pack_weights(scratch_w, hi, hi + n, D, m->jf_k, s, m->range_flag)) return rc;
    }
    m->lnfold = true;
  }
  m->prepared = true;
  return MDM_OK;
}

int mdm_weights_in_range(mdm_model_t* m, int32_t* in_range, void* stream) {
  if (int rc = check_ready(m)) return rc;
  if (in_range == nullptr) return fail(MDM_EINVAL, "mdm_weights_in_range: null argument");
  int flag = 0;
#ifdef MDM_EMU
  (void)stream;
  flag = *m->range_flag;
#else
  hipStream_t s = static_cast<hipStream_t>(stream);
  if (hipMemcpyAsync(&flag, m->range_flag, 4, hipMemcpyDeviceToHost, s) != hipSuccess || hipStreamSynchronize(s) != hipSuccess)
    return fail(MDM_EHIP, "mdm_weights_in_range: reading the flag back failed");
#endif
  *in_range = flag == 0 ? 1 : 0;
  return MDM_OK;
}

int mdm_set_precision(mdm_model_t* m, int32_t mode) {
  if (m == nullptr) return fail(MDM_EINVAL, "mdm_set_precision: null model");
  if (mode != MDM_PREC_F32 && mode != MDM_PREC_F16X3) return fail(MDM_EINVAL, "mdm_set_precision: unknown mode");
  if (mode == MDM_PREC_F16X3 && (m->cfg.latent_dim % X3_BK != 0 || m->cfg.ff_size % X3_BK != 0))
    return fail(MDM_EUNSUPPORTED, "f16x3 needs latent_dim and ff_size to be multiples of 32");
  m->precision = mode;
  return MDM_OK;
}

size_t mdm_workspace_bytes(const mdm_model_t* m, int32_t nseq, int32_t nframes) {
  if (m == nullptr || nseq <= 0 || nframes <= 0) return 0;
  return carve(m, nseq, nframes, nullptr).bytes;
}

int mdm_forward(mdm_model_t* m, const float* x, const int64_t* timesteps, const float* text_embed,
                const int32_t* lengths, int32_t B, int32_t T, int32_t branches, float* out, void* ws_dev,
                size_t ws_bytes, void* stream) {
  ChainGuard chain_guard(stream);
  if (int rc = check_ready(m)) return rc;
  TimeAddScope time_add(m, B, "mdm_forward");
  if (time_add.rc) return time_add.rc;
  if (m->cfg.arch != MDM_ARCH_TRANS_ENC) return fail(MDM_ESTATE, "mdm_forward: trans_dec models go through mdm_forward_dec");
  if (x == nullptr || timesteps == nullptr || out == nullptr || ws_dev == nullptr) return fail(MDM_EINVAL, "mdm_forward: null pointer");
  if (B <= 0 || T <= 0 || T + 1 > m->cfg.max_len) return fail(MDM_EINVAL, "mdm_forward: need B >= 1 and 1 <= T < the positional table's length");
  if (branches < 0 || branches > 2) return fail(MDM_EINVAL, "mdm_forward: bad branches");
  if (branches != MDM_BRANCH_UNCOND && text_embed == nullptr) return fail(MDM_EINVAL, "mdm_forward: text_embed required");
  hipStream_t s = static_cast<hipStream_t>(stream);
  const int nbranch = (branches == MDM_BRANCH_BOTH) ? 2 : 1;
  const int nseq = nbranch * B, S = T + 1, D = m->cfg.latent_dim;
  Workspace ws = carve(m, nseq, T, ws_dev);
  if (ws_bytes < ws.bytes) return fail(MDM_ENOSPC, "mdm_forward: workspace too small");
  const int* len = m->cfg.mask_frames ? lengths : nullptr;
  if (branches != MDM_BRANCH_UNCOND)
    if (int rc = launch_linear(nullptr, text_embed, m->cfg.clip_dim, m->W("embed_text.weight"), m->W("embed_text.bias"), nullptr,
                               ws.cond, B, D, m->cfg.clip_dim, ACT_NONE, 0, 1.f, s)) return rc;
  const int uncond_from = (branches == MDM_BRANCH_UNCOND) ? 0 : 1;
  if (int rc = embed_tokens(m, ws, x, reinterpret_cast<const long long*>(timesteps), 0, ws.cond, B, T, nbranch,
                            uncond_from, s)) return rc;
  if (int rc = encoder(m, ws, nseq, B, S, len, s)) return rc;
  if (m->precision == MDM_PREC_F16X3)
    return outproj_x3(m, ws, nseq, B, T, nullptr, 0, out, nullptr, nullptr, NoiseSource{}, nullptr, nullptr, StepCoefs{}, s);
  RowMajorLoader al{m->W("output_process.poseFinal.weight"), D, m->jf, D};
  CfgTokenLoader bl{ws.tok, nullptr, nseq, T, S, D, nseq * T};
  OutProjEpilogue ep{};
  ep.bias = m->W("output_process.poseFinal.bias");
  ep.out = out;
  ep.T = T; ep.JF = m->jf; ep.mode = 0;
  ProfScope ps(&m->prof, MDM_PROF_OUTPROJ, 2.0 * nseq * T * (double)D * m->jf, s);
  launch_gemm_f32(al, bl, ep, m->jf, nseq * T, D, s);
  return rt_launch_status();
}

#include "decoder.h"

size_t mdm_workspace_bytes_dec(const mdm_model_t* m, int32_t nseq, int32_t pred_len, int32_t ntok) {
  if (m == nullptr || nseq <= 0 || pred_len <= 0 || ntok <= 0) return 0;
  return carve_dec(m, nseq, m->cfg.context_len + pred_len, ntok, nseq, nullptr).bytes;
}

size_t mdm_workspace_bytes_dec_loop(const mdm_model_t* m, int32_t nseq, int32_t pred_len, int32_t ntok, int32_t nsteps) {
  if (m == nullptr || nseq <= 0 || pred_len <= 0 || ntok <= 0 || nsteps <= 0) return 0;
  return carve_dec(m, nseq, m->cfg.context_len + pred_len, ntok, nseq, nullptr, nsteps, pred_len).bytes;
}

int mdm_forward_dec(mdm_model_t* m, const float* x, const float* prefix, const int64_t* timesteps, const float* text_tokens,
                    const int32_t* text_lengths, const int32_t* lengths, int32_t B, int32_t pred_len, int32_t ntok,
                    int32_t branches, float* out, void* ws_dev, size_t ws_bytes, void* stream) {
  ChainGuard chain_guard(stream);
  if (int rc = check_ready(m)) return rc;
  TimeAddScope time_add(m, B, "mdm_forward_dec");
  if (time_add.rc) return time_add.rc;
  if (x == nullptr || timesteps == nullptr || out == nullptr || ws_dev == nullptr || text_lengths == nullptr)
    return fail(MDM_EINVAL, "mdm_forward_dec: null pointer");
  if (int rc = check_dec_shapes(m, "mdm_forward_dec", prefix, B, pred_len, ntok)) return rc;
  if (branches < 0 || branches > 2) return fail(MDM_EINVAL, "mdm_forward_dec: bad branches");
  if (branches != MDM_BRANCH_UNCOND && text_tokens == nullptr) return fail(MDM_EINVAL, "mdm_forward_dec: text tokens required");
  const int nseq = ((branches == MDM_BRANCH_BOTH) ? 2 : 1) * B;
  DecWorkspace ws = carve_dec(m, nseq, m->cfg.context_len + pred_len, ntok, B, ws_dev);
  if (ws_bytes < ws.bytes) return fail(MDM_ENOSPC, "mdm_forward_dec: workspace too small");
  return decoder_pass(m, ws, x, prefix, timesteps, text_tokens, text_lengths, lengths, B, pred_len, ntok, branches, out,
                      static_cast<hipStream_t>(stream), DecHoist{});
}

int mdm_sampler_step(const float* x_t, const float* out_cond, const float* out_uncond, const float* scale,
                     const uint8_t* inpaint_mask, const float* inpaint_motion, const float* noise, float* x_prev,
// ... 151 lines not shown
```

motion-diffusion-model_amd/csrc/probe_api.h:

```cpp
#pragma once

extern "C" {

int mdm_debug_set(int what, int value) {
  if (what == 0 || what == 2 || what == 3 || what == 6 || what == 8)
    return fail(MDM_EINVAL, "mdm_debug_set: code " + std::to_string(what) + " belonged to a " +
                                (what == 3 ? "attention_x3.h" : "gemm_x3.h") + " experiment that has been removed");
  if (what == 1) g_x3_reuse_planes = value;
  if (what == 4) g_f6_reference = value;
  if (what == 5) g_f6_linear = value;
#ifndef MDM_EMU
  if (what == 9) { x3s_tl_target() = value; x3s_tl_count() = 0; }
  if (what == 10) { xb_tl_target() = value; xb_tl_count() = 0; }
  if (what == 11) { sb_tl_target() = value; sb_tl_count() = 0; }
#endif
  return MDM_OK;
}

int mdm_debug_get(int idx, double* out) {
#ifndef MDM_EMU
  if (idx >= 300000) {
    static std::vector<unsigned long long> tl(8 * SB_TL_WGS);
    if (idx - 300000 >= 8 * SB_TL_WGS || out == nullptr) return fail(MDM_EINVAL, "mdm_debug_get: bad timeline index");
    if (idx == 300000 && (hipDeviceSynchronize() != hipSuccess ||
                          hipMemcpyFromSymbol(tl.data(), HIP_SYMBOL(g_sb_tl), tl.size() * sizeof(unsigned long long)) != hipSuccess))
      return fail(MDM_EHIP, "mdm_debug_get: reading the timeline failed");
    *out = (double)tl[idx - 300000];
    return MDM_OK;
  }
  if (idx >= 200000) {
    static std::vector<unsigned long long> tl(8 * XB_TL_WGS);
    if (idx - 200000 >= 8 * XB_TL_WGS || out == nullptr) return fail(MDM_EINVAL, "mdm_debug_get: bad timeline index");
    if (idx == 200000 && (hipDeviceSynchronize() != hipSuccess ||
                          hipMemcpyFromSymbol(tl.data(), HIP_SYMBOL(g_xb_tl), tl.size() * sizeof(unsigned long long)) != hipSuccess))
      return fail(MDM_EHIP, "mdm_debug_get: reading the timeline failed");
    *out = (double)tl[idx - 200000];
    return MDM_OK;
  }
  if (idx >= 100) {
    static std::vector<unsigned long long> tl(4 * X3S_TL_WGS);
    if (idx - 100 >= 4 * X3S_TL_WGS || out == nullptr) return fail(MDM_EINVAL, "mdm_debug_get: bad timeline index");
    if (idx == 100 && (hipDeviceSynchronize() != hipSuccess ||
                       hipMemcpyFromSymbol(tl.data(), HIP_SYMBOL(g_x3s_tl), tl.size() * sizeof(unsigned long long)) != hipSuccess))
      return fail(MDM_EHIP, "mdm_debug_get: reading the timeline failed");
    *out = (double)tl[idx - 100];
    return MDM_OK;
  }
  return fail(MDM_EINVAL, "mdm_debug_get: not a timeline index");
#else
  if (out != nullptr) *out = 0.0;
  (void)idx;
  return MDM_OK;
#endif
}

size_t mdm_linear_f16f6_scratch_bytes(int32_t M, int32_t N, int32_t K) {
  if (M <= 0 || N <= 0 || K <= 0 || K % 32 != 0) return 0;
  return f6_plane_bytes(M, K) + 2 * align_up(x3_packed_weight_elems(N, K) * 2, 256) + f6_plane_bytes(N, K);
}

int mdm_linear_f16f6(const float* in, const float* w, const float* bias, const float* res, float* out, int32_t M,
                     int32_t N, int32_t K, int32_t act, void* scratch, size_t scratch_bytes, void* stream) {
  ChainGuard chain_guard(stream);
  if (!in || !w || !bias || !out || !scratch || M <= 0 || N <= 0 || K <= 0) return fail(MDM_EINVAL, "mdm_linear_f16f6: bad argument");
  if (K % 32 != 0) return fail(MDM_EINVAL, "mdm_linear_f16f6: K must be a multiple of 32");
  if (act != ACT_NONE && act != ACT_GELU && act != ACT_SILU) return fail(MDM_EINVAL, "mdm_linear_f16f6: bad activation");
  if (scratch_bytes < mdm_linear_f16f6_scratch_bytes(M, N, K)) return fail(MDM_ENOSPC, "mdm_linear_f16f6: scratch too small");
  hipStream_t s = static_cast<hipStream_t>(stream);
  char* base = static_cast<char*>(scratch);
  const F6Planes pa = f6_carve(base, M, K);
  p16_t* wfh = reinterpret_cast<p16_t*>(base + f6_plane_bytes(M, K));
  p16_t* wfl = reinterpret_cast<p16_t*>(base + f6_plane_bytes(M, K) + align_up(x3_packed_weight_elems(N, K) * 2, 256));
  const F6Planes pw = f6_carve(base + f6_plane_bytes(M, K) + 2 * align_up(x3_packed_weight_elems(N, K) * 2, 256), N, K);
  const bool fast = !g_f6_reference && N % 4 == 0 && ((act == ACT_NONE) || (act == ACT_GELU && res == nullptr));
  if (!g_x3_reuse_planes) {
    MDM_LAUNCH(pack_f16f6_kernel, dim3((M * (K / 32) + 255) / 256), dim3(256), 0, s, in, pa, M, K, K);
    if (int rc = rt_launch_status()) return rc;
    if (fast) {
      const int npad = (N + 31) / 32 * 32;
      MDM_LAUNCH(pack_weight_f16f6_kernel, dim3((npad * (K / 32) + 255) / 256), dim3(256), 0, s, w, wfh, wfl, N, K);
    } else {
      MDM_LAUNCH(pack_f16f6_kernel, dim3((N * (K / 32) + 255) / 256), dim3(256), 0, s, w, pw, N, K, K);
    }
    if (int rc = rt_launch_status()) return rc;
  }
  if (fast) {
    X3Call c; c.out = out; c.bias = bias; c.res_f32 = res; c.N = N;
    X3Epilogue ep = x3_epilogue(c);
    ep.acc_scale = 1.f;
    const X3Operand a{reinterpret_cast<const p16_t*>(pa.h16), reinterpret_cast<const p16_t*>(pa.rec)};
    const int rc = launch_gemm_f16f6(a, X3Weights{wfh, wfl}, ep, M, N, K, act, s);
    if (rc == -1 || rc == -3) return lds_fail(rc, "mdm_linear_f16f6");
    if (rc == -2) return fail(MDM_EUNSUPPORTED, "mdm_linear_f16f6: unsupported (activation, residual) combination");
    return rt_launch_status();
  }
  const dim3 grid((N + 31) / 32, (M + 31) / 32);
  if (act == ACT_GELU) MDM_LAUNCH(gemm_f16f6_ref_kernel<ACT_GELU>, grid, dim3(64), 0, s, pa, pw, bias, res, out, M, N, K);
  else if (act == ACT_SILU) MDM_LAUNCH(gemm_f16f6_ref_kernel<ACT_SILU>, grid, dim3(64), 0, s, pa, pw, bias, res, out, M, N, K);
  else MDM_LAUNCH(gemm_f16f6_ref_kernel<ACT_NONE>, grid, dim3(64), 0, s, pa, pw, bias, res, out, M, N, K);
  return rt_launch_status();
}

int mdm_probe_attention_x3(const float* qkv, float* out, void* out_hi, void* out_lo, const int32_t* lengths, int32_t nseq, int32_t B,
                           int32_t S, int32_t D, int32_t H, int32_t lead, int32_t wide, void* scratch, size_t scratch_bytes,
                           void* stream) {
  ChainGuard chain_guard(stream);
  if (!qkv || (!out && !out_hi) || (out_hi == nullptr) != (out_lo == nullptr) || !scratch || nseq <= 0 || B <= 0 || S <= 0 || H <= 0 ||
      lead < 0)
    return fail(MDM_EINVAL, "mdm_probe_attention_x3: bad argument");
  if (D != H * AX_HD) return fail(MDM_EUNSUPPORTED, "attention: head_dim must be 128");
  if (scratch_bytes < mdm_attention_x3_scratch_bytes(nseq, S, D)) return fail(MDM_ENOSPC, "mdm_probe_attention_x3: scratch too small");
  hipStream_t s = static_cast<hipStream_t>(stream);
  const int NKT = (S + 31) / 32, SP = 32 * NKT;
  const size_t plane = (size_t)nseq * SP * D;
  p16_t* q = static_cast<p16_t*>(scratch);
  QkvPlanes qp{q, q + plane, q + 2 * plane, q + 3 * plane, q + 4 * plane, q + 5 * plane, SP, NKT, H};
  MDM_LAUNCH(qkv_pack_kernel, dim3((int)std::min<size_t>((plane + 255) / 256, 4096)), dim3(256), 0, s, qkv, qp, nseq, S, D);
  if (int rc = rt_launch_status()) return rc;
  return launch_attention_x3(nullptr, qp, lengths, nseq, B, S, D, out, static_cast<p16_t*>(out_hi), static_cast<p16_t*>(out_lo), s, lead,
                             false, wide != 0);
}

int mdm_probe_in_proj(const float* tokens, const float* w, const float* bias, void* planes_dev, int32_t nseq, int32_t S,
                      int32_t D, void* scratch_dev, void* stream) {
  ChainGuard chain_guard(stream);
  if (!tokens || !w || !bias || !planes_dev || !scratch_dev || nseq <= 0 || S <= 0 || D % 256 != 0) return fail(MDM_EINVAL, "mdm_probe_in_proj");
  hipStream_t s = static_cast<hipStream_t>(stream);
  const size_t n = (size_t)nseq * S * D;
  p16_t* ah = static_cast<p16_t*>(scratch_dev);
  p16_t* al = ah + n;
  p16_t* wh = al + n;
  p16_t* wl = wh + (size_t)3 * D * D;
  if (!g_x3_reuse_planes) {
    if (int rc = launch_split(tokens, ah, al, n, s)) return rc;
    if (int rc = launch_pack_weights(w, wh, wl, 3 * D, D, s)) return rc;
  }
  const int H = D / AX_HD, NKT = (S + 31) / 32, SP = 32 * NKT;
  const size_t plane = (size_t)nseq * SP * D;
  p16_t* q = static_cast<p16_t*>(planes_dev);
  QkvPlanes qp{q, q + plane, q + 2 * plane, q + 3 * plane, q + 4 * plane, q + 5 * plane, SP, NKT, H};
  return launch_in_proj_x3(nullptr, X3Operand{ah, al}, X3Weights{wh, wl}, bias, qp, nseq, S, D, 0.08838834764831845f, s);
}

}
```

Baseline: 401.8 motions/s.

## Share layer-0 attention between CFG branches with a paired single-plane kernel

New measurement: 405.9 motions/s, median of 5. 1.0% higher.

```diff
diff --git a/include/mdm_hip_probe.h b/include/mdm_hip_probe.h
--- a/include/mdm_hip_probe.h
+++ b/include/mdm_hip_probe.h
@@ -22,6 +22,12 @@
                            int32_t nseq, int32_t B, int32_t S, int32_t D, int32_t H, int32_t lead, int32_t wide, void* scratch_dev,
                            size_t scratch_bytes, void* stream);
 
+int mdm_probe_attention_x3_pair(const float* qkv_dev, float* out_dev, void* out_hi_dev, void* out_lo_dev, const int32_t* lengths_dev,
+                                int32_t B, int32_t S, int32_t D, int32_t H, void* scratch_dev, size_t scratch_bytes, void* stream);
+
+int mdm_probe_in_proj_pair(const float* tokens, const float* w, const float* bias, void* planes_dev, int32_t B, int32_t S, int32_t D,
+                           int32_t one, void* scratch_dev, void* stream);
+
 #ifdef __cplusplus
 }
 #endif
diff --git a/motion-diffusion-model_amd/_native.py b/motion-diffusion-model_amd/_native.py
--- a/motion-diffusion-model_amd/_native.py
+++ b/motion-diffusion-model_amd/_native.py
@@ -27,7 +27,7 @@
     "mdm_clip_text_workspace_bytes", "mdm_clip_text_encode",
 ]
 PROBE_SYMBOLS = ["mdm_debug_set", "mdm_debug_get", "mdm_linear_f16f6", "mdm_linear_f16f6_scratch_bytes", "mdm_probe_in_proj",
-                 "mdm_probe_attention_x3"]
+                 "mdm_probe_attention_x3", "mdm_probe_attention_x3_pair", "mdm_probe_in_proj_pair"]
 ABI_VERSION = 10
 OPTIONS = {"small_gemm_max_seqs": 1, "small_gemm_row_tiles": 2, "dec_fused_xattn": 3, "dec_fused_selfattn": 4, "attn_direct_out": 5,
            "dec_time_token": 6, "enc_shared_layer0": 7, "attn_wide": 8}
@@ -203,6 +203,8 @@
             "mdm_linear_f16f6": (C.c_int, [vp, vp, vp, vp, vp, i32, i32, i32, i32, vp, sz, vp]),
             "mdm_probe_in_proj": (C.c_int, [vp, vp, vp, vp, i32, i32, i32, vp, vp]),
             "mdm_probe_attention_x3": (C.c_int, [vp, vp, vp, vp, vp, i32, i32, i32, i32, i32, i32, i32, vp, sz, vp]),
+            "mdm_probe_attention_x3_pair": (C.c_int, [vp, vp, vp, vp, vp, i32, i32, i32, i32, vp, sz, vp]),
+            "mdm_probe_in_proj_pair": (C.c_int, [vp, vp, vp, vp, i32, i32, i32, i32, vp, vp]),
         }
         self.has_probes = hasattr(lib, "mdm_debug_set")
         if self.has_probes:
diff --git a/motion-diffusion-model_amd/csrc/api_launch.h b/motion-diffusion-model_amd/csrc/api_launch.h
--- a/motion-diffusion-model_amd/csrc/api_launch.h
+++ b/motion-diffusion-model_amd/csrc/api_launch.h
@@ -144,6 +144,31 @@
   return rt_launch_status();
 }
 
+template <int NKT>
+int launch_attention_x3_pair_t(const QkvPlanes& qp, const int* lengths, int B, int S, int D, float* out, p16_t* oh, p16_t* ol,
+                               hipStream_t s, int lead) {
+  auto k = &attention_x3_kernel_pair<NKT>;
+  const size_t lds = (size_t)axw_pair_lds_bytes(NKT);
+  if (int rc = rt_allow_lds(k, lds)) return rc;
+  const int items = B * qp.H;
+  const int grid = std::min(items, x3_grid_limit());
+  MDM_LAUNCH(k, dim3(grid), dim3(AXW_THREADS), lds, s, qp, lengths, S, D, B, lead, out, oh, ol, items);
+  return rt_launch_status();
+}
+inline bool attention_x3_pairs(int S) { return S % 32 != 0 && (S + 31) / 32 >= 5 && S <= 224; }
+int launch_attention_x3_pair(Profiler* pf, const QkvPlanes& qp, const int* lengths, int B, int S, int D, float* out, p16_t* oh,
+                             p16_t* ol, hipStream_t s, int lead = 1) {
+  ProfScope ps(pf, MDM_PROF_ATTENTION, 4.0 * B * qp.H * (double)(S + 1) * (S + 1) * AX_HD, s);
+  if (D != qp.H * AX_HD) return fail(MDM_EUNSUPPORTED, "attention: head_dim must be 128");
+  if (!attention_x3_pairs(S) || lead != 1) return fail(MDM_EUNSUPPORTED, "paired attention: this length has no row S in the planes");
+  if (qp.NKT != (S + 31) / 32 || qp.SP != 32 * qp.NKT) return fail(MDM_EINVAL, "attention: the operand planes do not match the sequence length");
+  switch (qp.NKT) {
+    case 5: return launch_attention_x3_pair_t<5>(qp, lengths, B, S, D, out, oh, ol, s, lead);
+    case 6: return launch_attention_x3_pair_t<6>(qp, lengths, B, S, D, out, oh, ol, s, lead);
+    default: return launch_attention_x3_pair_t<7>(qp, lengths, B, S, D, out, oh, ol, s, lead);
+  }
+}
+
 int launch_attention_x3(Profiler* pf, const QkvPlanes& qp, const int* lengths, int nseq, int B, int S, int D, float* out,
                         p16_t* oh, p16_t* ol, hipStream_t s, int lead = 1, bool direct = false, bool wide = true) {
   ProfScope ps(pf, MDM_PROF_ATTENTION, 4.0 * nseq * qp.H * (double)S * S * AX_HD, s);
@@ -282,12 +307,12 @@
 }
 
 int launch_in_proj_x3(Profiler* pf, X3Operand a, X3Weights w, const float* bias, const QkvPlanes& qp, int nseq, int S,
-                      int D, float qscale, hipStream_t s, int pair_B = 0) {
+                      int D, float qscale, hipStream_t s, int pair_B = 0, bool pair_one = false) {
   if (D % X3_BK != 0) return fail(MDM_EINVAL, "f16x3 in_proj: latent_dim must be a multiple of 32");
   const double rows = pair_B > 0 ? (double)pair_B * (S + 1) : (double)nseq * S;
   ProfScope ps(pf, MDM_PROF_LINEAR, 2.0 * rows * 3.0 * D * (double)D, s);
   X3Call c; c.bias = bias; c.qp = &qp; c.N = 3 * D; c.S = S; c.D = D; c.scale_cols = D; c.col_scale = qscale;
-  const int rc = launch_gemm_x3_qkv(a, w, x3_epilogue(c), nseq, S, D, s, pair_B);
+  const int rc = launch_gemm_x3_qkv(a, w, x3_epilogue(c), nseq, S, D, s, pair_B, pair_one);
   if (rc == -2) return fail(MDM_EUNSUPPORTED, pair_B > 0 ? "f16x3 in_proj: the paired layer-0 launch does not cover this shape"
                                                          : "f16x3 in_proj: sequences longer than 224 tokens");
   return rt_launch_status();
diff --git a/motion-diffusion-model_amd/csrc/api_runtime.h b/motion-diffusion-model_amd/csrc/api_runtime.h
--- a/motion-diffusion-model_amd/csrc/api_runtime.h
+++ b/motion-diffusion-model_amd/csrc/api_runtime.h
@@ -155,7 +155,7 @@
   X3sOptions x3s;
   int fused_xattn = 3;
   bool fused_selfattn = true;
-  bool enc_shared_l0 = true;
+  int enc_shared_l0 = 2;
   bool attn_direct = false;
   bool attn_wide = true;
   X3Weights out_planes{nullptr, nullptr};
diff --git a/motion-diffusion-model_amd/csrc/attention_x3.h b/motion-diffusion-model_amd/csrc/attention_x3.h
--- a/motion-diffusion-model_amd/csrc/attention_x3.h
+++ b/motion-diffusion-model_amd/csrc/attention_x3.h
@@ -337,10 +337,13 @@
   return s >= AXW_RING ? s - AXW_RING : s;
 }
 
-template <int NKT>
-__global__ __launch_bounds__(AXW_THREADS) void attention_x3_kernel_wide(QkvPlanes P, const int* __restrict__ lengths, int S, int D,
-                                                                       int B, int lead, float* __restrict__ out,
-                                                                       p16_t* __restrict__ oh, p16_t* __restrict__ ol, int items) {
+constexpr int axw_pair_lds_bytes(int nkt) { return axw_lds_bytes(nkt) + 2 * AX_HD * 4; }
+static_assert(axw_pair_lds_bytes(7) <= 160 * 1024, "... and the two lead-token V rows");
+static_assert(AX_OST - 64 >= 4, "the four branch coefficients of a query ride in the pad columns of its staging row");
+
+template <int NKT, bool PAIR>
+__device__ __forceinline__ void axw_body(const QkvPlanes& P, const int* __restrict__ lengths, int S, int D, int B, int lead,
+                                         float* __restrict__ out, p16_t* __restrict__ oh, p16_t* __restrict__ ol, int items) {
   static_assert(NKT >= 5 && NKT <= 7, "one wave per query tile and at least one copy wave");
   MDM_DYN_SMEM(unsigned char, lds);
   constexpr int SP = 32 * NKT;
@@ -372,7 +375,7 @@
         unsigned char* dst = lds + slot * AX_SLOT + plane * 8192 + idx * 1024;
         if (t < NKT) {
           const int key = 32 * t + 4 * idx + (lv >> 4);
-          const p16_t* src = (plane ? P.kl : P.kh) + (sh * SP + (size_t)min(key, S - 1)) * AX_HD + (((lv & 15) ^ (key & 15)) * 8);
+          const p16_t* src = (plane ? P.kl : P.kh) + (sh * SP + (size_t)min(key, PAIR ? S : S - 1)) * AX_HD + (((lv & 15) ^ (key & 15)) * 8);
           glds16(src, dst);
         } else {
           const int d = 16 * idx + (lv >> 2);
@@ -411,10 +414,10 @@
 
   const int r = lane & 31, h = lane >> 5;
   const int qt = w;
-  const bool last_group = S > 32 * (NKT - 1) + 16;
+  const bool last_group = S + (PAIR ? 1 : 0) > 32 * (NKT - 1) + 16;
   p16x8 qh[8], ql[8];
   auto load_q = [&](size_t sh) {
-    const size_t qo = (sh * SP + min(32 * qt + r, S - 1)) * AX_HD + 8 * h;
+    const size_t qo = (sh * SP + min(32 * qt + r, PAIR ? S : S - 1)) * AX_HD + 8 * h;
 #pragma unroll
     for (int st = 0; st < 8; ++st) {
       qh[st] = *reinterpret_cast<const p16x8*>(P.qh + qo + 16 * st);
@@ -429,6 +432,7 @@
 #endif
   float* const kmask = reinterpret_cast<float*>(lds + AXW_KMASK_OFF);
   float* const so = reinterpret_cast<float*>(lds + AXW_STAGE_OFF) + w * (32 * AX_OST);
+  float* const v0 = reinterpret_cast<float*>(lds + axw_lds_bytes(NKT));
 
   for (;;) {
   const int seq = item / H, head = item - seq * H;
@@ -444,7 +448,16 @@
   if (tid < 32 * NKT) {
     const int f = max(tid - lead, 0);
     const bool ok = kbits == nullptr ? tid < nvalid : (tid < S && (tid < lead || ((kbits[f >> 5] >> (f & 31)) & 1u)));
-    kmask[tid] = ok ? 0.f : -INFINITY;
+    kmask[tid] = (ok && !(PAIR && tid == 0)) ? 0.f : -INFINITY;
+  }
+  float v0_mine = 0.f;
+  if constexpr (PAIR) {
+    if (tid < 2 * AX_HD) {
+      const int key = tid >= AX_HD ? S : 0, k16 = key & 15;
+      const int pos = 16 * ((key >> 4) & 1) + ((k16 & 3) | (((k16 >> 3) & 1) << 2) | (((k16 >> 2) & 1) << 3));
+      const size_t vo = (((size_t)item * NKT + (key >> 5)) * AX_HD + (tid & (AX_HD - 1))) * 32 + pos;
+      v0_mine = p16_to_f32(P.vh[vo]) + p16_to_f32(P.vl[vo]);
+    }
   }
 
 #ifndef MDM_EMU
@@ -464,6 +477,9 @@
     const uint32_t soff = (uint32_t)(axw_slot(first, t) * AX_SLOT);
     wg_barrier();
     if constexpr (t == NTILES - 1) load_q(has_next ? (size_t)next : (size_t)item);
+    if constexpr (PAIR && t == 1) {
+      if (tid < 2 * AX_HD) v0[tid] = v0_mine;
+    }
 
     if constexpr (t < NKT) {
       {
@@ -495,6 +511,16 @@
       }
       if constexpr (t == NKT - 1) {
         float mx = -INFINITY;
+        float s_c = -INFINITY, s_u = -INFINITY;
+        if constexpr (PAIR) {
+          if (h == 0) s_c = p[0][0];
+          const int kS = S & 31;
+#pragma unroll
+          for (int e = 0; e < 16; ++e)
+            if (8 * (e >> 2) + 4 * h + (e & 3) == kS) s_u = p[NKT - 1][e];
+          s_c = fmaxf(s_c, shfl_xor_f32(s_c, 32));
+          s_u = fmaxf(s_u, shfl_xor_f32(s_u, 32));
+        }
         {
           const float* km = kmask + 4 * h;
 #pragma unroll
@@ -509,6 +535,8 @@
             }
         }
         mx = fmaxf(mx, shfl_xor_f32(mx, 32));
+        const float m_sh = mx;
+        if constexpr (PAIR) mx = mx == -INFINITY ? 0.f : mx;
         mx -= 6.931471805599453f;
         float sum = 0.f;
 #pragma unroll
@@ -524,7 +552,20 @@
             sum += pe;
           }
         sum += shfl_xor_f32(sum, 32);
-        inv = 1.0f / sum;
+        if constexpr (PAIR) {
+          const float m_c = fmaxf(m_sh, s_c), m_u = fmaxf(m_sh, s_u);
+#ifdef MDM_EMU
+          const float a_c = expf(m_sh - m_c), e_c = expf(s_c - m_c + 6.931471805599453f);
+          const float a_u = expf(m_sh - m_u), e_u = expf(s_u - m_u + 6.931471805599453f);
+#else
+          const float a_c = __expf(m_sh - m_c), e_c = __expf(s_c - m_c + 6.931471805599453f);
+          const float a_u = __expf(m_sh - m_u), e_u = __expf(s_u - m_u + 6.931471805599453f);
+#endif
+          const float i_c = 1.0f / (a_c * sum + e_c), i_u = 1.0f / (a_u * sum + e_u);
+          st4(&so[r * AX_OST + 64], make_float4(a_c * i_c, e_c * i_c, a_u * i_u, e_u * i_u));
+        } else {
+          inv = 1.0f / sum;
+        }
       }
     } else {
       constexpr int kt = t - NKT;
@@ -588,7 +629,35 @@
 #pragma unroll
       for (int i = 0; i < 4; ++i) {
         const int row = 8 * i + (lane >> 3), qq = 32 * qt + row, c8 = lane & 7;
-        if (qq < S) {
+        if constexpr (PAIR) {
+          if (qq <= S) {
+            const float4 a0 = ld4(&so[row * AX_OST + 8 * c8]), a1 = ld4(&so[row * AX_OST + 8 * c8 + 4]);
+            const float4 cf = ld4(&so[row * AX_OST + 64]);
+            const float a[8] = {a0.x, a0.y, a0.z, a0.w, a1.x, a1.y, a1.z, a1.w};
+            const int d0 = 64 * pass + 8 * c8;
+#pragma unroll
+            for (int x = 0; x < 2; ++x) {
+              if (x == 0 ? qq < S : qq >= 1) {
+                const float ca = x == 0 ? cf.x : cf.z, ce = x == 0 ? cf.y : cf.w;
+                const float4 w0 = ld4(&v0[x * AX_HD + d0]), w1 = ld4(&v0[x * AX_HD + d0 + 4]);
+                const float v[8] = {ca * a[0] + ce * w0.x, ca * a[1] + ce * w0.y, ca * a[2] + ce * w0.z, ca * a[3] + ce * w0.w,
+                                    ca * a[4] + ce * w1.x, ca * a[5] + ce * w1.y, ca * a[6] + ce * w1.z, ca * a[7] + ce * w1.w};
+                const int orow = (x == 1 && qq == S) ? 0 : qq;
+                const size_t oo = ((size_t)(seq + x * B) * S + orow) * D + head * AX_HD + d0;
+                if (out != nullptr) {
+                  st4(out + oo, make_float4(v[0], v[1], v[2], v[3]));
+                  st4(out + oo + 4, make_float4(v[4], v[5], v[6], v[7]));
+                }
+                if (oh != nullptr) {
+                  p16x8 hi, lo;
+                  split8(v, hi, lo);
+                  *reinterpret_cast<p16x8*>(oh + oo) = hi;
+                  *reinterpret_cast<p16x8*>(ol + oo) = lo;
+                }
+              }
+            }
+          }
+        } else if (qq < S) {
           const float4 v0 = ld4(&so[row * AX_OST + 8 * c8]), v1 = ld4(&so[row * AX_OST + 8 * c8 + 4]);
           const size_t oo = obase + (size_t)qq * D + 64 * pass + 8 * c8;
           if (out != nullptr) {
@@ -613,8 +682,21 @@
   }
 }
 
+template <int NKT>
+__global__ __launch_bounds__(AXW_THREADS) void attention_x3_kernel_wide(QkvPlanes P, const int* __restrict__ lengths, int S, int D,
+                                                                       int B, int lead, float* __restrict__ out,
+                                                                       p16_t* __restrict__ oh, p16_t* __restrict__ ol, int items) {
+  axw_body<NKT, false>(P, lengths, S, D, B, lead, out, oh, ol, items);
+}
+template <int NKT>
+__global__ __launch_bounds__(AXW_THREADS) void attention_x3_kernel_pair(QkvPlanes P, const int* __restrict__ lengths, int S, int D,
+                                                                       int B, int lead, float* __restrict__ out,
+                                                                       p16_t* __restrict__ oh, p16_t* __restrict__ ol, int items) {
+  axw_body<NKT, true>(P, lengths, S, D, B, lead, out, oh, ol, items);
+}
+
 __global__ __launch_bounds__(256) void qkv_pack_kernel(const float* __restrict__ qkv, QkvPlanes P, int nseq, int S,
-                                                       int D) {
+                                                       int D, int pair_B = 0) {
   const int SP = P.SP, H = P.H;
   const size_t total = (size_t)nseq * H * SP * AX_HD;
   for (size_t i = (size_t)blockIdx.x * blockDim.x + threadIdx.x; i < total; i += (size_t)gridDim.x * blockDim.x) {
@@ -626,6 +708,9 @@
     if (tok < S) {
       const float* row = qkv + ((size_t)seq * S + tok) * 3 * D + head * AX_HD + d;
       q = row[0]; k = row[D]; v = row[2 * D];
+    } else if (pair_B > 0 && tok == S) {
+      const float* row = qkv + (size_t)(pair_B + seq) * S * 3 * D + head * AX_HD + d;
+      q = row[0]; k = row[D]; v = row[2 * D];
     }
     p16_t a, b;
     const size_t rk = (shd * SP + tok) * AX_HD + d;
diff --git a/motion-diffusion-model_amd/csrc/encoder.h b/motion-diffusion-model_amd/csrc/encoder.h
--- a/motion-diffusion-model_amd/csrc/encoder.h
+++ b/motion-diffusion-model_amd/csrc/encoder.h
@@ -75,6 +75,7 @@
       X3Call c = stack; c.kind = kind; c.pf = pf; c.a = a; c.w = w; c.bias = bias; c.N = N; c.K = K;
       return c;
     };
+    bool pair_att = false;
     for (int l = 0; l < m->cfg.num_layers; ++l) {
       const mdm_model::LayerPlanes& P = m->planes[l];
       const mdm_model::LayerFold& F = m->fold[l];
@@ -83,14 +84,17 @@
         c.qp = &ws.qp; c.scale_cols = D; c.col_scale = qscale;
         if (int rc = launch_x3_ln(c, s)) return rc;
       } else if (l == 0) {
-        const int pair_B = (m->enc_shared_l0 && nseq == 2 * B && x3_qkv_pairs(S, D)) ? B : 0;
-        if (int rc = launch_in_proj_x3(pf, xb, P.in_proj, m->L(l, "self_attn.in_proj_bias"), ws.qp, nseq, S, D, qscale, s, pair_B)) return rc;
+        const int pair_B = (m->enc_shared_l0 >= 1 && nseq == 2 * B && x3_qkv_pairs(S, D)) ? B : 0;
+        pair_att = pair_B > 0 && m->enc_shared_l0 >= 2 && attention_x3_pairs(S) && m->attn_wide;
+        if (int rc = launch_in_proj_x3(pf, xb, P.in_proj, m->L(l, "self_attn.in_proj_bias"), ws.qp, nseq, S, D, qscale, s, pair_B, pair_att)) return rc;
       } else {
         X3Call c = LN(X3K_IN_PROJ_FOLD, xb, F.in_proj, F.b_qkv, 3 * D, D);
         c.astat = ws.stat2; c.colsum = F.c_qkv; c.qp = &ws.qp; c.scale_cols = D; c.col_scale = qscale;
         if (int rc = launch_x3_ln(c, s)) return rc;
       }
-      if (int rc = launch_attention_x3(pf, ws.qp, lengths, nseq, B, S, D, nullptr, ws.atth, ws.attl, s, 1, m->attn_direct, m->attn_wide)) return rc;
+      if (l == 0 && pair_att) {
+        if (int rc = launch_attention_x3_pair(pf, ws.qp, lengths, B, S, D, nullptr, ws.atth, ws.attl, s)) return rc;
+      } else if (int rc = launch_attention_x3(pf, ws.qp, lengths, nseq, B, S, D, nullptr, ws.atth, ws.attl, s, 1, m->attn_direct, m->attn_wide)) return rc;
       {
         X3Call c = LN(l == 0 ? X3K_OUT_PROJ_L0 : X3K_OUT_LN_RES, attp, P.out_proj, m->L(l, "self_attn.out_proj.bias"), D, D);
         c.oh = ws.xah; c.ol = ws.xal; c.res = xb; c.ostat = ws.stat1;
diff --git a/motion-diffusion-model_amd/csrc/gemm_x3.h b/motion-diffusion-model_amd/csrc/gemm_x3.h
--- a/motion-diffusion-model_amd/csrc/gemm_x3.h
+++ b/motion-diffusion-model_amd/csrc/gemm_x3.h
@@ -142,6 +142,7 @@
   X3_F6 = 1u << 7,
   X3_PIPE = 1u << 8,
   X3_PAIR = 1u << 9,
+  X3_PAIR_ONE = 1u << 10,
 };
 template <int ACT, int RES, unsigned FLAGS>
 __global__ __launch_bounds__(64 * X3_NWAVE, 2) void gemm_x3_kernel(X3Operand A, X3Weights W, X3Epilogue ep, int M, int N, int K,
@@ -150,7 +151,9 @@
   constexpr bool OUT_F32 = (FLAGS & X3_OUT_F32) != 0, OUT_PLANES = (FLAGS & X3_OUT_PLANES) != 0, OUT_QKV = (FLAGS & X3_OUT_QKV) != 0;
   constexpr bool FOLD = (FLAGS & X3_FOLD) != 0, OSTAT = (FLAGS & X3_OSTAT) != 0, EMBED = (FLAGS & X3_EMBED) != 0;
   constexpr bool T16 = (FLAGS & X3_T16) != 0, F6 = (FLAGS & X3_F6) != 0, PIPE = (FLAGS & X3_PIPE) != 0, PAIR = (FLAGS & X3_PAIR) != 0;
-  static_assert(FLAGS < (X3_PAIR << 1), "unknown flag");
+  constexpr bool PAIR_ONE = (FLAGS & X3_PAIR_ONE) != 0;
+  static_assert(FLAGS < (X3_PAIR_ONE << 1), "unknown flag");
+  static_assert(!PAIR_ONE || PAIR, "the single-destination epilogue belongs to the paired tile");
   static_assert((int)OUT_F32 + (int)OUT_PLANES + (int)OUT_QKV == 1, "exactly one output form");
   static_assert(RES >= 0 && RES <= 3 && !(OUT_QKV && RES != 0), "in_proj has no residual");
   static_assert(!(FOLD && RES == 3), "one (mean, rstd) table: of the A rows or of the residual rows");
@@ -618,7 +621,7 @@
               auto vfin = [&](float a) __attribute__((always_inline)) { return a * accs + b16; };
               float u0 = 0.f;
               size_t po = 0;
-              if constexpr (PAIR) {
+              if constexpr (PAIR && !PAIR_ONE) {
                 const int sS = ep.S >> 4, eS = ep.S & 3;
 #pragma unroll
                 for (int s = 0; s < NS16; ++s) {
@@ -645,7 +648,7 @@
                   }
                   const size_t o = o0 + (size_t)(s >> 1) * (AX_HD * 32) + 16 * (s & 1);
                   split4_store(ep.qkv.vh + o, ep.qkv.vl + o, make_float4(vv[0], vv[1], vv[2], vv[3]));
-                  if constexpr (PAIR) {
+                  if constexpr (PAIR && !PAIR_ONE) {
                     const float k0 = (s == 0 && g16 == 0) ? u0 : vv[0];
                     split4_store(ep.qkv.vh + po + o, ep.qkv.vl + po + o, make_float4(k0, vv[1], vv[2], vv[3]));
                   }
@@ -717,7 +720,9 @@
             if (t < nkt) {
               const int tok = 32 * t + 8 * g + prow;
               v4 = finish4(v4, st);
-              if constexpr (PAIR) {
+              if constexpr (PAIR_ONE) {
+                if (tok <= ep.S) split4_store(dh + tok * AX_HD, dl + tok * AX_HD, v4);
+              } else if constexpr (PAIR) {
                 if (tok < ep.S) split4_store(dh + tok * AX_HD, dl + tok * AX_HD, v4);
                 if ((unsigned)(tok - 1) < (unsigned)ep.S) {
                   const int tok2 = tok == ep.S ? 0 : tok;
@@ -904,6 +909,7 @@
   auto kfn = &gemm_x3_kernel<ACT, RES, FLAGS>;
   if (T16 && rpt > X3_TM - 16) return -2;
   if (PAIR && (rpt + 1 > X3_TM - 16 || ep.pair_B < 1 || M != ep.pair_B * rpt)) return -2;
+  if ((FLAGS & X3_PAIR_ONE) != 0 && (rpt % 32 == 0 || rpt >= ep.qkv.SP)) return -2;
   if (PIPE && (K / X3_BK) % 2 != 0) return -2;
   if (!x3_has_col_scale(ACT, RES) && ep.scale_cols > 0) return -2;
 #ifndef MDM_EMU
@@ -980,14 +986,17 @@
 inline bool x3_qkv_pairs(int S, int D) { return S + 1 <= X3_TM - 16 && (D / X3_BK) % 2 == 0; }
 
 inline int launch_gemm_x3_qkv(const X3Operand& A, const X3Weights& W, const X3Epilogue& ep, int nseq, int S, int D,
-                                  hipStream_t s, int pair_B = 0) {
+                                  hipStream_t s, int pair_B = 0, bool pair_one = false) {
   if (S > X3_TM) return -2;
   if (pair_B > 0) {
     if (nseq != 2 * pair_B || !x3_qkv_pairs(S, D)) return -2;
     X3Epilogue ep2 = ep;
     ep2.pair_B = pair_B;
+    if (pair_one)
+      return launch_gemm_x3_w<ACT_NONE,  0, X3_OUT_QKV | X3_T16 | X3_PIPE | X3_PAIR | X3_PAIR_ONE>(A, W, ep2, pair_B * S, 3 * D, D, S, s);
     return launch_gemm_x3_w<ACT_NONE,  0, X3_OUT_QKV | X3_T16 | X3_PIPE | X3_PAIR>(A, W, ep2, pair_B * S, 3 * D, D, S, s);
   }
+  if (pair_one) return -2;
   if (S <= X3_TM - 16) {
     if ((D / X3_BK) % 2 == 0) return launch_gemm_x3_w<ACT_NONE,  0, X3_OUT_QKV | X3_T16 | X3_PIPE>(A, W, ep, nseq * S, 3 * D, D, S, s);
     return launch_gemm_x3_w<ACT_NONE,  0, X3_OUT_QKV | X3_T16>(A, W, ep, nseq * S, 3 * D, D, S, s);
diff --git a/motion-diffusion-model_amd/csrc/mdm_api.hip b/motion-diffusion-model_amd/csrc/mdm_api.hip
--- a/motion-diffusion-model_amd/csrc/mdm_api.hip
+++ b/motion-diffusion-model_amd/csrc/mdm_api.hip
@@ -164,8 +164,8 @@
       m->dec_time_token = value != 0;
       return MDM_OK;
     case MDM_OPT_ENC_SHARED_LAYER0:
-      if (value != 0 && value != 1) return fail(MDM_EINVAL, "mdm_set_option: MDM_OPT_ENC_SHARED_LAYER0 must be 0 or 1");
-      m->enc_shared_l0 = value != 0;
+      if (value < 0 || value > 2) return fail(MDM_EINVAL, "mdm_set_option: MDM_OPT_ENC_SHARED_LAYER0 must be 0, 1 or 2");
+      m->enc_shared_l0 = value;
       return MDM_OK;
     default:
       return fail(MDM_EINVAL, "mdm_set_option: unknown key " + std::to_string(key));
@@ -190,7 +190,7 @@
     case MDM_OPT_ATTN_DIRECT_OUT: *value = m->attn_direct ? 1 : 0; return MDM_OK;
     case MDM_OPT_ATTN_WIDE: *value = m->attn_wide ? 1 : 0; return MDM_OK;
     case MDM_OPT_DEC_TIME_TOKEN: *value = m->dec_time_token ? 1 : 0; return MDM_OK;
-    case MDM_OPT_ENC_SHARED_LAYER0: *value = m->enc_shared_l0 ? 1 : 0; return MDM_OK;
+    case MDM_OPT_ENC_SHARED_LAYER0: *value = m->enc_shared_l0; return MDM_OK;
     default: return fail(MDM_EINVAL, "mdm_get_option: unknown key " + std::to_string(key));
   }
 }
diff --git a/motion-diffusion-model_amd/csrc/probe_api.h b/motion-diffusion-model_amd/csrc/probe_api.h
--- a/motion-diffusion-model_amd/csrc/probe_api.h
+++ b/motion-diffusion-model_amd/csrc/probe_api.h
@@ -121,6 +121,25 @@
                              false, wide != 0);
 }
 
+int mdm_probe_attention_x3_pair(const float* qkv, float* out, void* out_hi, void* out_lo, const int32_t* lengths, int32_t B, int32_t S,
+                                int32_t D, int32_t H, void* scratch, size_t scratch_bytes, void* stream) {
+  if (!qkv || B <= 0 || S <= 0 || H <= 0) return fail(MDM_EINVAL, "mdm_probe_attention_x3_pair: bad argument");
+  if (!attention_x3_pairs(S))
+    return mdm_probe_attention_x3(qkv, out, out_hi, out_lo, lengths, 2 * B, B, S, D, H, 1, 1, scratch, scratch_bytes, stream);
+  ChainGuard chain_guard(stream);
+  if ((!out && !out_hi) || (out_hi == nullptr) != (out_lo == nullptr) || !scratch) return fail(MDM_EINVAL, "mdm_probe_attention_x3_pair: bad argument");
+  if (D != H * AX_HD) return fail(MDM_EUNSUPPORTED, "attention: head_dim must be 128");
+  if (scratch_bytes < mdm_attention_x3_scratch_bytes(B, S, D)) return fail(MDM_ENOSPC, "mdm_probe_attention_x3_pair: scratch too small");
+  hipStream_t s = static_cast<hipStream_t>(stream);
+  const int NKT = (S + 31) / 32, SP = 32 * NKT;
+  const size_t plane = (size_t)B * SP * D;
+  p16_t* q = static_cast<p16_t*>(scratch);
+  QkvPlanes qp{q, q + plane, q + 2 * plane, q + 3 * plane, q + 4 * plane, q + 5 * plane, SP, NKT, H};
+  MDM_LAUNCH(qkv_pack_kernel, dim3((int)std::min<size_t>((plane + 255) / 256, 4096)), dim3(256), 0, s, qkv, qp, B, S, D, B);
+  if (int rc = rt_launch_status()) return rc;
+  return launch_attention_x3_pair(nullptr, qp, lengths, B, S, D, out, static_cast<p16_t*>(out_hi), static_cast<p16_t*>(out_lo), s);
+}
+
 int mdm_probe_in_proj(const float* tokens, const float* w, const float* bias, void* planes_dev, int32_t nseq, int32_t S,
                       int32_t D, void* scratch_dev, void* stream) {
   ChainGuard chain_guard(stream);
@@ -142,4 +161,25 @@
   return launch_in_proj_x3(nullptr, X3Operand{ah, al}, X3Weights{wh, wl}, bias, qp, nseq, S, D, 0.08838834764831845f, s);
 }
 
+int mdm_probe_in_proj_pair(const float* tokens, const float* w, const float* bias, void* planes_dev, int32_t B, int32_t S, int32_t D,
+                           int32_t one, void* scratch_dev, void* stream) {
+  ChainGuard chain_guard(stream);
+  if (!tokens || !w || !bias || !planes_dev || !scratch_dev || B <= 0 || S <= 0 || D % 256 != 0) return fail(MDM_EINVAL, "mdm_probe_in_proj_pair");
+  if (!x3_qkv_pairs(S, D) || (one && S % 32 == 0)) return fail(MDM_EUNSUPPORTED, "mdm_probe_in_proj_pair: no paired tile at this shape");
+  hipStream_t s = static_cast<hipStream_t>(stream);
+  const int nseq = 2 * B;
+  const size_t n = (size_t)nseq * S * D;
+  p16_t* ah = static_cast<p16_t*>(scratch_dev);
+  p16_t* al = ah + n;
+  p16_t* wh = al + n;
+  p16_t* wl = wh + (size_t)3 * D * D;
+  if (int rc = launch_split(tokens, ah, al, n, s)) return rc;
+  if (int rc = launch_pack_weights(w, wh, wl, 3 * D, D, s)) return rc;
+  const int H = D / AX_HD, NKT = (S + 31) / 32, SP = 32 * NKT;
+  const size_t plane = (size_t)nseq * SP * D;
+  p16_t* q = static_cast<p16_t*>(planes_dev);
+  QkvPlanes qp{q, q + plane, q + 2 * plane, q + 3 * plane, q + 4 * plane, q + 5 * plane, SP, NKT, H};
+  return launch_in_proj_x3(nullptr, X3Operand{ah, al}, X3Weights{wh, wl}, bias, qp, nseq, S, D, 0.08838834764831845f, s, B, one != 0);
 }
+
+}
```
